# shahbuland/owl-audio-exps

Measured on AMD Instinct MI355X. Metric: latent-tokens/sec/GPU (fwd+bwd) DiT-v4 bf16; 1/2/4/8-GPU scaling, higher is better.
Workload: dtype bf16; 1 GPU; configs/dit_v4.yml training step: global batch 16 x 1536 frames x 8x8 latents (98304 tokens/sample), fwd+bwd + Muon/AdamW step + EMA; model=dit_v4 (16 L, d1536, 24 H, 704.9M params), global_batch=16, seq_len=98304, parallelism=dp1

## Files before the change

include/owlk.h:

```cpp
#ifndef OWLK_H
#define OWLK_H
#ifdef __cplusplus
extern "C" {
#endif

const char* owlk_last_error(void);
int owlk_version(void);
int owlk_device_ok(void);

#define OWLK_DECODE_COUNTER_BYTES 4096
int owlk_gemm(long M, long N, long K, long batch,
              const void* A, long lda, long sA, int a_trans,
              const void* B, long ldb, long sB, int b_trans,
              void* C, long ldc, long sC, int c_f32,
              int epi, float alpha, float beta, const float* bias,
              void* aux, long ldaux, long sAux,
              const void* gate, long ldgate, long sGate, long tpf,
              const void* resid, long ldres, long sRes,
              float* colsum, void* ws, long ws_bytes, void* stream);
#define OWLK_FRAME_ROWS 64
int owlk_gemm_frames(long M, long N, long K, const void* A, long lda, long a_fs, int a_trans,
                     const void* B, long ldb, long b_fs, int b_trans, void* C, long ldc, long c_fs,
                     int c_f32, int epi, float alpha, float beta, const float* bias, void* aux, long ldaux,
                     const void* gate, long ldgate, long tpf, const void* resid, long ldres, void* ws,
                     long ws_bytes, void* stream);
int owlk_gemm_attn_delta(long M, long N, long K, const void* dY, long lddy, const void* W, long ldw, void* dO,
                         long ldc, const void* o, long ldo, long L, int H, int D, float* delta, void* stream);
int owlk_gemm_qk_rope(long M, long N, long K, const void* A, long lda, const void* W, long ldw, const float* bias,
                      void* qkv, long ldq, int H, int D, const float* cosb, const float* sinb, long ld_tab, long n_tab,
                      long tab_off, long tpos_div, void* out, long ldo, float* rstd, void* stream);
long owlk_gemm_splitk_bytes(long M, long N, long K, long batch, int a_trans, int b_trans, int c_f32, int epi,
                            float beta);
long owlk_gemm_ws_bytes(long M, long N, long K, long batch, int a_trans, int b_trans, int c_f32, int epi,
                        float beta, int colsum);
long owlk_gemm_ws_counter_bytes(long M, long N, long K, long batch, int a_trans, int b_trans, int c_f32, int epi,
                                float beta);

int owlk_adaln_fwd(const void* x, long ldx, const void* scale, const void* shift, long ldm, long tpf,
                   long T, int d, void* y, long ldy, float* rstd, void* yact , void* stream);
int owlk_adaln_bwd(const void* dy, long lddy, const void* x, long ldx, const float* rstd,
                   const void* scale, long ldm, long tpf, long T, int d, const void* dres, long ldres,
                   void* dx, long lddx, void* dscale, void* dshift, long ldg,
                   const void* ypre , int mod_bf16, void* stream);

int owlk_gate_bwd(const void* dout, long ldo, const void* y, long ldy, const void* g, long ldg, long tpf,
                  long T, int d, void* dy, long lddy, void* dg, long lddg, int dg_bf16, float* dbias_frames,
                  long ldr, void* stream);
int owlk_adaln_gate_bwd(const void* dy, long lddy, const void* x, long ldx, const float* rstd,
                        const void* scale, long ldm, long tpf, long T, int d, const void* dres, long ldres,
                        void* dx, long lddx, void* dscale, void* dshift, long ldg, int mod_bf16,
                        const void* y, long ldy, const void* g, long ldgg, void* dyg, long lddyg, void* dg,
                        long lddg, int dg_bf16, float* dbias_frames, long ldr, void* stream);

int owlk_qk_rope_fwd(const void* qkv, long ldq, long T, int H, int D, const float* cosb, const float* sinb,
                     long ld_tab, long n_tab, long tab_off, long tpos_div, void* out, long ldo, float* rstd,
                     void* stream);
int owlk_qk_rope_fwd_kv(const void* qkv, long ldq, long T, long L, int H, int D, const float* cosb,
                        const float* sinb, long ld_tab, long n_tab, long tab_off, void* qo, long ldqo, long sqo,
                        void* ko, long ldko, long sko, void* vo, long ldvo, long svo, void* stream);
int owlk_qk_rope_fwd_kv_dev(const void* qkv, long ldq, long T, long L, int H, int D, const float* cosb,
                            const float* sinb, long ld_tab, long n_tab, const long* state, void* qo, long ldqo,
                            long sqo, void* kbuf, long ldk, long skb, void* vbuf, long ldv, long svb, long cap,
                            void* stream);
int owlk_mm_qk_rope_fwd_kv(const void* qkv0, long ld0, const void* qkv1, long ld1, long B, long nf, int n0, int n1,
                           int H, int D, const float* cosb, const float* sinb, long ld_tab, long n_tab,
                           long tab_off, void* qo, long ldqo, long sqo, void* ko, long ldko, long sko, void* vo,
                           long ldvo, long svo, void* stream);
int owlk_qk_rope_bwd(const void* dqk, long ldd, const void* qkv, long ldq, long T, int H, int D,
                     const float* cosb, const float* sinb, long ld_tab, long n_tab, long tab_off, long tpos_div,
                     const float* rstd, void* dqkv, long ldg, void* stream);
long owlk_qk_rope_bwd_ws_bytes(long T, int H, int D);
int owlk_qk_rope_bwd_bias(const void* dqk, long ldd, const void* qkv, long ldq, long T, int H, int D,
                          const float* cosb, const float* sinb, long ld_tab, long n_tab, long tab_off, long tpos_div,
                          const float* rstd, void* dqkv, long ldg, float* dbias, void* ws, long ws_bytes,
                          void* stream);

int owlk_attn_fwd(const void* q, long ldq, long sqb, const void* k, long ldk, long skb, const void* v,
                  long ldv, long svb, void* o, long ldo, long sob, float* lse, long B, int H, long Lq,
                  long Lkv, int head_dim, float scale, float score_bound, long tpf, int window, int causal,
                  long q_offset,
                  const int* kv_lo, const int* q_hi, const int* run_start, const int* doc, long fstride,
                  void* stream);
int owlk_attn_decode_fwd(const void* q, long ldq, long sqb, const void* kbuf, long ldk, long skb,
                         const void* vbuf, long ldv, long svb, void* o, long ldo, long sob, float* lse, long B,
                         int H, long Lq, int head_dim, float scale, float score_bound, const long* state,
                         long Lnew, long window_tokens, long cap, void* stream);
int owlk_attn_decode_joint_fwd(const void* q, long ldq, long sqb, const void* k, long ldk, long skb, const void* v,
                               long ldv, long svb, void* o0, long ldo0, void* o1, long ldo1, float* lse, long B,
                               int H, int n0, int n1, long Lkv, int head_dim, float scale, float score_bound,
                               void* stream);
int owlk_attn_delta(const void* o, const void* dout, long ld, long B, long L, int H, int D, float* delta,
                    void* stream);
int owlk_attn_bwd(const void* q, long ldq, long sqb, const void* k, long ldk, long skb, const void* v,
                  long ldv, long svb, const void* dout, long ldo, long sob, const float* lse,
                  const float* delta, void* dq, long lddq, long sdqb, void* dk, long lddk, long sdkb,
                  void* dv, long lddv, long sdvb, long B, int H, long Lq, long Lkv, int head_dim,
                  float scale, long tpf, int window, int causal, const int* kv_lo, const int* q_hi,
                  const int* run_start, const int* doc, long fstride, void* stream);
int owlk_attn_bwd_dkdv(const void* q, long ldq, long sqb, const void* k, long ldk, long skb, const void* v,
                       long ldv, long svb, const void* dout, long ldo, long sob, const float* lse,
                       const float* delta, void* dq, long lddq, long sdqb, void* dk, long lddk, long sdkb,
                       void* dv, long lddv, long sdvb, long B, int H, long Lq, long Lkv, int head_dim,
                       float scale, long tpf, int window, int causal, const int* kv_lo, const int* q_hi,
                       const int* run_start, const int* doc, long fstride, void* stream);
int owlk_attn_bwd_dq(const void* q, long ldq, long sqb, const void* k, long ldk, long skb, const void* v,
                     long ldv, long svb, const void* dout, long ldo, long sob, const float* lse,
                     const float* delta, void* dq, long lddq, long sdqb, void* dk, long lddk, long sdkb,
                     void* dv, long lddv, long sdvb, long B, int H, long Lq, long Lkv, int head_dim,
                     float scale, long tpf, int window, int causal, const int* kv_lo, const int* q_hi,
                     const int* run_start, const int* doc, long fstride, void* stream);

long owlk_attn_decode_bwd_ws_bytes(long B, int H, long Lq, long Lkv, int head_dim);
int owlk_attn_decode_bwd(const void* q, long ldq, long sqb, const void* k, long ldk, long skb, const void* v,
                         long ldv, long svb, const void* dout, long ldo, long sob, const float* lse,
                         const float* delta, void* dq, long lddq, long sdqb, void* dk_new, long lddk, long sdkb,
                         void* dv_new, long lddv, long sdvb, long B, int H, long Lq, long Lkv, long Lnew,
                         int head_dim, float scale, void* ws, long ws_bytes, void* stream);

long owlk_attn_bwd_fused_ws_bytes(long B, int H, long L, int head_dim);
int owlk_attn_bwd_fused(const void* q, long ldq, long sqb, const void* k, long ldk, long skb, const void* v,
                        long ldv, long svb, const void* dout, long ldo, long sob, const float* lse,
                        const float* delta, void* dq, long lddq, long sdqb, void* dk, long lddk, long sdkb,
                        void* dv, long lddv, long sdvb, long B, int H, long L, int head_dim, float scale,
                        long tpf, int window, int causal, const int* kv_lo, const int* q_hi,
                        const int* run_start, const int* doc, long fstride, void* ws, long ws_bytes,
                        int variant, void* stream);
int owlk_set_cu_reserve(int cus);

int owlk_flow_noise(const void* x, const void* z, const float* ts_raw, int C, int P, long BN, void* xt,
                    void* tgt, float* ts_out, void* stream);
int owlk_unpatchify(const void* tok, int C, int P, long BN, void* out, void* stream);
int owlk_gate_resid(const void* x, long ldx, const void* y, long ldy, const void* g, long ldg, long tpf, long T,
                    int d, void* out, long ldo, void* stream);
int owlk_mse(const void* pred, const void* tgt, long n, float gscale, void* dpred, float* partial,
             int nblocks, float* loss, void* stream);
int owlk_mse_grad(const void* pred, const void* tgt, long n, float gscale, const float* gout, void* dpred,
                  void* stream);
long owlk_dmd_loss_ws_bytes(long B, long N, long F);
int owlk_dmd_loss(const void* video, const void* noisy, int in_f32, const void* v_cond, const void* v_uncond,
                  const void* v_critic, int v_f32, const float* ts, const void* mask, long B, long N, long F,
                  float cfg_scale, float* loss, void* dvideo, void* ws, long ws_bytes, void* stream);
long owlk_critic_loss_ws_bytes(long n);
int owlk_critic_loss(const void* pred, int pred_f32, const void* z, const void* video, int in_f32,
                     const void* mask, long B, long N, long F, float gscale, float* loss, void* dpred, void* ws,
                     long ws_bytes, void* stream);
long owlk_colsum_ws_bytes(long R, long N);
int owlk_colsum(const void* x, int x_f32, long R, long N, long ld, float* out, void* ws, long ws_bytes,
                void* stream);
int owlk_colsum_frames(const void* x, int x_f32, long R, long N, long ld, long fs, float* out, void* ws,
                       long ws_bytes, void* stream);

#define OWLK_NORM_PARTS 256
int owlk_ns_normalize(const void* g, int g_f32, long rows, long cols, long batch, int transpose, void* x,
                      float* work, void* stream);
int owlk_ns_scale(const void* g, int g_f32, long rows, long cols, long batch, int transpose, void* x,
                  const float* sumsq, void* stream);
long owlk_ns_iterate_ws_bytes(long batch, long m, long k);
int owlk_ns_iterate(void* x, long batch, long m, long k, int steps, float a, float b, float c, void* ws,
                    long ws_bytes, void* stream);
long owlk_newton_schulz_ws_bytes(long batch, long rows, long cols);
int owlk_newton_schulz_bf16(const void* g, int g_f32, long batch, long rows, long cols, int steps, float a,
                            float b, float c, void* out, void* ws, long ws_bytes, void* stream);

int owlk_cond_embed(const void* ts, int ts_f32, const float* tfreq, int ht, float tmult, void* ts_in, long ldt,
                    const void* mouse, int mouse_f32, long ldm, const float* mfreq, int hm, float mmult,
                    const float* wang, void* mouse_in, long ldmi, void* ang, const void* btn, int btn_f32, long ldb,
                    int nb, int nbp, void* btn_in, long ldbi, long R, void* stream);
int owlk_cond_silu_fwd(const void* t, const void* m, const void* b, const void* hc, long rows_per, long R, int d,
                       void* cond, void* s, void* stream);
int owlk_cond_silu_bwd(const void* ds, int ds_bf16, const void* cond, const void* hc, long rows_per, long R, int d,
                       void* dcond, void* dctrl, void* stream);
int owlk_small_k_wgrad(const void* dy, long lddy, const void* x, long ldx, long R, long N, int K, float* dw,
                       long ldw, float beta, void* stream);

int owlk_muon_momentum(int count, float* const* g, float* const* buf, long n, float momentum, int nesterov,
                       float* stack, float* sumsq, void* stream);
int owlk_muon_apply(int count, float* const* p, const void* u, long rows, long cols, int transpose, float decay,
                    float alpha, void* stream);
int owlk_adamw(int count, float* const* p, const float* const* g, float* const* m, float* const* v, const long* n,
               float lr, float beta1, float beta2, float weight_decay, float eps, float step_size, float bc2_sqrt,
               void* stream);
int owlk_ema(int count, float* const* shadow, const float* const* p, const long* n, float weight, void* stream);

int owlk_frame_mux(int dir, long frames, int n0, int n1, int cols, void* a, long lda, void* b, long ldb,
                   void* joint, long ldj, void* stream);
int owlk_layernorm_fwd(const void* x, long ldx, long T, int d, void* y, long ldy, float* mean, float* rstd,
                       void* stream);
int owlk_layernorm_bwd(const void* dy, long lddy, const void* x, long ldx, const float* mean, const float* rstd,
                       long T, int d, void* dx, long lddx, void* stream);

#ifdef __cplusplus
}
#endif
#endif
```

owl-audio-exps_amd/csrc/gemm.hip:

```cpp
#include "common.hpp"

#include <algorithm>
#include <cstdlib>

namespace {

enum Epi : int {
  EPI_STORE = 0,
  EPI_SILU = 1,
  EPI_GATE_RESID = 2,
  EPI_DSILU = 3,
  EPI_AXPBY = 4,
  EPI_SCALE2 = 5,
  EPI_DELTA = 6,
  EPI_QKROPE = 7,
};

constexpr int BK = 64;
constexpr int NT = 256;

struct GemmP {
  long M, N, K;
  const bf16* A; long lda, sA;
  const bf16* B; long ldb, sB;
  void* C; long ldc, sC;
  float alpha, beta;
  const float* bias;
  bf16* aux; long ldaux, sAux;
  const bf16* gate; long ldgate, sGate, tpf;
  unsigned tpf_mul; int tpf_shift;
  const bf16* resid; long ldres, sRes;
  int tiles_m, tiles_n;
  long kchunk;
  float* ws;
  float* colsum_req;
  float* colsum;
  float* cs_part;
  int group_m;
  long a_fs, b_fs, c_fs;
  float* delta;
  long dl;
  const float* rcos;
  const float* rsin;
  long ld_tab, tab_off, tpos_div;
  float* rstd;
  long qk_cols;
};
constexpr float QK_RMS_EPS = 1.1920928955078125e-07f;

constexpr int FRAME_ROWS = 64;
#ifndef OWLK_GEMM_EPI2
#define OWLK_GEMM_EPI2 1
#endif

template <bool F>
DEV long row_off(long r, long ld, long fs) {
  return F ? (r >> 6) * fs + (r & 63) * ld : r * ld;
}

template <int ROWS>
DEV int swz_t(int k) {
  if (ROWS >= 128) return (k & 3) | (((k >> 3) & 1) << 2);
  return ((k >> 1) & 1) | (((k >> 3) & 1) << 1);
}

template <int ROWS, bool TRANS>
struct Stager {
  static constexpr int CHUNKS = ROWS * BK / 8;
  static constexpr int PER = CHUNKS / NT;
  bf16x8 r[PER];

  DEV void load(const bf16* base, long ld, long r0, long k0, long R, long K) {
    const int tid = threadIdx.x;
#pragma unroll
    for (int i = 0; i < PER; ++i) {
      const int c = tid + i * NT;
      long row, col;
      bool ok;
      if (!TRANS) {
        row = r0 + (c >> 3);
        col = k0 + (c & 7) * 8;
        ok = row < R && col < K;
        r[i] = ok ? *(const bf16x8*)(base + row * ld + col) : bf16x8{};
      } else {
        constexpr int CPR = ROWS / 8;
        row = k0 + c / CPR;
        col = r0 + (c % CPR) * 8;
        ok = row < K && col < R;
        r[i] = ok ? *(const bf16x8*)(base + row * ld + col) : bf16x8{};
      }
    }
  }

  DEV void store(char* lds) const {
    const int tid = threadIdx.x;
#pragma unroll
    for (int i = 0; i < PER; ++i) {
      const int c = tid + i * NT;
      int off;
      if (!TRANS) {
        const int row = c >> 3, kc = c & 7;
        off = row * 128 + ((kc ^ ((row >> 1) & 7)) << 4);
      } else {
        constexpr int CPR = ROWS / 8;
        const int k = c / CPR, mc = c % CPR;
        off = k * (ROWS * 2) + (((mc >> 1) ^ swz_t<ROWS>(k)) << 5) + ((mc & 1) << 4);
      }
      *(bf16x8*)(lds + off) = r[i];
    }
  }
};

template <int ROWS, bool TRANS>
DEV bf16x8 read_frag(const char* lds, int row0, int kk, int lane) {
  if (!TRANS) {
    const int r = row0 + (lane & 15);
    const int kc = 4 * kk + (lane >> 4);
    return *(const bf16x8*)(lds + r * 128 + ((kc ^ ((r >> 1) & 7)) << 4));
  } else {
    const int g = lane >> 4, q = (lane & 15) >> 2, pp = lane & 3;
    const int blk = row0 >> 4;
    const int k0 = 32 * kk + 8 * g + q;
    const int k1 = k0 + 4;
    s16x4 lo = ds_read_tr16(lds + k0 * (ROWS * 2) + ((blk ^ swz_t<ROWS>(k0)) << 5) + pp * 8);
    s16x4 hi = ds_read_tr16(lds + k1 * (ROWS * 2) + ((blk ^ swz_t<ROWS>(k1)) << 5) + pp * 8);
    return join_tr(lo, hi);
  }
}

template <int ROWS, bool TRANS>
DEV bf16x8 read_frag_async(const char* lds, int row0, int kk, int lane) {
  if (!TRANS) return read_frag<ROWS, false>(lds, row0, kk, lane);
  const int g = lane >> 4, q = (lane & 15) >> 2, pp = lane & 3;
  const int blk = row0 >> 4;
  const int k0 = 32 * kk + 8 * g + q;
  const int k1 = k0 + 4;
  s16x4 lo = ds_read_tr16_async(lds + k0 * (ROWS * 2) + ((blk ^ swz_t<ROWS>(k0)) << 5) + pp * 8);
  s16x4 hi = ds_read_tr16_async(lds + k1 * (ROWS * 2) + ((blk ^ swz_t<ROWS>(k1)) << 5) + pp * 8);
  return join_tr(lo, hi);
}

DEV unsigned frame_of(const GemmP& p, unsigned row) {
  return p.tpf_mul ? __umulhi(row, p.tpf_mul) >> p.tpf_shift : row >> p.tpf_shift;
}

template <int EPI, bool OF32>
DEV void epi_chunk(const GemmP& p, long z, long gm, long gn, float (&v)[8]) {
  float bb[8];
#pragma unroll
  for (int e = 0; e < 8; ++e) bb[e] = 0.f;
  if (p.bias) {
    const f32x4 lo = *(const f32x4*)(p.bias + gn), hi = *(const f32x4*)(p.bias + gn + 4);
#pragma unroll
    for (int e = 0; e < 4; ++e) {
      bb[e] = rb(lo[e]);
      bb[e + 4] = rb(hi[e]);
    }
  }
  if (EPI == EPI_STORE) {
#pragma unroll
    for (int e = 0; e < 8; ++e) v[e] = p.alpha * v[e] + bb[e];
    if (OF32) {
      float* C = (float*)p.C + z * p.sC + gm * p.ldc + gn;
      if (p.beta != 0.f) {
        const f32x4 o0 = *(const f32x4*)C, o1 = *(const f32x4*)(C + 4);
#pragma unroll
        for (int e = 0; e < 4; ++e) {
          v[e] += p.beta * o0[e];
          v[e + 4] += p.beta * o1[e];
        }
      }
      *(f32x4*)C = f32x4{v[0], v[1], v[2], v[3]};
      *(f32x4*)(C + 4) = f32x4{v[4], v[5], v[6], v[7]};
    } else {
      bf16* C = (bf16*)p.C + z * p.sC + gm * p.ldc + gn;
      if (p.beta != 0.f) {
        float o[8];
        unpack8(*(const bf16x8*)C, o);
#pragma unroll
        for (int e = 0; e < 8; ++e) v[e] += p.beta * o[e];
      }
      *(bf16x8*)C = pack8(v);
    }
  } else if (EPI == EPI_SILU) {
    float y[8], s[8];
#pragma unroll
    for (int e = 0; e < 8; ++e) {
      y[e] = rb(v[e] + bb[e]);
      s[e] = silu_f(y[e]);
    }
    *(bf16x8*)(p.aux + z * p.sAux + gm * p.ldaux + gn) = pack8(y);
    *(bf16x8*)((bf16*)p.C + z * p.sC + gm * p.ldc + gn) = pack8(s);
  } else if (EPI == EPI_GATE_RESID) {
    float y[8], g[8], r[8], o[8];
#pragma unroll
    for (int e = 0; e < 8; ++e) y[e] = rb(v[e] + bb[e]);
    unpack8(*(const bf16x8*)(p.gate + z * p.sGate + (long)frame_of(p, (unsigned)gm) * p.ldgate + gn), g);
    unpack8(*(const bf16x8*)(p.resid + z * p.sRes + gm * p.ldres + gn), r);
#pragma unroll
    for (int e = 0; e < 8; ++e) o[e] = r[e] + rb(g[e] * y[e]);
    if (p.aux) *(bf16x8*)(p.aux + z * p.sAux + gm * p.ldaux + gn) = pack8(y);
    *(bf16x8*)((bf16*)p.C + z * p.sC + gm * p.ldc + gn) = pack8(o);
  } else if (EPI == EPI_DSILU) {
    float x[8], o[8];
    unpack8(*(const bf16x8*)(p.aux + z * p.sAux + gm * p.ldaux + gn), x);
#pragma unroll
    for (int e = 0; e < 8; ++e) {
      const float sg = sigmoid_f(x[e]);
      o[e] = rb(v[e]) * sg * (1.f + x[e] * (1.f - sg));
    }
    *(bf16x8*)((bf16*)p.C + z * p.sC + gm * p.ldc + gn) = pack8(o);
    if (p.resid) {
      float a[8];
#pragma unroll
      for (int e = 0; e < 8; ++e) a[e] = silu_f(x[e]);
      *(bf16x8*)((bf16*)p.resid + z * p.sRes + gm * p.ldres + gn) = pack8(a);
    }
  } else if (EPI == EPI_AXPBY) {
    float x[8], o[8];
    unpack8(*(const bf16x8*)(p.aux + z * p.sAux + gm * p.ldaux + gn), x);
#pragma unroll
    for (int e = 0; e < 8; ++e) o[e] = rb(rb(p.alpha * rb(v[e])) + rb(p.beta * x[e]));
    *(bf16x8*)((bf16*)p.C + z * p.sC + gm * p.ldc + gn) = pack8(o);
  } else if (EPI == EPI_SCALE2) {
    float y[8], o[8];
#pragma unroll
    for (int e = 0; e < 8; ++e) {
      y[e] = rb(v[e]);
      o[e] = rb(p.alpha * y[e]);
    }
    *(bf16x8*)((bf16*)p.C + z * p.sC + gm * p.ldc + gn) = pack8(y);
    *(bf16x8*)(p.aux + z * p.sAux + gm * p.ldaux + gn) = pack8(o);
  }
}

DEV void st_nt(bf16x8* dst, bf16x8 v) { __builtin_nontemporal_store(v, dst); }

template <int EPI, bool OF32, bool CF = false>
DEV void epi_apply(const GemmP& p, long z, long gm, long gn, float (&v)[8], const float (&bb)[8], const bf16x8& x,
                   const bf16x8& g, float (&cs)[8]) {
  if (EPI == EPI_STORE) {
#pragma unroll
    for (int e = 0; e < 8; ++e) v[e] = p.alpha * v[e] + bb[e];
    if (OF32) {
      float* C = (float*)p.C + z * p.sC + gm * p.ldc + gn;
      if (p.beta != 0.f) {
        const f32x4 o0 = *(const f32x4*)C, o1 = *(const f32x4*)(C + 4);
#pragma unroll
        for (int e = 0; e < 4; ++e) {
          v[e] += p.beta * o0[e];
          v[e + 4] += p.beta * o1[e];
        }
      }
      *(f32x4*)C = f32x4{v[0], v[1], v[2], v[3]};
      *(f32x4*)(C + 4) = f32x4{v[4], v[5], v[6], v[7]};
    } else {
      bf16* C = (bf16*)p.C + z * p.sC + row_off<CF>(gm, p.ldc, p.c_fs) + gn;
      if (p.beta != 0.f) {
        float o[8];
        unpack8(*(const bf16x8*)C, o);
#pragma unroll
        for (int e = 0; e < 8; ++e) v[e] += p.beta * o[e];
      }
      st_nt((bf16x8*)C, pack8(v));
    }
  } else if (EPI == EPI_SILU) {
    float y[8], s[8];
#pragma unroll
    for (int e = 0; e < 8; ++e) {
      y[e] = rb(v[e] + bb[e]);
      s[e] = silu_f(y[e]);
    }
    st_nt((bf16x8*)(p.aux + z * p.sAux + gm * p.ldaux + gn), pack8(y));
    st_nt((bf16x8*)((bf16*)p.C + z * p.sC + gm * p.ldc + gn), pack8(s));
  } else if (EPI == EPI_GATE_RESID) {
    float y[8], gg[8], r[8], o[8];
#pragma unroll
    for (int e = 0; e < 8; ++e) y[e] = rb(v[e] + bb[e]);
    unpack8(g, gg);
    unpack8(x, r);
#pragma unroll
    for (int e = 0; e < 8; ++e) o[e] = r[e] + rb(gg[e] * y[e]);
    if (p.aux) st_nt((bf16x8*)(p.aux + z * p.sAux + gm * p.ldaux + gn), pack8(y));
    st_nt((bf16x8*)((bf16*)p.C + z * p.sC + gm * p.ldc + gn), pack8(o));
  } else if (EPI == EPI_DSILU) {
    float xx[8], o[8];
    unpack8(x, xx);
#pragma unroll
    for (int e = 0; e < 8; ++e) {
      const float sg = sigmoid_f(xx[e]);
      o[e] = rb(v[e]) * sg * (1.f + xx[e] * (1.f - sg));
    }
    st_nt((bf16x8*)((bf16*)p.C + z * p.sC + gm * p.ldc + gn), pack8(o));
    if (p.resid) {
      float a[8];
#pragma unroll
      for (int e = 0; e < 8; ++e) a[e] = silu_f(xx[e]);
      st_nt((bf16x8*)((bf16*)p.resid + z * p.sRes + gm * p.ldres + gn), pack8(a));
    }
    if (p.colsum) {
#pragma unroll
      for (int e = 0; e < 8; ++e) cs[e] += rb(o[e]);
    }
  } else if (EPI == EPI_AXPBY) {
    float xx[8], o[8];
    unpack8(x, xx);
#pragma unroll
    for (int e = 0; e < 8; ++e) o[e] = rb(rb(p.alpha * rb(v[e])) + rb(p.beta * xx[e]));
    st_nt((bf16x8*)((bf16*)p.C + z * p.sC + gm * p.ldc + gn), pack8(o));
  } else if (EPI == EPI_SCALE2) {
    float y[8], o[8];
#pragma unroll
    for (int e = 0; e < 8; ++e) {
      y[e] = rb(v[e]);
      o[e] = rb(p.alpha * y[e]);
    }
    st_nt((bf16x8*)((bf16*)p.C + z * p.sC + gm * p.ldc + gn), pack8(y));
    st_nt((bf16x8*)(p.aux + z * p.sAux + gm * p.ldaux + gn), pack8(o));
  }
}

template <int EPI, bool OF32>
DEV void epi_apply2(const GemmP& p, long c, long ao, long ro, float (&v)[8], const float (&bb)[8],
                    const bf16x8& x, const bf16x8& g, float (&cs)[8]) {
  const u32x4 xw = __builtin_bit_cast(u32x4, x), gw = __builtin_bit_cast(u32x4, g);
  u32x4 o, y;
  if (EPI == EPI_STORE) {
#pragma unroll
    for (int e = 0; e < 8; ++e) v[e] = p.alpha * v[e] + bb[e];
    if (OF32) {
      float* C = (float*)p.C + c;
      if (p.beta != 0.f) {
        const f32x4 o0 = *(const f32x4*)C, o1 = *(const f32x4*)(C + 4);
#pragma unroll
        for (int e = 0; e < 4; ++e) {
          v[e] += p.beta * o0[e];
          v[e + 4] += p.beta * o1[e];
        }
      }
      *(f32x4*)C = f32x4{v[0], v[1], v[2], v[3]};
      *(f32x4*)(C + 4) = f32x4{v[4], v[5], v[6], v[7]};
    } else {
      bf16* C = (bf16*)p.C + c;
      if (p.beta != 0.f) {
        float ob[8];
        unpack8(*(const bf16x8*)C, ob);
#pragma unroll
        for (int e = 0; e < 8; ++e) v[e] += p.beta * ob[e];
      }
#pragma unroll
      for (int k = 0; k < 4; ++k) o[k] = cvt2(v[2 * k], v[2 * k + 1]);
      st_nt((bf16x8*)C, __builtin_bit_cast(bf16x8, o));
    }
  } else if (EPI == EPI_SILU) {
#pragma unroll
    for (int k = 0; k < 4; ++k) {
      y[k] = cvt2(v[2 * k] + bb[2 * k], v[2 * k + 1] + bb[2 * k + 1]);
      o[k] = cvt2(silu_f(bf_lo(y[k])), silu_f(bf_hi(y[k])));
    }
    st_nt((bf16x8*)(p.aux + ao), __builtin_bit_cast(bf16x8, y));
    st_nt((bf16x8*)((bf16*)p.C + c), __builtin_bit_cast(bf16x8, o));
  } else if (EPI == EPI_GATE_RESID) {
#pragma unroll
    for (int k = 0; k < 4; ++k) {
      y[k] = cvt2(v[2 * k] + bb[2 * k], v[2 * k + 1] + bb[2 * k + 1]);
      const unsigned t = cvt2(bf_lo(gw[k]) * bf_lo(y[k]), bf_hi(gw[k]) * bf_hi(y[k]));
      o[k] = cvt2(bf_lo(xw[k]) + bf_lo(t), bf_hi(xw[k]) + bf_hi(t));
    }
    if (p.aux) st_nt((bf16x8*)(p.aux + ao), __builtin_bit_cast(bf16x8, y));
    st_nt((bf16x8*)((bf16*)p.C + c), __builtin_bit_cast(bf16x8, o));
  } else if (EPI == EPI_DSILU) {
    u32x4 a;
#pragma unroll
    for (int k = 0; k < 4; ++k) {
      const unsigned rv = cvt2(v[2 * k], v[2 * k + 1]);
      float ov[2];
#pragma unroll
      for (int h = 0; h < 2; ++h) {
        const float xx = h ? bf_hi(xw[k]) : bf_lo(xw[k]);
        const float sg = sigmoid_f(xx);
        ov[h] = (h ? bf_hi(rv) : bf_lo(rv)) * sg * (1.f + xx * (1.f - sg));
      }
      o[k] = cvt2(ov[0], ov[1]);
      a[k] = cvt2(silu_f(bf_lo(xw[k])), silu_f(bf_hi(xw[k])));
      cs[2 * k] += bf_lo(o[k]);
      cs[2 * k + 1] += bf_hi(o[k]);
    }
    st_nt((bf16x8*)((bf16*)p.C + c), __builtin_bit_cast(bf16x8, o));
    if (p.resid) st_nt((bf16x8*)((bf16*)p.resid + ro), __builtin_bit_cast(bf16x8, a));
  } else if (EPI == EPI_AXPBY) {
#pragma unroll
    for (int k = 0; k < 4; ++k) {
      const unsigned r = cvt2(v[2 * k], v[2 * k + 1]);
      const unsigned s1 = cvt2(p.alpha * bf_lo(r), p.alpha * bf_hi(r));
      const unsigned s2 = cvt2(p.beta * bf_lo(xw[k]), p.beta * bf_hi(xw[k]));
      o[k] = cvt2(bf_lo(s1) + bf_lo(s2), bf_hi(s1) + bf_hi(s2));
    }
    st_nt((bf16x8*)((bf16*)p.C + c), __builtin_bit_cast(bf16x8, o));
  } else if (EPI == EPI_SCALE2) {
#pragma unroll
    for (int k = 0; k < 4; ++k) {
      y[k] = cvt2(v[2 * k], v[2 * k + 1]);
      o[k] = cvt2(p.alpha * bf_lo(y[k]), p.alpha * bf_hi(y[k]));
    }
    st_nt((bf16x8*)((bf16*)p.C + c), __builtin_bit_cast(bf16x8, y));
    st_nt((bf16x8*)(p.aux + ao), __builtin_bit_cast(bf16x8, o));
  } else if (EPI == EPI_QKROPE) {
#pragma unroll
    for (int e = 0; e < 8; ++e) v[e] = p.alpha * v[e] + bb[e];
#pragma unroll
    for (int k = 0; k < 4; ++k) {
      o[k] = cvt2(v[2 * k], v[2 * k + 1]);
      cs[2 * k] = bf_lo(o[k]);
      cs[2 * k + 1] = bf_hi(o[k]);
    }
    st_nt((bf16x8*)((bf16*)p.C + c), __builtin_bit_cast(bf16x8, o));
  } else if (EPI == EPI_DELTA) {
    float sd = 0.f;
#pragma unroll
    for (int k = 0; k < 4; ++k) {
      o[k] = cvt2(p.alpha * v[2 * k], p.alpha * v[2 * k + 1]);
      sd += bf_lo(xw[k]) * bf_lo(o[k]);
      sd += bf_hi(xw[k]) * bf_hi(o[k]);
    }
    st_nt((bf16x8*)((bf16*)p.C + c), __builtin_bit_cast(bf16x8, o));
    cs[0] = sd;
  }
}

template <int BM, int BN, bool AT, bool BT, int EPI, bool OF32>
__global__ __launch_bounds__(NT) void gemm_kernel(GemmP p) {
  constexpr int WTM = BM / 2, WTN = BN / 2;
  constexpr int TM = WTM / 16, TN = WTN / 16;
  constexpr int A_BYTES = BM * BK * 2, B_BYTES = BN * BK * 2;
  constexpr int STAGE_BYTES = 2 * (A_BYTES + B_BYTES);
  constexpr int EPI_LD = BN + 4;
  constexpr int EPI_BYTES = BM * EPI_LD * 4;
  constexpr int LDS_BYTES = STAGE_BYTES > EPI_BYTES ? STAGE_BYTES : EPI_BYTES;
  __shared__ __attribute__((aligned(16))) char smem[LDS_BYTES];

  const int lane = threadIdx.x & 63, wave = threadIdx.x >> 6;
  const int wm = wave >> 1, wn = wave & 1;

  const int nwg = p.tiles_m * p.tiles_n;
  int bid = blockIdx.x;
  {
    const int q = nwg / 8, r = nwg % 8, x = bid % 8;
    bid = (x < r ? x * (q + 1) : r * (q + 1) + (x - r) * q) + bid / 8;
  }
  const int tm = bid / p.tiles_n, tn = bid % p.tiles_n;
  const long m0 = (long)tm * BM, n0 = (long)tn * BN;
  const long z = blockIdx.z;
  const bf16* A = p.A + z * p.sA;
  const bf16* B = p.B + z * p.sB;

  Stager<BM, AT> sa;
  Stager<BN, BT> sb;
  f32x4 acc[TM][TN];
#pragma unroll
  for (int i = 0; i < TM; ++i)
#pragma unroll
    for (int j = 0; j < TN; ++j) acc[i][j] = f32x4{0.f, 0.f, 0.f, 0.f};

  const long kbeg = (long)blockIdx.y * p.kchunk;
  const long kend = kbeg + p.kchunk < p.K ? kbeg + p.kchunk : p.K;
  const int nk = (int)((kend - kbeg + BK - 1) / BK);
  sa.load(A, p.lda, m0, kbeg, p.M, p.K);
  sb.load(B, p.ldb, n0, kbeg, p.N, p.K);
  sa.store(smem);
  sb.store(smem + A_BYTES);
  __syncthreads();

  for (int kt = 0; kt < nk; ++kt) {
    const int cur = kt & 1;
    const bool more = kt + 1 < nk;
    if (more) {
      sa.load(A, p.lda, m0, kbeg + (long)(kt + 1) * BK, p.M, p.K);
      sb.load(B, p.ldb, n0, kbeg + (long)(kt + 1) * BK, p.N, p.K);
    }
    const char* la = smem + cur * (A_BYTES + B_BYTES);
    const char* lb = la + A_BYTES;
#pragma unroll
    for (int kk = 0; kk < 2; ++kk) {
      bf16x8 af[TM], bfr[TN];
#pragma unroll
      for (int i = 0; i < TM; ++i) af[i] = read_frag<BM, AT>(la, wm * WTM + 16 * i, kk, lane);
#pragma unroll
      for (int j = 0; j < TN; ++j) bfr[j] = read_frag<BN, BT>(lb, wn * WTN + 16 * j, kk, lane);
#pragma unroll
      for (int i = 0; i < TM; ++i)
#pragma unroll
        for (int j = 0; j < TN; ++j)
          acc[i][j] = __builtin_amdgcn_mfma_f32_16x16x32_bf16(af[i], bfr[j], acc[i][j], 0, 0, 0);
    }
    if (more) {
      char* nb = smem + (cur ^ 1) * (A_BYTES + B_BYTES);
      sa.store(nb);
      sb.store(nb + A_BYTES);
    }
    __syncthreads();
  }

  float* ct = (float*)smem;
#pragma unroll
  for (int i = 0; i < TM; ++i)
#pragma unroll
    for (int j = 0; j < TN; ++j) {
      const int col = wn * WTN + 16 * j + (lane & 15);
      const int row = wm * WTM + 16 * i + (lane >> 4) * 4;
#pragma unroll
      for (int r = 0; r < 4; ++r) ct[(row + r) * EPI_LD + col] = acc[i][j][r];
    }
  __syncthreads();

  if (p.ws) {
    float* W = p.ws + (long)blockIdx.y * p.M * p.N;
    for (int c = threadIdx.x; c < BM * BN / 4; c += NT) {
      const int row = c / (BN / 4), col = (c % (BN / 4)) * 4;
      const long gm = m0 + row, gn = n0 + col;
      if (gm < p.M && gn < p.N)
        __builtin_nontemporal_store(*(const f32x4*)(ct + row * EPI_LD + col), (f32x4*)(W + gm * p.N + gn));
    }
    return;
  }
  if (OF32 && EPI == EPI_STORE && gridDim.y > 1) {
    float* C = (float*)p.C + z * p.sC;
    for (int row = wave; row < BM; row += NT / 64) {
      const long gm = m0 + row;
      if (gm >= p.M) break;
#pragma unroll
      for (int cc = 0; cc < BN; cc += 64) {
        const long gn = n0 + cc + lane;
        if (gn < p.N) atomicAdd(C + gm * p.ldc + gn, p.alpha * ct[row * EPI_LD + cc + lane]);
      }
    }
    return;
  }

  constexpr int CH = BM * BN / 8;
  for (int c = threadIdx.x; c < CH; c += NT) {
    const int row = c / (BN / 8), col = (c % (BN / 8)) * 8;
    const long gm = m0 + row, gn = n0 + col;
    if (gm >= p.M || gn >= p.N) continue;
    float v[8];
    {
      const f32x4 lo = *(const f32x4*)(ct + row * EPI_LD + col);
      const f32x4 hi = *(const f32x4*)(ct + row * EPI_LD + col + 4);
#pragma unroll
      for (int e = 0; e < 4; ++e) {
        v[e] = lo[e];
        v[e + 4] = hi[e];
      }
    }
    epi_chunk<EPI, OF32>(p, z, gm, gn, v);
  }
}


constexpr int NT8 = 512;

template <int ROWS, bool TRANS, bool F = false>
DEV void glds_tile(char* lds, const bf16* base, long ld, long r0, long k0, long R, int wave, int lane, long fs = 0) {
  if (!TRANS) {
#pragma unroll
    for (int i = 0; i < ROWS / 64; ++i) {
      const int rbase = (wave * (ROWS / 64) + i) * 8;
      const int row = rbase + (lane >> 3);
      const int ch = (lane & 7) ^ ((row >> 1) & 7);
      long gr = r0 + row;
      gr = gr < R ? gr : R - 1;
      __builtin_amdgcn_global_load_lds((const void __attribute__((address_space(1)))*)(base + row_off<F>(gr, ld, fs) +
                                                                                         k0 + ch * 8),
                                       (void __attribute__((address_space(3)))*)(lds + rbase * 128), 16, 0, 0);
    }
  } else {
    constexpr int KPI = 512 / ROWS;
    constexpr int CPR = ROWS / 8;
#pragma unroll
    for (int i = 0; i < 64 / KPI / 8; ++i) {
      const int kb = (wave * (64 / KPI / 8) + i) * KPI;
      const int k = kb + lane / CPR;
      const int pch = lane % CPR;
      const int lch = ((((pch >> 1) ^ swz_t<ROWS>(k))) << 1) | (pch & 1);
      __builtin_amdgcn_global_load_lds(
          (const void __attribute__((address_space(1)))*)(base + row_off<F>(k0 + k, ld, fs) + r0 + lch * 8),
          (void __attribute__((address_space(3)))*)(lds + kb * ROWS * 2), 16, 0, 0);
    }
  }
}

template <int BN, bool AT, bool BT, int EPI, bool OF32>
__global__ __launch_bounds__(NT8, 1) void gemm256_kernel(GemmP p) {
  constexpr int BM = 256, WARPS_N = BN / 64, WTM = BM / (8 / WARPS_N), WTN = 64, TM = WTM / 16, TN = 4;
  constexpr int NBUF = BN == 256 ? 2 : 3;
  constexpr int A_BYTES = BM * BK * 2, B_BYTES = BN * BK * 2, STAGE = A_BYTES + B_BYTES;
  constexpr int OPS = (BM + BN) * BK * 2 / (NT8 * 16);
  __shared__ __attribute__((aligned(16))) char smem[NBUF * STAGE];
  const int lane = threadIdx.x & 63, wave = __builtin_amdgcn_readfirstlane(threadIdx.x >> 6);
  const int wm = wave / WARPS_N, wn = wave % WARPS_N;

  const int nwg = p.tiles_m * p.tiles_n;
  int bid = blockIdx.x;
  {
    const int q = nwg / 8, r = nwg % 8, x = bid % 8;
    bid = (x < r ? x * (q + 1) : r * (q + 1) + (x - r) * q) + bid / 8;
  }
  const int tm = bid / p.tiles_n, tn = bid % p.tiles_n;
  const long m0 = (long)tm * BM, n0 = (long)tn * BN;
  const long z = blockIdx.z;
  const bf16* A = p.A + z * p.sA;
  const bf16* B = p.B + z * p.sB;
  const long kbeg = (long)blockIdx.y * p.kchunk;
  const long kend = kbeg + p.kchunk < p.K ? kbeg + p.kchunk : p.K;
  const int nk = (int)((kend - kbeg) / BK);

  f32x4 acc[TM][TN];
#pragma unroll
  for (int i = 0; i < TM; ++i)
#pragma unroll
    for (int j = 0; j < TN; ++j) acc[i][j] = f32x4{0.f, 0.f, 0.f, 0.f};

  auto issue = [&](int kt) {
    char* buf = smem + (kt % NBUF) * STAGE;
    glds_tile<BM, AT>(buf, A, p.lda, m0, kbeg + (long)kt * BK, p.M, wave, lane);
    glds_tile<BN, BT>(buf + A_BYTES, B, p.ldb, n0, kbeg + (long)kt * BK, p.N, wave, lane);
  };
  auto wait_next = [&](bool younger_in_flight) {
    if (NBUF > 2 && younger_in_flight)
      asm volatile("s_waitcnt vmcnt(%0)" ::"n"(OPS) : "memory");
    else
      asm volatile("s_waitcnt vmcnt(0)" ::: "memory");
  };
#pragma unroll
  for (int i = 0; i < NBUF - 1; ++i)
    if (i < nk) issue(i);
  wait_next(nk > 1);
  asm volatile("s_waitcnt lgkmcnt(0)\n\ts_barrier" ::: "memory");

  for (int kt = 0; kt < nk; ++kt) {
    if (kt + NBUF - 1 < nk) issue(kt + NBUF - 1);
    const char* la = smem + (kt % NBUF) * STAGE;
    const char* lb = la + A_BYTES;
#pragma unroll
    for (int kk = 0; kk < 2; ++kk) {
      bf16x8 af[TM], bfr[TN];
#pragma unroll
      for (int j = 0; j < TN; ++j) bfr[j] = read_frag<BN, BT>(lb, wn * WTN + 16 * j, kk, lane);
#pragma unroll
      for (int i = 0; i < TM; ++i) af[i] = read_frag<BM, AT>(la, wm * WTM + 16 * i, kk, lane);
      __builtin_amdgcn_s_setprio(1);
#pragma unroll
      for (int i = 0; i < TM; ++i)
#pragma unroll
        for (int j = 0; j < TN; ++j)
          acc[i][j] = __builtin_amdgcn_mfma_f32_16x16x32_bf16(af[i], bfr[j], acc[i][j], 0, 0, 0);
      __builtin_amdgcn_s_setprio(0);
    }
    wait_next(kt + NBUF - 1 < nk);
    asm volatile("s_waitcnt lgkmcnt(0)\n\ts_barrier" ::: "memory");
  }

  float* strip = (float*)smem + wave * (16 * 68);
  const bool atomic = OF32 && EPI == EPI_STORE && gridDim.y > 1;
#pragma unroll
  for (int i = 0; i < TM; ++i) {
#pragma unroll
    for (int j = 0; j < TN; ++j)
#pragma unroll
      for (int r = 0; r < 4; ++r) strip[((lane >> 4) * 4 + r) * 68 + 16 * j + (lane & 15)] = acc[i][j][r];
    asm volatile("s_waitcnt lgkmcnt(0)" ::: "memory");
    const long rbase = m0 + wm * WTM + 16 * i;
    if (atomic) {
      float* C = (float*)p.C + z * p.sC;
#pragma unroll
      for (int rr = 0; rr < 16; ++rr) {
        const long gm = rbase + rr;
        if (gm < p.M) atomicAdd(C + gm * p.ldc + n0 + wn * WTN + lane, p.alpha * strip[rr * 68 + lane]);
      }
    } else {
#pragma unroll
      for (int q = 0; q < 2; ++q) {
        const int c = lane + 64 * q;
        const int rr = c >> 3, col = (c & 7) * 8;
        const long gm = rbase + rr, gn = n0 + wn * WTN + col;
        float v[8];
        const f32x4 lo = *(const f32x4*)(strip + rr * 68 + col);
        const f32x4 hi = *(const f32x4*)(strip + rr * 68 + col + 4);
#pragma unroll
        for (int e = 0; e < 4; ++e) {
          v[e] = lo[e];
          v[e + 4] = hi[e];
        }
        if (gm < p.M) epi_chunk<EPI, OF32>(p, z, gm, gn, v);
      }
    }
    asm volatile("s_waitcnt lgkmcnt(0)" ::: "memory");
  }
}

template <bool AT, bool BT, int EPI, bool OF32, int FS = 0>
__global__ __launch_bounds__(NT8, 1) void gemm_pp_kernel(GemmP p) {
  constexpr bool FA = FS & 1, FB = (FS & 2) != 0, FC = (FS & 4) != 0;
  constexpr int HALF = 128 * BK * 2, STAGE = 4 * HALF;
  __shared__ __attribute__((aligned(16))) char smem[2 * STAGE];
  const int lane = threadIdx.x & 63, wave = __builtin_amdgcn_readfirstlane(threadIdx.x >> 6);
  const int wr = wave >> 2, wc = wave & 3;

  const int nwg = p.tiles_m * p.tiles_n;
  int bid = blockIdx.x;
  {
    const int q = nwg / 8, r = nwg % 8, x = bid % 8;
    bid = (x < r ? x * (q + 1) : r * (q + 1) + (x - r) * q) + bid / 8;
  }
  int tm, tn;
  if (p.group_m > 1) {
    const int span = p.group_m * p.tiles_n, g = bid / span, first = g * p.group_m;
    const int gs = p.tiles_m - first < p.group_m ? p.tiles_m - first : p.group_m;
    tm = first + (bid % span) % gs;
    tn = (bid % span) / gs;
  } else {
    tm = bid / p.tiles_n;
    tn = bid % p.tiles_n;
  }
  const long m0 = (long)tm * 256, n0 = (long)tn * 256;
  const long z = blockIdx.z;
  const bf16* A = p.A + z * p.sA;
  const bf16* B = p.B + z * p.sB;
  const long kbeg = (long)blockIdx.y * p.kchunk;
  const long kend = kbeg + p.kchunk < p.K ? kbeg + p.kchunk : p.K;
  const int nk = (int)((kend - kbeg) / BK);

  f32x4 acc[8][4];
#pragma unroll
  for (int i = 0; i < 8; ++i)
#pragma unroll
    for (int j = 0; j < 4; ++j) acc[i][j] = f32x4{0.f, 0.f, 0.f, 0.f};

  auto issueA = [&](int t) {
    char* st = smem + (t & 1) * STAGE;
    glds_tile<128, AT, FA>(st, A, p.lda, m0, kbeg + (long)t * BK, p.M, wave, lane, p.a_fs);
    glds_tile<128, AT, FA>(st + HALF, A, p.lda, m0 + 128, kbeg + (long)t * BK, p.M, wave, lane, p.a_fs);
  };
  auto issueB = [&](int t) {
    char* st = smem + (t & 1) * STAGE + 2 * HALF;
    glds_tile<128, BT, FB>(st, B, p.ldb, n0, kbeg + (long)t * BK, p.N, wave, lane, p.b_fs);
    glds_tile<128, BT, FB>(st + HALF, B, p.ldb, n0 + 128, kbeg + (long)t * BK, p.N, wave, lane, p.b_fs);
  };
  const int bcol = (wc & 1) * 64;
  auto readA = [&](bf16x8 (&af)[4][2], const char* la, int mh) {
#pragma unroll
    for (int kk = 0; kk < 2; ++kk)
#pragma unroll
      for (int i = 0; i < 4; ++i) af[i][kk] = read_frag_async<128, AT>(la, 64 * mh + 16 * i, kk, lane);
  };
  auto readB = [&](bf16x8 (&bq)[2][2], const char* lb, int nh) {
#pragma unroll
    for (int kk = 0; kk < 2; ++kk)
#pragma unroll
      for (int j = 0; j < 2; ++j) bq[j][kk] = read_frag_async<128, BT>(lb, bcol + 32 * nh + 16 * j, kk, lane);
  };
  auto quad = [&](const bf16x8 (&af)[4][2], const bf16x8 (&bq)[2][2], int mh, int nh) {
    __builtin_amdgcn_s_setprio(1);
#pragma unroll
    for (int kk = 0; kk < 2; ++kk)
#pragma unroll
      for (int i = 0; i < 4; ++i)
#pragma unroll
        for (int j = 0; j < 2; ++j)
          acc[4 * mh + i][2 * nh + j] =
              __builtin_amdgcn_mfma_f32_16x16x32_bf16(af[i][kk], bq[j][kk], acc[4 * mh + i][2 * nh + j], 0, 0, 0);
    __builtin_amdgcn_s_setprio(0);
  };
#define OWLK_PP_BAR() asm volatile("s_barrier" ::: "memory")
#define OWLK_PP_SYNC()                                                  \
  do {                                                                  \
    asm volatile("s_barrier\n\ts_waitcnt lgkmcnt(0)" ::: "memory");   \
    __builtin_amdgcn_sched_barrier(0);                                  \
  } while (0)

  issueA(0);
  issueB(0);
  if (nk > 1) {
    issueB(1);
    asm volatile("s_waitcnt vmcnt(4)" ::: "memory");
  } else {
    asm volatile("s_waitcnt vmcnt(0)" ::: "memory");
  }
  OWLK_PP_BAR();
  if (wr == 1) OWLK_PP_BAR();

  bf16x8 af[4][2], b0[2][2], b1[2][2];
  for (int t = 0; t < nk; ++t) {
    const char* la = smem + (t & 1) * STAGE + wr * HALF;
    const char* lb = smem + (t & 1) * STAGE + (2 + (wc >> 1)) * HALF;
    readB(b0, lb, 0);
    readA(af, la, 0);
    if (t + 1 < nk) issueA(t + 1);
    OWLK_PP_SYNC();
    quad(af, b0, 0, 0);
    OWLK_PP_BAR();
    readB(b1, lb, 1);
    OWLK_PP_SYNC();
    quad(af, b1, 0, 1);
    OWLK_PP_BAR();
    readA(af, la, 1);
    OWLK_PP_SYNC();
    quad(af, b1, 1, 1);
    OWLK_PP_BAR();
    if (t + 2 < nk) {
      issueB(t + 2);
      asm volatile("s_waitcnt vmcnt(4)" ::: "memory");
    } else {
      asm volatile("s_waitcnt vmcnt(0)" ::: "memory");
    }
    OWLK_PP_SYNC();
    quad(af, b0, 1, 0);
    OWLK_PP_BAR();
  }
  if (wr == 0) OWLK_PP_BAR();
#undef OWLK_PP_BAR
#undef OWLK_PP_SYNC
#ifdef OWLK_GEMM_EXP_NOEPI
  {
    float t = 0.f;
#pragma unroll
    for (int i = 0; i < 8; ++i)
#pragma unroll
      for (int j = 0; j < 4; ++j) t += acc[i][j][0];
    if (t == 1234.5f) ((float*)p.C)[threadIdx.x] = t;
    return;
  }
#endif

  const long wrow0 = m0 + 128 * wr, wcol0 = n0 + 64 * wc;
  float* strip = (float*)smem + wave * (16 * 68);
  const bool atomic = OF32 && EPI == EPI_STORE && gridDim.y > 1;
  const int ccol = (lane & 7) * 8;
  const long gn = wcol0 + ccol;
  float bb[8];
#pragma unroll
  for (int e = 0; e < 8; ++e) bb[e] = 0.f;
  if (!atomic && p.bias) {
    const f32x4 lo = *(const f32x4*)(p.bias + gn), hi = *(const f32x4*)(p.bias + gn + 4);
#pragma unroll
    for (int e = 0; e < 4; ++e) {
      bb[e] = rb(lo[e]);
      bb[e + 4] = rb(hi[e]);
    }
  }
  constexpr bool HAS_X = EPI == EPI_GATE_RESID || EPI == EPI_DSILU || EPI == EPI_AXPBY || EPI == EPI_DELTA;
  constexpr bool HAS_G = EPI == EPI_GATE_RESID;
  static_assert((EPI != EPI_DELTA && EPI != EPI_QKROPE) || OWLK_GEMM_EPI2,
                "EPI_DELTA / EPI_QKROPE are built in the paired epilogue only");
  constexpr int PD = (EPI == EPI_DSILU || EPI == EPI_AXPBY || EPI == EPI_DELTA) ? 8 : (EPI == EPI_GATE_RESID ? 4 : 1);
  bf16x8 xin[8][2], gin[8][2];
  const int l8 = lane >> 3;
  const bool full = m0 + 256 <= p.M;
  const long cbase = z * p.sC + row_off<FC>(wrow0 + l8, p.ldc, p.c_fs) + gn;
  const long abase = z * p.sAux + (wrow0 + l8) * p.ldaux + gn;
  const long rbase0 = z * p.sRes + (wrow0 + l8) * p.ldres + gn;
  auto c_step = [&](int d) { return FC ? (long)(d >> 6) * p.c_fs + (long)(d & 63) * p.ldc : (long)d * p.ldc; };
  auto load_in = [&](int i, bf16x8 (&x)[2], bf16x8 (&g)[2]) {
#pragma unroll
    for (int q = 0; q < 2; ++q) {
      long gm = wrow0 + 16 * i + 8 * q + (lane >> 3);
      gm = gm < p.M ? gm : p.M - 1;
      if (HAS_X && OWLK_GEMM_EPI2) {
        const int d = 16 * i + 8 * q;
        const long xo = EPI == EPI_GATE_RESID ? (full ? rbase0 + d * p.ldres : z * p.sRes + gm * p.ldres + gn)
                                              : (full ? abase + d * p.ldaux : z * p.sAux + gm * p.ldaux + gn);
        x[q] = *(const bf16x8*)((EPI == EPI_GATE_RESID ? p.resid : p.aux) + xo);
      } else if (HAS_X) {
        const bf16* src = EPI == EPI_GATE_RESID ? p.resid + z * p.sRes + gm * p.ldres
                                                 : p.aux + z * p.sAux + gm * p.ldaux;
        x[q] = *(const bf16x8*)(src + gn);
      }
      if (HAS_G) g[q] = *(const bf16x8*)(p.gate + z * p.sGate + (long)frame_of(p, (unsigned)gm) * p.ldgate + gn);
    }
  };
  if (!atomic) {
#pragma unroll
    for (int i = 0; i < PD; ++i) load_in(i, xin[i], gin[i]);
  }
  float cs[8];
#pragma unroll
  for (int e = 0; e < 8; ++e) cs[e] = 0.f;
#pragma unroll
  for (int i = 0; i < 8; ++i) {
    if (!atomic && i + PD < 8) load_in(i + PD, xin[i + PD], gin[i + PD]);
    f32x4 rcv[2], rsv[2];
    if constexpr (EPI == EPI_QKROPE) {
      if (wcol0 < p.qk_cols) {
#pragma unroll
        for (int q = 0; q < 2; ++q) {
          long gm = wrow0 + 16 * i + 8 * q + (lane >> 3);
          gm = gm < p.M ? gm : p.M - 1;
          const long pos = p.tab_off + (p.tpos_div > 0 ? gm % p.tpos_div : gm);
          rcv[q] = *(const f32x4*)(p.rcos + pos * p.ld_tab + (lane & 7) * 4);
          rsv[q] = *(const f32x4*)(p.rsin + pos * p.ld_tab + (lane & 7) * 4);
        }
      }
    }
#pragma unroll
    for (int j = 0; j < 4; ++j)
#pragma unroll
      for (int r = 0; r < 4; ++r) strip[((lane >> 4) * 4 + r) * 68 + 16 * j + (lane & 15)] = acc[i][j][r];
    asm volatile("s_waitcnt lgkmcnt(0)" ::: "memory");
    const long rbase = wrow0 + 16 * i;
    if (atomic && p.ws) {
      float* W = p.ws + (long)blockIdx.y * p.M * p.N;
#pragma unroll
      for (int rq = 0; rq < 4; ++rq) {
        const int rr = 4 * rq + (lane >> 4);
        const long gm = rbase + rr;
        if (gm < p.M)
          *(f32x4*)(W + gm * p.N + wcol0 + 4 * (lane & 15)) = *(const f32x4*)(strip + rr * 68 + 4 * (lane & 15));
      }
    } else if (atomic) {
      float* C = (float*)p.C + z * p.sC;
#pragma unroll
      for (int rr = 0; rr < 16; ++rr) {
        const long gm = rbase + rr;
        if (gm < p.M) atomicAdd(C + gm * p.ldc + wcol0 + lane, p.alpha * strip[rr * 68 + lane]);
      }
    } else {
#pragma unroll
      for (int q = 0; q < 2; ++q) {
        const int rr = 8 * q + (lane >> 3);
        const long gm = rbase + rr;
        float v[8];
        const f32x4 lo = *(const f32x4*)(strip + rr * 68 + ccol);
        const f32x4 hi = *(const f32x4*)(strip + rr * 68 + ccol + 4);
#pragma unroll
        for (int e = 0; e < 4; ++e) {
          v[e] = lo[e];
          v[e + 4] = hi[e];
        }
        if (OWLK_GEMM_EPI2) {
          const int d = 16 * i + 8 * q;
          if (gm < p.M)
            epi_apply2<EPI, OF32>(p, cbase + c_step(d), abase + d * p.ldaux, rbase0 + d * p.ldres, v, bb, xin[i][q],
                                  gin[i][q], cs);
          if constexpr (EPI == EPI_QKROPE) {
            if (wcol0 < p.qk_cols) {
              float ss = 0.f;
#pragma unroll
              for (int e = 0; e < 8; ++e) ss += cs[e] * cs[e];
              ss = gm < p.M ? ss : 0.f;
              ss += __shfl_xor(ss, 1, 64);
              ss += __shfl_xor(ss, 2, 64);
              ss += __shfl_xor(ss, 4, 64);
              const float r = rsqrtf(ss / 64 + QK_RMS_EPS);
              if (gm < p.M) {
                const int j = lane & 7;
                const long wh = wcol0 >> 6;
                if (j == 0 && p.rstd) p.rstd[gm * (p.qk_cols >> 6) + wh] = r;
                const f32x4 cv = rcv[q], sv = rsv[q];
                bf16x4 y0, y1;
#pragma unroll
                for (int e = 0; e < 4; ++e) {
                  const float x0 = rb(cs[2 * e] * r), x1 = rb(cs[2 * e + 1] * r);
                  y0[e] = (bf16)(x0 * cv[e] - x1 * sv[e]);
                  y1[e] = (bf16)(x1 * cv[e] + x0 * sv[e]);
                }
                const uint2 w0 = __builtin_bit_cast(uint2, y0), w1 = __builtin_bit_cast(uint2, y1);
                const bool odd = j & 1;
                const uint2 snd = odd ? w0 : w1;
                const uint2 rcv{(unsigned)__shfl_xor((int)snd.x, 1, 64), (unsigned)__shfl_xor((int)snd.y, 1, 64)};
                const u32x4 ow = odd ? u32x4{rcv.x, rcv.y, w1.x, w1.y} : u32x4{w0.x, w0.y, rcv.x, rcv.y};
                *(u32x4*)(p.aux + gm * p.ldaux + wh * 64 + (odd ? 32 : 0) + 8 * (j >> 1)) = ow;
              }
            }
          }
          if constexpr (EPI == EPI_DELTA) {
            float sd = gm < p.M ? cs[0] : 0.f;
            sd += __shfl_xor(sd, 1, 64);
            sd += __shfl_xor(sd, 2, 64);
            sd += __shfl_xor(sd, 4, 64);
            if ((lane & 7) == 0 && gm < p.M) {
              const long b = gm / p.dl;
              p.delta[(b * (p.N >> 6) + (gn >> 6)) * p.dl + (gm - b * p.dl)] = sd;
            }
          }
        } else if (gm < p.M) {
          if constexpr (EPI != EPI_DELTA && EPI != EPI_QKROPE)
            epi_apply<EPI, OF32, FC>(p, z, gm, gn, v, bb, xin[i][q], gin[i][q], cs);
        }
      }
    }
    asm volatile("s_waitcnt lgkmcnt(0)" ::: "memory");
  }
  if (EPI == EPI_DSILU && p.colsum) {
#pragma unroll
    for (int e = 0; e < 8; ++e) {
      cs[e] += __shfl_xor(cs[e], 8, 64);
      cs[e] += __shfl_xor(cs[e], 16, 64);
      cs[e] += __shfl_xor(cs[e], 32, 64);
    }
    if (lane < 8) {
      if (p.cs_part) {
        float* dst = p.cs_part + (long)(2 * tm + wr) * p.N + gn;
        *(f32x4*)dst = f32x4{cs[0], cs[1], cs[2], cs[3]};
        *(f32x4*)(dst + 4) = f32x4{cs[4], cs[5], cs[6], cs[7]};
      } else {
#pragma unroll
        for (int e = 0; e < 8; ++e) atomicAdd(p.colsum + gn + e, cs[e]);
      }
    }
  }
}

template <int BM, int BN, bool AT, bool BT, int EPI, bool OF32>
int launch(GemmP& p, long batch, hipStream_t s) {
  p.tiles_m = (int)((p.M + BM - 1) / BM);
  p.tiles_n = (int)((p.N + BN - 1) / BN);
  const int splits = (int)((p.K + p.kchunk - 1) / p.kchunk);
  dim3 grid(p.tiles_m * p.tiles_n, (unsigned)splits, (unsigned)batch);
  hipLaunchKernelGGL((gemm_kernel<BM, BN, AT, BT, EPI, OF32>), grid, dim3(NT), 0, s, p);
  return owlk::check_launch("gemm");
}

template <int BM, int BN, int EPI, bool OF32>
int dispatch_t(GemmP& p, int at, int bt, long batch, hipStream_t s) {
  if (!at && !bt) return launch<BM, BN, false, false, EPI, OF32>(p, batch, s);
  if (!at && bt) return launch<BM, BN, false, true, EPI, OF32>(p, batch, s);
  if (at && bt) return launch<BM, BN, true, true, EPI, OF32>(p, batch, s);
  return launch<BM, BN, true, false, EPI, OF32>(p, batch, s);
}

template <int BM, int BN>
int dispatch_e(GemmP& p, int at, int bt, int epi, int cf32, long batch, hipStream_t s) {
  switch (epi) {
    case EPI_STORE:
      return cf32 ? dispatch_t<BM, BN, EPI_STORE, true>(p, at, bt, batch, s)
                  : dispatch_t<BM, BN, EPI_STORE, false>(p, at, bt, batch, s);
    case EPI_SILU: return dispatch_t<BM, BN, EPI_SILU, false>(p, at, bt, batch, s);
    case EPI_GATE_RESID: return dispatch_t<BM, BN, EPI_GATE_RESID, false>(p, at, bt, batch, s);
    case EPI_DSILU: return dispatch_t<BM, BN, EPI_DSILU, false>(p, at, bt, batch, s);
    case EPI_AXPBY: return dispatch_t<BM, BN, EPI_AXPBY, false>(p, at, bt, batch, s);
    case EPI_SCALE2:
      if (at || bt) break;
      return launch<BM, BN, false, false, EPI_SCALE2, false>(p, batch, s);
  }
  owlk::set_error("gemm: unknown epilogue %d", epi);
  return 1;
}


template <bool AT, bool BT, int EPI, bool OF32>
int launch256(GemmP& p, long batch, hipStream_t s) {
  p.tiles_m = (int)((p.M + 255) / 256);
  p.tiles_n = (int)((p.N + 255) / 256);
  const int splits = (int)((p.K + p.kchunk - 1) / p.kchunk);
  dim3 grid(p.tiles_m * p.tiles_n, (unsigned)splits, (unsigned)batch);
  static const int pp = getenv("OWLK_GEMM_PP") ? atoi(getenv("OWLK_GEMM_PP")) : 1;
  static const int fuse_cs = getenv("OWLK_GEMM_COLSUM") ? atoi(getenv("OWLK_GEMM_COLSUM")) : 1;
  if (pp && EPI == EPI_DSILU && batch == 1 && fuse_cs) p.colsum = p.colsum_req;
  static const int group_m = getenv("OWLK_GEMM_GROUP") ? atoi(getenv("OWLK_GEMM_GROUP")) : -1;
  p.group_m = group_m >= 0 ? group_m : (splits == 1 && p.kchunk <= 4096 ? 4 : 0);
  const int fs = (p.a_fs ? 1 : 0) | (p.b_fs ? 2 : 0) | (p.c_fs ? 4 : 0);
  if (fs) {
    bool ok = false;
    if constexpr (!AT && !BT && EPI == EPI_STORE && !OF32) {
      if (fs == 4) {
        hipLaunchKernelGGL((gemm_pp_kernel<AT, BT, EPI, OF32, 4>), grid, dim3(NT8), 0, s, p);
        ok = true;
      }
    }
    if constexpr (!AT && !BT && EPI == EPI_GATE_RESID) {
      if (fs == 1) {
        hipLaunchKernelGGL((gemm_pp_kernel<AT, BT, EPI, OF32, 1>), grid, dim3(NT8), 0, s, p);
        ok = true;
      }
    }
    if constexpr (!AT && BT && EPI == EPI_STORE && !OF32) {
      if (fs == 4) {
        hipLaunchKernelGGL((gemm_pp_kernel<AT, BT, EPI, OF32, 4>), grid, dim3(NT8), 0, s, p);
        ok = true;
      }
      if (fs == 1) {
        hipLaunchKernelGGL((gemm_pp_kernel<AT, BT, EPI, OF32, 1>), grid, dim3(NT8), 0, s, p);
        ok = true;
      }
    }
    if constexpr (AT && BT && EPI == EPI_STORE && OF32) {
      if (fs == 1) {
        hipLaunchKernelGGL((gemm_pp_kernel<AT, BT, EPI, OF32, 1>), grid, dim3(NT8), 0, s, p);
        ok = true;
      }
      if (fs == 2) {
        hipLaunchKernelGGL((gemm_pp_kernel<AT, BT, EPI, OF32, 2>), grid, dim3(NT8), 0, s, p);
        ok = true;
      }
    }
    OWLK_REQUIRE(ok && pp, "gemm: frame-strided rows (mask %d) not built for this operand layout / epilogue", fs);
    return owlk::check_launch("gemm256");
  }
  if constexpr (EPI == EPI_DELTA || EPI == EPI_QKROPE) {
    OWLK_REQUIRE(pp && splits == 1 && batch == 1, "gemm: the delta / rope epilogues run in the unsplit ping-pong kernel");
    hipLaunchKernelGGL((gemm_pp_kernel<AT, BT, EPI, OF32>), grid, dim3(NT8), 0, s, p);
  } else if (pp) {
    hipLaunchKernelGGL((gemm_pp_kernel<AT, BT, EPI, OF32>), grid, dim3(NT8), 0, s, p);
  } else {
    hipLaunchKernelGGL((gemm256_kernel<256, AT, BT, EPI, OF32>), grid, dim3(NT8), 0, s, p);
  }
  return owlk::check_launch("gemm256");
}

template <int EPI, bool OF32>
int dispatch256_t(GemmP& p, int at, int bt, long batch, hipStream_t s) {
  if (!at && !bt) return launch256<false, false, EPI, OF32>(p, batch, s);
  if (!at && bt) return launch256<false, true, EPI, OF32>(p, batch, s);
  if (at && bt) return launch256<true, true, EPI, OF32>(p, batch, s);
  return launch256<true, false, EPI, OF32>(p, batch, s);
}

int dispatch256(GemmP& p, int at, int bt, int epi, int cf32, long batch, hipStream_t s) {
  switch (epi) {
    case EPI_STORE:
      return cf32 ? dispatch256_t<EPI_STORE, true>(p, at, bt, batch, s)
                  : dispatch256_t<EPI_STORE, false>(p, at, bt, batch, s);
    case EPI_SILU: return dispatch256_t<EPI_SILU, false>(p, at, bt, batch, s);
    case EPI_GATE_RESID: return dispatch256_t<EPI_GATE_RESID, false>(p, at, bt, batch, s);
    case EPI_DSILU: return dispatch256_t<EPI_DSILU, false>(p, at, bt, batch, s);
    case EPI_AXPBY: return dispatch256_t<EPI_AXPBY, false>(p, at, bt, batch, s);
    case EPI_SCALE2:
      if (at || bt) break;
      return launch256<false, false, EPI_SCALE2, false>(p, batch, s);
    case EPI_DELTA:
      if (at || !bt) break;
      return launch256<false, true, EPI_DELTA, false>(p, batch, s);
    case EPI_QKROPE:
      if (at || bt) break;
      return launch256<false, false, EPI_QKROPE, false>(p, batch, s);
  }
  owlk::set_error("gemm: unknown epilogue %d", epi);
  return 1;
}
__global__ __launch_bounds__(256) void splitk_reduce_k(const float* __restrict__ W, int splits, long M, long N,
                                                       float* C, long ldc, float alpha, float beta) {
  const long nq = N / 4, total = M * nq, MN = M * N;
  for (long i = (long)blockIdx.x * 256 + threadIdx.x; i < total; i += (long)gridDim.x * 256) {
    const long m = i / nq, n = (i - m * nq) * 4;
    const float* w = W + m * N + n;
    f32x4 a = __builtin_nontemporal_load((const f32x4*)w);
    for (int sp = 1; sp < splits; ++sp) {
      const f32x4 b = __builtin_nontemporal_load((const f32x4*)(w + sp * MN));
#pragma unroll
      for (int e = 0; e < 4; ++e) a[e] += b[e];
    }
    f32x4* c = (f32x4*)(C + m * ldc + n);
    f32x4 o;
    if (beta != 0.f) {
      const f32x4 old = *c;
#pragma unroll
      for (int e = 0; e < 4; ++e) o[e] = alpha * a[e] + beta * old[e];
    } else {
#pragma unroll
      for (int e = 0; e < 4; ++e) o[e] = alpha * a[e];
    }
    *c = o;
  }
}

template <int EPI>
__global__ __launch_bounds__(256) void splitk_epi_k(GemmP p, int splits) {
  const long n8 = p.N / 8, total = p.M * n8, MN = p.M * p.N;
  for (long i = (long)blockIdx.x * 256 + threadIdx.x; i < total; i += (long)gridDim.x * 256) {
    const long m = i / n8, n = (i - m * n8) * 8;
    const float* w = p.ws + m * p.N + n;
    float v[8];
    {
      const f32x4 lo = __builtin_nontemporal_load((const f32x4*)w), hi = __builtin_nontemporal_load((const f32x4*)(w + 4));
#pragma unroll
      for (int e = 0; e < 4; ++e) {
        v[e] = lo[e];
        v[e + 4] = hi[e];
      }
    }
#pragma unroll 8
    for (int sp = 1; sp < splits; ++sp) {
      const f32x4 lo = __builtin_nontemporal_load((const f32x4*)(w + sp * MN));
      const f32x4 hi = __builtin_nontemporal_load((const f32x4*)(w + sp * MN + 4));
#pragma unroll
      for (int e = 0; e < 4; ++e) {
        v[e] += lo[e];
        v[e + 4] += hi[e];
      }
    }
    epi_chunk<EPI, false>(p, 0, m, n, v);
  }
}

constexpr int DEC_T = 64;
constexpr int DEC_KC = 256;
constexpr int DEC_ROWB = DEC_KC * 2;
constexpr int DEC_LD = DEC_T + 4;
constexpr long kDecodeCounterBytes = 4096;

template <int EPI>
__global__ __launch_bounds__(256, 1) void gemm_decode_k(GemmP p, int* counters, int nsub) {
  constexpr int STAGE = 2 * DEC_T * DEC_ROWB;
  __shared__ __attribute__((aligned(16))) char smem[2 * STAGE];
  float* tilef = (float*)smem;
  int* flag = (int*)(smem + DEC_T * DEC_LD * 4);
  const int lane = threadIdx.x & 63, wave = threadIdx.x >> 6;
  const int tile = blockIdx.x, split = blockIdx.y, S = gridDim.y, mt = blockIdx.z;
  const int tiles = gridDim.x;
  const long n0 = (long)tile * DEC_T, m0 = (long)mt * DEC_T;
  const int r16 = lane & 15, g = lane >> 4;
  const long kfirst = (long)split * nsub * DEC_KC;
  const int nst = (int)((p.K - kfirst + DEC_KC - 1) / DEC_KC < nsub ? (p.K - kfirst + DEC_KC - 1) / DEC_KC : nsub);
  const bool isw = wave < 2;
  const bf16* rowp[16];
#pragma unroll
  for (int j = 0; j < 16; ++j) {
    const int r = (wave & 1) * 32 + 2 * j + (lane >> 5);
    if (isw) {
      rowp[j] = p.B + (n0 + r) * p.ldb;
    } else {
      const long m = m0 + r < p.M ? m0 + r : p.M - 1;
      rowp[j] = p.A + m * p.lda;
    }
  }
  const int ldsrow0 = (isw ? 0 : DEC_T) + (wave & 1) * 32;
  auto issue = [&](int i) {
    const long kbeg = kfirst + (long)i * DEC_KC;
    const int nch = (int)((p.K - kbeg < DEC_KC ? p.K - kbeg : DEC_KC) / 8);
    char* buf = smem + (i & 1) * STAGE + ldsrow0 * DEC_ROWB;
#pragma unroll
    for (int j = 0; j < 16; ++j) {
      const int r = 2 * j + (lane >> 5);
      int ch = (lane & 31) ^ r;
      ch = ch < nch ? ch : nch - 1;
      __builtin_amdgcn_global_load_lds((const void __attribute__((address_space(1)))*)(rowp[j] + kbeg + ch * 8),
                                       (void __attribute__((address_space(3)))*)(buf + 2 * j * DEC_ROWB), 16, 0, 0);
    }
  };
  f32x4 acc[4];
#pragma unroll
  for (int j = 0; j < 4; ++j) acc[j] = f32x4{0.f, 0.f, 0.f, 0.f};
  const int xr = DEC_T + 16 * wave + r16;
  issue(0);
  if (nst > 1) issue(1);
  for (int sc = 0; sc < nst; ++sc) {
    if (sc + 1 < nst)
      asm volatile("s_waitcnt vmcnt(16)" ::: "memory");
    else
      asm volatile("s_waitcnt vmcnt(0)" ::: "memory");
    asm volatile("s_barrier" ::: "memory");
    const long kbeg = kfirst + (long)sc * DEC_KC;
    const int kc = (int)(p.K - kbeg < DEC_KC ? p.K - kbeg : DEC_KC);
    const char* buf = smem + (sc & 1) * STAGE;
    for (int st = 0; st < kc / 32; ++st) {
      const int c = 4 * st + g;
      const bf16x8 a = *(const bf16x8*)(buf + xr * DEC_ROWB + ((c ^ (xr & 31)) << 4));
#pragma unroll
      for (int j = 0; j < 4; ++j) {
        const int wr = 16 * j + r16;
        const bf16x8 b = *(const bf16x8*)(buf + wr * DEC_ROWB + ((c ^ (wr & 31)) << 4));
        acc[j] = __builtin_amdgcn_mfma_f32_16x16x32_bf16(a, b, acc[j], 0, 0, 0);
      }
    }
    if (sc + 2 < nst) {
      asm volatile("s_waitcnt lgkmcnt(0)\n\ts_barrier" ::: "memory");
      issue(sc + 2);
    }
  }
  __syncthreads();
#pragma unroll
  for (int j = 0; j < 4; ++j)
#pragma unroll
    for (int r = 0; r < 4; ++r) tilef[(16 * wave + 4 * g + r) * DEC_LD + 16 * j + r16] = acc[j][r];
  __syncthreads();
  const long rows = p.M - m0 < DEC_T ? p.M - m0 : DEC_T;
  const long pstride = (long)tiles * DEC_T * DEC_T * 4;
  const long mbase = (long)mt * S * pstride + (long)tile * DEC_T * DEC_T * 4;
  const __amdgpu_buffer_rsrc_t prs =
      __builtin_amdgcn_make_buffer_rsrc(p.ws, (short)0, S > 1 ? (int)(S * pstride * gridDim.z) : 0, 0x00020000);
  for (int it = threadIdx.x; it < DEC_T * (DEC_T / 8); it += 256) {
    const int row = it >> 3, c = (it & 7) * 8;
    if (row >= rows) continue;
    const f32x4 lo = *(const f32x4*)(tilef + row * DEC_LD + c), hi = *(const f32x4*)(tilef + row * DEC_LD + c + 4);
    if (S == 1) {
      float v[8] = {lo[0], lo[1], lo[2], lo[3], hi[0], hi[1], hi[2], hi[3]};
      epi_chunk<EPI, false>(p, 0, m0 + row, n0 + c, v);
    } else {
      const int off = (int)(mbase + split * pstride + (row * DEC_T + c) * 4);
      __builtin_amdgcn_raw_buffer_store_b128(__builtin_bit_cast(u32x4, lo), prs, off, 0, 16);
      __builtin_amdgcn_raw_buffer_store_b128(__builtin_bit_cast(u32x4, hi), prs, off + 16, 0, 16);
    }
  }
  if (S == 1) return;
  asm volatile("s_waitcnt vmcnt(0)" ::: "memory");
  __syncthreads();
  int* cnt = counters + mt * tiles + tile;
  if (threadIdx.x == 0) *flag = __hip_atomic_fetch_add(cnt, 1, __ATOMIC_RELAXED, __HIP_MEMORY_SCOPE_AGENT);
  __syncthreads();
  if (*flag != S - 1) return;
  __builtin_amdgcn_fence(__ATOMIC_ACQUIRE, "wavefront");
  for (int it = threadIdx.x; it < DEC_T * (DEC_T / 8); it += 256) {
    const int row = it >> 3, c = (it & 7) * 8;
    if (row >= rows) continue;
    const int off = (int)(mbase + (row * DEC_T + c) * 4);
    float v[8];
#pragma unroll
    for (int e = 0; e < 8; ++e) v[e] = 0.f;
#pragma unroll 4
    for (int sp = 0; sp < S; ++sp) {
      const f32x4 lo = __builtin_bit_cast(f32x4, __builtin_amdgcn_raw_buffer_load_b128(prs, off + sp * (int)pstride, 0, 16));
      const f32x4 hi =
          __builtin_bit_cast(f32x4, __builtin_amdgcn_raw_buffer_load_b128(prs, off + sp * (int)pstride + 16, 0, 16));
#pragma unroll
      for (int e = 0; e < 4; ++e) {
        v[e] += lo[e];
        v[e + 4] += hi[e];
      }
    }
    epi_chunk<EPI, false>(p, 0, m0 + row, n0 + c, v);
  }
  if (threadIdx.x == 0) __hip_atomic_store(cnt, 0, __ATOMIC_RELAXED, __HIP_MEMORY_SCOPE_AGENT);
}

void decode_split(long M, long N, long K, long& S, long& nsub) {
  const long mtiles = (M + DEC_T - 1) / DEC_T, tiles = N / DEC_T, subs = (K + DEC_KC - 1) / DEC_KC;
  static const int force = getenv("OWLK_DECODE_NSUB") ? atoi(getenv("OWLK_DECODE_NSUB")) : 0;
  long sp = 256 / (tiles * mtiles);
  if (sp < 1) sp = 1;
  nsub = force > 0 ? force : (subs + sp - 1) / sp;
  if (nsub > subs) nsub = subs;
  S = (subs + nsub - 1) / nsub;
}

int launch_decode(GemmP& p, int epi, void* ws, hipStream_t s) {
  long S, nsub;
  decode_split(p.M, p.N, p.K, S, nsub);
  const long tiles = p.N / DEC_T, mtiles = (p.M + DEC_T - 1) / DEC_T;
  int* counters = (int*)ws;
  p.ws = S > 1 ? (float*)((char*)ws + kDecodeCounterBytes) : nullptr;
  const dim3 grid((unsigned)tiles, (unsigned)S, (unsigned)mtiles);
  switch (epi) {
    case EPI_STORE: hipLaunchKernelGGL(gemm_decode_k<EPI_STORE>, grid, dim3(256), 0, s, p, counters, (int)nsub); break;
    case EPI_SILU: hipLaunchKernelGGL(gemm_decode_k<EPI_SILU>, grid, dim3(256), 0, s, p, counters, (int)nsub); break;
    default: hipLaunchKernelGGL(gemm_decode_k<EPI_GATE_RESID>, grid, dim3(256), 0, s, p, counters, (int)nsub); break;
  }
  return owlk::check_launch("gemm_decode");
}

long pick_splits(long tiles, long K) {
  constexpr long CUS = 256;
  long best = 1;
  double best_score = -1.0;
  for (long sp = 2; sp <= 64 && K / sp >= 2048; ++sp) {
    const long wg = tiles * sp;
    if (wg < 2 * CUS) continue;
    const long rounds = (wg + CUS - 1) / CUS;
    const double score = (double)wg / (double)(rounds * CUS) - 0.004 * (double)sp;
    if (score > best_score) {
      best_score = score;
      best = sp;
    }
  }
  return best;
}
}

static bool fits256(long M, long N, long K, int a_trans, int b_trans, int c_f32, float beta) {
  static const int use256 = getenv("OWLK_GEMM_NO256") ? 0 : 1;
  return use256 && K % 64 == 0 && N % 256 == 0 && (!a_trans || M % 256 == 0) && (!b_trans || N % 256 == 0) &&
         !(c_f32 && beta != 0.f && beta != 1.f);
}
static long min_tiles256() {
  static const long v = getenv("OWLK_GEMM_MIN256") ? atol(getenv("OWLK_GEMM_MIN256")) : 192;
  return v;
}
static long skinny_splits(long M, long N, long K, long batch, int c_f32, int epi, float beta) {
  if (batch != 1 || c_f32 || M > 256 || K < 512 || K % BK) return 1;
  if (!(epi == EPI_SILU || epi == EPI_GATE_RESID || (epi == EPI_STORE && beta == 0.f))) return 1;
  const long tiles = ((M + 63) / 64) * ((N + 63) / 64);
  if (tiles >= 256) return 1;
  long sp = (768 + tiles - 1) / tiles;
  const long maxsp = K / (2 * BK);
  if (sp > maxsp) sp = maxsp;
  if (sp < 2) return 1;
  const long kchunk = ((K + sp - 1) / sp + BK - 1) / BK * BK;
  return (K + kchunk - 1) / kchunk;
}

enum SplitKind { SPLIT_NONE = 0, SPLIT_SKINNY, SPLIT_256, SPLIT_128, SPLIT_DECODE };
struct SplitPlan {
  int kind;
  long splits, kchunk;
  bool opt = false;
};

static SplitPlan split_plan(long M, long N, long K, long batch, int a_trans, int b_trans, int c_f32, int epi,
                            float beta, bool frames = false, bool allow_opt = true) {
  SplitPlan pl{SPLIT_NONE, 1, K, false};
  static const int use_decode = getenv("OWLK_GEMM_DECODE") ? atoi(getenv("OWLK_GEMM_DECODE")) : 1;
  if (use_decode && !frames && M <= 128 && batch == 1 && !a_trans && !b_trans && !c_f32 && N % DEC_T == 0 && K % 32 == 0 &&
      ((M + DEC_T - 1) / DEC_T) * (N / DEC_T) <= kDecodeCounterBytes / 4 &&
      (epi == EPI_SILU || epi == EPI_GATE_RESID || epi == EPI_STORE)) {
    decode_split(M, N, K, pl.splits, pl.kchunk);
    pl.kind = SPLIT_DECODE;
    return pl;
  }
  auto chunk = [&](long sp) { return ((K + sp - 1) / sp + BK - 1) / BK * BK; };
  const long sk = frames ? 1 : skinny_splits(M, N, K, batch, c_f32, epi, beta);
  if (sk > 1) {
    pl.kchunk = chunk(sk);
    pl.splits = (K + pl.kchunk - 1) / pl.kchunk;
    pl.kind = SPLIT_SKINNY;
    return pl;
  }
  const long tiles128 = ((M + 127) / 128) * ((N + 127) / 128) * batch;
  const long tiles256 = ((M + 255) / 256) * ((N + 255) / 256) * batch;
  if (fits256(M, N, K, a_trans, b_trans, c_f32, beta)) {
    if (c_f32 && epi == EPI_STORE && batch == 1 && (beta == 0.f || beta == 1.f) && K >= 8192 && tiles256 < 1024) {
      const long sp = pick_splits(tiles256, K);
      if (sp > 1) {
        pl.kchunk = chunk(sp);
        pl.splits = (K + pl.kchunk - 1) / pl.kchunk;
        pl.kind = SPLIT_256;
        return pl;
      }
    }
    if (allow_opt && c_f32 && epi == EPI_STORE && batch == 1 && (beta == 0.f || beta == 1.f) && K >= 8192 &&
        K < 16384 && tiles256 < 128) {
      long sp = 256 / tiles256;
      if (sp > K / 1024) sp = K / 1024;
      if (sp > 1) {
        pl.kchunk = chunk(sp);
        pl.splits = (K + pl.kchunk - 1) / pl.kchunk;
        pl.kind = SPLIT_256;
        pl.opt = true;
        return pl;
      }
    }
    if (tiles256 >= min_tiles256()) return pl;
  }
  if (c_f32 && epi == EPI_STORE && (beta == 1.f || (beta == 0.f && batch == 1)) && K >= 8192 && tiles128 < 1024) {
    long sp = (1024 + tiles128 - 1) / tiles128;
    if (sp > K / 4096) sp = K / 4096;
    if (sp > 1) {
      pl.kchunk = chunk(sp);
      pl.splits = (K + pl.kchunk - 1) / pl.kchunk;
      pl.kind = SPLIT_128;
    }
  }
  return pl;
}

static long split_ws_bytes(const SplitPlan& pl, long M, long N, long batch) {
  if (pl.kind == SPLIT_NONE || (pl.kind == SPLIT_128 && batch != 1)) return 0;
  if (pl.kind == SPLIT_DECODE)
    return pl.splits > 1 ? kDecodeCounterBytes + pl.splits * ((M + DEC_T - 1) / DEC_T) * DEC_T * N * (long)sizeof(float)
                         : 0;
  return pl.splits * M * N * (long)sizeof(float);
}

static int gemm_dispatch(GemmP& p, long M, long N, long K, long batch,
                         const void* A, long lda, long sA, int a_trans,
                         const void* B, long ldb, long sB, int b_trans,
                         void* C, long ldc, long sC, int c_f32,
                         int epi, float alpha, float beta, const float* bias,
                         void* aux, long ldaux, long sAux,
                         const void* gate, long ldgate, long sGate, long tpf,
                         const void* resid, long ldres, long sRes,
                         void* ws, long ws_bytes, void* stream) {
  OWLK_REQUIRE(M > 0 && N > 0 && K > 0 && batch > 0, "gemm: bad sizes M=%ld N=%ld K=%ld b=%ld", M, N, K, batch);
  OWLK_REQUIRE(N % 8 == 0, "gemm: N=%ld must be a multiple of 8", N);
  OWLK_REQUIRE(a_trans ? (M % 8 == 0) : (K % 8 == 0), "gemm: A contiguous dim must be a multiple of 8");
  OWLK_REQUIRE(b_trans ? (N % 8 == 0) : (K % 8 == 0), "gemm: B contiguous dim must be a multiple of 8");
  OWLK_REQUIRE(lda % 8 == 0 && ldb % 8 == 0 && ldc % 8 == 0, "gemm: leading dims must be multiples of 8");
  OWLK_REQUIRE(((uintptr_t)A | (uintptr_t)B | (uintptr_t)C) % 16 == 0, "gemm: operands must be 16-byte aligned");
  OWLK_REQUIRE(!c_f32 || epi == EPI_STORE, "gemm: fp32 output only with EPI_STORE");
  OWLK_REQUIRE(epi != EPI_GATE_RESID || (gate && resid && tpf > 0), "gemm: gate epilogue needs gate/resid/tpf");
  OWLK_REQUIRE(epi != EPI_GATE_RESID || M < (1L << 31), "gemm: gate epilogue rows must stay below 2^31");
  OWLK_REQUIRE(!(epi == EPI_SILU || epi == EPI_DSILU || epi == EPI_AXPBY || epi == EPI_SCALE2) || aux,
               "gemm: epilogue needs aux");
  OWLK_REQUIRE(epi != EPI_SCALE2 || (!a_trans && !b_trans), "gemm: SCALE2 epilogue needs k-contiguous operands");
  p.M = M; p.N = N; p.K = K;
  p.A = (const bf16*)A; p.lda = lda; p.sA = sA;
  p.B = (const bf16*)B; p.ldb = ldb; p.sB = sB;
  p.C = C; p.ldc = ldc; p.sC = sC;
  p.alpha = alpha; p.beta = beta; p.bias = bias;
  p.aux = (bf16*)aux; p.ldaux = ldaux; p.sAux = sAux;
  p.gate = (const bf16*)gate; p.ldgate = ldgate; p.sGate = sGate; p.tpf = tpf > 0 ? tpf : 1;
  {
    int sh = 0;
    while ((2L << sh) <= p.tpf) ++sh;
    p.tpf_shift = sh;
    p.tpf_mul = (p.tpf & (p.tpf - 1)) ? (unsigned)(((1ULL << (32 + sh)) + p.tpf - 1) / p.tpf) : 0u;
  }
  p.resid = (const bf16*)resid; p.ldres = ldres; p.sRes = sRes;
  hipStream_t s = (hipStream_t)stream;
  const long tiles128 = ((M + 127) / 128) * ((N + 127) / 128) * batch;
  const long tiles256 = ((M + 255) / 256) * ((N + 255) / 256) * batch;
  p.kchunk = K;
  const bool frames = p.a_fs || p.b_fs || p.c_fs;
  SplitPlan pl = split_plan(M, N, K, batch, a_trans, b_trans, c_f32, epi, beta, frames);
  const long pws = split_ws_bytes(pl, M, N, batch);
  bool have_ws = ws && (uintptr_t)ws % 16 == 0 && pws > 0 && ws_bytes >= pws;
  static const int atomic_splitk = getenv("OWLK_GEMM_ATOMIC") ? atoi(getenv("OWLK_GEMM_ATOMIC")) : 0;
  if (pl.opt && (!have_ws || atomic_splitk)) {
    const SplitPlan p128 = split_plan(M, N, K, batch, a_trans, b_trans, c_f32, epi, beta, frames, false);
    const long w128 = split_ws_bytes(p128, M, N, batch);
    const bool ws128 = ws && (uintptr_t)ws % 16 == 0 && w128 > 0 && ws_bytes >= w128;
    pl = (atomic_splitk || ws128) ? p128 : SplitPlan{SPLIT_NONE, 1, K, false};
    have_ws = ws128;
  }
  if (pl.kind == SPLIT_DECODE && (pl.splits == 1 || have_ws)) return launch_decode(p, epi, ws, s);
  {
    const long sk = pl.splits;
    if (pl.kind == SPLIT_SKINNY && have_ws) {
      p.kchunk = pl.kchunk;
      p.ws = (float*)ws;
      if (int e = dispatch_e<64, 64>(p, a_trans, b_trans, epi, c_f32, batch, s)) return e;
      const long work = M * (N / 8);
      const unsigned grid = (unsigned)std::min<long>((work + 255) / 256, 2048);
      switch (epi) {
        case EPI_STORE: hipLaunchKernelGGL(splitk_epi_k<EPI_STORE>, dim3(grid), dim3(256), 0, s, p, (int)sk); break;
        case EPI_SILU: hipLaunchKernelGGL(splitk_epi_k<EPI_SILU>, dim3(grid), dim3(256), 0, s, p, (int)sk); break;
        default: hipLaunchKernelGGL(splitk_epi_k<EPI_GATE_RESID>, dim3(grid), dim3(256), 0, s, p, (int)sk); break;
      }
      return owlk::check_launch("splitk_epi");
    }
  }
  OWLK_REQUIRE(!frames || (fits256(M, N, K, a_trans, b_trans, c_f32, beta) && batch == 1 &&
                           (pl.kind == SPLIT_256 || pl.kind == SPLIT_NONE) &&
                           (pl.kind != SPLIT_256 || (have_ws && !atomic_splitk)) && pl.kchunk % FRAME_ROWS == 0),
               "gemm: frame-strided rows need the 256^2 kernel (M=%ld N=%ld K=%ld)", M, N, K);
  if (frames && pl.kind == SPLIT_NONE) return dispatch256(p, a_trans, b_trans, epi, c_f32, batch, s);
  if (fits256(M, N, K, a_trans, b_trans, c_f32, beta)) {
    const long nsp = pl.kind == SPLIT_256 ? pl.splits : 1;
    if (nsp > 1) {
      p.kchunk = pl.kchunk;
      if (atomic_splitk || !have_ws) {
        if (beta == 0.f)
          OWLK_REQUIRE(hipMemset2DAsync(C, ldc * sizeof(float), 0, N * sizeof(float), M, s) == hipSuccess,
                       "gemm: clearing the split-K output failed");
        return dispatch256(p, a_trans, b_trans, epi, c_f32, batch, s);
      }
      {
        p.ws = (float*)ws;
        if (int e = dispatch256(p, a_trans, b_trans, epi, c_f32, batch, s)) return e;
        const long work = M * (N / 4);
        const unsigned grid = (unsigned)std::min<long>((work + 255) / 256, 2048);
        hipLaunchKernelGGL(splitk_reduce_k, dim3(grid), dim3(256), 0, s, p.ws, (int)nsp, M, N, (float*)C, ldc,
                           alpha, beta);
        return owlk::check_launch("splitk_reduce");
      }
    }
    if (tiles256 >= min_tiles256()) return dispatch256(p, a_trans, b_trans, epi, c_f32, batch, s);
  }
  if (pl.kind == SPLIT_128) {
    p.kchunk = pl.kchunk;
    if (have_ws && !atomic_splitk) {
      p.ws = (float*)ws;
      if (int e = dispatch_e<128, 128>(p, a_trans, b_trans, epi, c_f32, batch, s)) return e;
      const long work = M * (N / 4);
      const unsigned grid = (unsigned)std::min<long>((work + 255) / 256, 2048);
      hipLaunchKernelGGL(splitk_reduce_k, dim3(grid), dim3(256), 0, s, p.ws, (int)pl.splits, M, N, (float*)C, ldc,
                         alpha, beta);
      return owlk::check_launch("splitk_reduce");
    }
    if (beta == 0.f) {
      OWLK_REQUIRE(hipMemset2DAsync(C, ldc * sizeof(float), 0, N * sizeof(float), M, s) == hipSuccess,
                   "gemm: clearing the split-K output failed");
      p.beta = 1.f;
    }
    return dispatch_e<128, 128>(p, a_trans, b_trans, epi, c_f32, batch, s);
  }
  if (tiles128 < 512) return dispatch_e<64, 64>(p, a_trans, b_trans, epi, c_f32, batch, s);
  return dispatch_e<128, 128>(p, a_trans, b_trans, epi, c_f32, batch, s);
}

extern "C" int owlk_colsum(const void* x, int x_f32, long R, long N, long ld, float* out, void* ws, long ws_bytes,
                           void* stream);
extern "C" long owlk_colsum_ws_bytes(long R, long N);

static long fused_colsum_bytes(long M, long N) { return ((M + 255) / 256) * 2 * N * (long)sizeof(float); }

extern "C" int owlk_gemm(long M, long N, long K, long batch,
                         const void* A, long lda, long sA, int a_trans,
                         const void* B, long ldb, long sB, int b_trans,
                         void* C, long ldc, long sC, int c_f32,
                         int epi, float alpha, float beta, const float* bias,
                         void* aux, long ldaux, long sAux,
                         const void* gate, long ldgate, long sGate, long tpf,
                         const void* resid, long ldres, long sRes,
                         float* colsum, void* ws, long ws_bytes, void* stream) {
  OWLK_REQUIRE(!colsum || (batch == 1 && !c_f32), "gemm: colsum needs batch 1 and a bf16 output");
  GemmP p{};
  p.colsum_req = colsum;
  if (colsum && ws && (uintptr_t)ws % 16 == 0 && ws_bytes >= fused_colsum_bytes(M, N)) p.cs_part = (float*)ws;
  if (int e = gemm_dispatch(p, M, N, K, batch, A, lda, sA, a_trans, B, ldb, sB, b_trans, C, ldc, sC, c_f32, epi,
                            alpha, beta, bias, aux, ldaux, sAux, gate, ldgate, sGate, tpf, resid, ldres, sRes, ws,
                            ws_bytes, stream))
    return e;
  if (colsum && p.colsum && p.cs_part)
    return owlk::colsum_reduce(p.cs_part, (int)(((M + 255) / 256) * 2), N, colsum, (hipStream_t)stream);
  if (colsum && !p.colsum)
    return owlk_colsum(C, 0, M, N, ldc, colsum, ws, ws_bytes, stream);
  return 0;
}

extern "C" int owlk_attn_delta(const void* o, const void* dout, long ld, long B, long L, int H, int D, float* delta,
                               void* stream);

extern "C" int owlk_gemm_attn_delta(long M, long N, long K, const void* dY, long lddy, const void* W, long ldw,
                                    void* dO, long ldc, const void* o, long ldo, long L, int H, int D,
                                    float* delta, void* stream) {
  OWLK_REQUIRE(L > 0 && M % L == 0 && H > 0 && D > 0 && N == (long)H * D && o && delta,
               "gemm_attn_delta: bad shape M=%ld N=%ld L=%ld H=%d D=%d", M, N, L, H, D);
  static const int pp = getenv("OWLK_GEMM_PP") ? atoi(getenv("OWLK_GEMM_PP")) : 1;
  static const int fuse_env = getenv("OWLK_GEMM_DELTA") ? atoi(getenv("OWLK_GEMM_DELTA")) : 1;
  const long tiles256 = ((M + 255) / 256) * ((N + 255) / 256);
  const SplitPlan pl = split_plan(M, N, K, 1, 0, 1, 0, EPI_DELTA, 0.f);
  if (fuse_env && pp && D == 64 && fits256(M, N, K, 0, 1, 0, 0.f) && tiles256 >= min_tiles256() &&
      pl.kind == SPLIT_NONE && ldo % 8 == 0 && (uintptr_t)o % 16 == 0) {
    GemmP p{};
    p.delta = delta;
    p.dl = L;
    return gemm_dispatch(p, M, N, K, 1, dY, lddy, 0, 0, W, ldw, 0, 1, dO, ldc, 0, 0, EPI_DELTA, 1.f, 0.f, nullptr,
                         const_cast<void*>(o), ldo, 0, nullptr, 0, 0, 0, nullptr, 0, 0, nullptr, 0, stream);
  }
  OWLK_REQUIRE(ldo == ldc, "gemm_attn_delta: the unfused form needs O and dO with one row stride");
  if (int e = owlk_gemm(M, N, K, 1, dY, lddy, 0, 0, W, ldw, 0, 1, dO, ldc, 0, 0, EPI_STORE, 1.f, 0.f, nullptr,
                        nullptr, 0, 0, nullptr, 0, 0, 0, nullptr, 0, 0, nullptr, nullptr, 0, stream))
    return e;
  return owlk_attn_delta(o, dO, ldc, M / L, L, H, D, delta, stream);
}

extern "C" int owlk_qk_rope_fwd(const void* qkv, long ldq, long T, int H, int D, const float* cosb,
                                const float* sinb, long ld_tab, long n_tab, long tab_off, long tpos_div, void* out,
                                long ldo, float* rstd, void* stream);

extern "C" int owlk_gemm_qk_rope(long M, long N, long K, const void* A, long lda, const void* W, long ldw,
                                 const float* bias, void* qkv, long ldq, int H, int D, const float* cosb,
                                 const float* sinb, long ld_tab, long n_tab, long tab_off, long tpos_div, void* out,
                                 long ldo, float* rstd, void* stream) {
  OWLK_REQUIRE(H > 0 && (D == 64 || D == 128) && N == 3L * H * D && out && cosb && sinb,
               "gemm_qk_rope: bad shape N=%ld H=%d D=%d", N, H, D);
  {
    const long span = tpos_div > 0 ? (M < tpos_div ? M : tpos_div) : M;
    OWLK_REQUIRE(n_tab > 0 && tab_off >= 0 && tab_off + span <= n_tab,
                 "gemm_qk_rope: positions %ld.. past the %ld-row rope table", tab_off, n_tab);
  }
  static const int pp = getenv("OWLK_GEMM_PP") ? atoi(getenv("OWLK_GEMM_PP")) : 1;
  static const int fuse_env = getenv("OWLK_GEMM_ROPE") ? atoi(getenv("OWLK_GEMM_ROPE")) : 1;
  const long tiles256 = ((M + 255) / 256) * ((N + 255) / 256);
  const SplitPlan pl = split_plan(M, N, K, 1, 0, 0, 0, EPI_QKROPE, 0.f);
  if (fuse_env && pp && D == 64 && fits256(M, N, K, 0, 0, 0, 0.f) && tiles256 >= min_tiles256() &&
      pl.kind == SPLIT_NONE && ldo % 8 == 0 && ld_tab % 4 == 0 && (uintptr_t)out % 16 == 0 &&
      (uintptr_t)cosb % 16 == 0 && (uintptr_t)sinb % 16 == 0) {
    GemmP p{};
    p.rcos = cosb;
    p.rsin = sinb;
    p.ld_tab = ld_tab;
    p.tab_off = tab_off;
    p.tpos_div = tpos_div;
    p.rstd = rstd;
    p.qk_cols = 2L * H * D;
    return gemm_dispatch(p, M, N, K, 1, A, lda, 0, 0, W, ldw, 0, 0, qkv, ldq, 0, 0, EPI_QKROPE, 1.f, 0.f, bias, out,
                         ldo, 0, nullptr, 0, 0, 0, nullptr, 0, 0, nullptr, 0, stream);
  }
  if (int e = owlk_gemm(M, N, K, 1, A, lda, 0, 0, W, ldw, 0, 0, qkv, ldq, 0, 0, EPI_STORE, 1.f, 0.f, bias, nullptr,
                        0, 0, nullptr, 0, 0, 0, nullptr, 0, 0, nullptr, nullptr, 0, stream))
    return e;
  return owlk_qk_rope_fwd(qkv, ldq, M, H, D, cosb, sinb, ld_tab, n_tab, tab_off, tpos_div, out, ldo, rstd, stream);
}

extern "C" int owlk_gemm_frames(long M, long N, long K, const void* A, long lda, long a_fs, int a_trans,
                                const void* B, long ldb, long b_fs, int b_trans, void* C, long ldc, long c_fs,
                                int c_f32, int epi, float alpha, float beta, const float* bias, void* aux, long ldaux,
                                const void* gate, long ldgate, long tpf, const void* resid, long ldres, void* ws,
                                long ws_bytes, void* stream) {
  OWLK_REQUIRE(a_fs >= 0 && b_fs >= 0 && c_fs >= 0 && a_fs % 8 == 0 && b_fs % 8 == 0 && c_fs % 8 == 0,
               "gemm_frames: frame strides must be non-negative multiples of 8");
  OWLK_REQUIRE(!c_fs || (!c_f32 && epi == EPI_STORE), "gemm_frames: frame-strided C only for a bf16 STORE");
  OWLK_REQUIRE((!a_fs || (a_trans ? K : M) % FRAME_ROWS == 0) && (!b_fs || (b_trans ? K : N) % FRAME_ROWS == 0) &&
                   (!c_fs || M % FRAME_ROWS == 0),
               "gemm_frames: frame-strided dims must be whole frames of %d rows", FRAME_ROWS);
  GemmP p{};
  p.a_fs = a_fs;
  p.b_fs = b_fs;
  p.c_fs = c_fs;
  return gemm_dispatch(p, M, N, K, 1, A, lda, 0, a_trans, B, ldb, 0, b_trans, C, ldc, 0, c_f32, epi, alpha, beta, bias,
                       aux, ldaux, 0, gate, ldgate, 0, tpf, resid, ldres, 0, ws, ws_bytes, stream);
}

extern "C" long owlk_gemm_splitk_bytes(long M, long N, long K, long batch, int a_trans, int b_trans, int c_f32,
                                       int epi, float beta) {
  if (M <= 0 || N <= 0 || K <= 0 || batch <= 0) return 0;
  return split_ws_bytes(split_plan(M, N, K, batch, a_trans, b_trans, c_f32, epi, beta), M, N, batch);
}

extern "C" long owlk_gemm_ws_counter_bytes(long M, long N, long K, long batch, int a_trans, int b_trans, int c_f32,
                                           int epi, float beta) {
  if (M <= 0 || N <= 0 || K <= 0 || batch <= 0) return 0;
  const SplitPlan pl = split_plan(M, N, K, batch, a_trans, b_trans, c_f32, epi, beta);
  return pl.kind == SPLIT_DECODE && pl.splits > 1 ? kDecodeCounterBytes : 0;
}

extern "C" long owlk_gemm_ws_bytes(long M, long N, long K, long batch, int a_trans, int b_trans, int c_f32, int epi,
                                   float beta, int colsum) {
  long b = owlk_gemm_splitk_bytes(M, N, K, batch, a_trans, b_trans, c_f32, epi, beta);
  if (colsum && M > 0 && N > 0) {
    const long c = std::max(fused_colsum_bytes(M, N), owlk_colsum_ws_bytes(M, N));
    b = std::max(b, c);
  }
  return b;
}
```

owl-audio-exps_amd/owl_wms/_lib/__init__.py:

```python
import ctypes
import os

import torch

_HERE = os.path.dirname(os.path.abspath(__file__))
LIB_PATH = os.path.join(_HERE, "libowlk.so")

L, I, F, P = ctypes.c_long, ctypes.c_int, ctypes.c_float, ctypes.c_void_p

_SIGS = {
    "owlk_gemm": [L, L, L, L, P, L, L, I, P, L, L, I, P, L, L, I, I, F, F, P, P, L, L, P, L, L, L, P, L, L, P, P, L,
                  P],
    "owlk_gemm_frames": [L, L, L, P, L, L, I, P, L, L, I, P, L, L, I, I, F, F, P, P, L, P, L, L, P, L, P, L, P],
    "owlk_gemm_splitk_bytes": [L, L, L, L, I, I, I, I, F],
    "owlk_gemm_ws_bytes": [L, L, L, L, I, I, I, I, F, I],
    "owlk_gemm_ws_counter_bytes": [L, L, L, L, I, I, I, I, F],
    "owlk_adaln_fwd": [P, L, P, P, L, L, L, I, P, L, P, P, P],
    "owlk_adaln_bwd": [P, L, P, L, P, P, L, L, L, I, P, L, P, L, P, P, L, P, I, P],
    "owlk_gate_bwd": [P, L, P, L, P, L, L, L, I, P, L, P, L, I, P, L, P],
    "owlk_adaln_gate_bwd": [P, L, P, L, P, P, L, L, L, I, P, L, P, L, P, P, L, I, P, L, P, L, P, L, P, L, I, P, L,
                            P],
    "owlk_cond_embed": [P, I, P, I, F, P, L, P, I, L, P, I, F, P, P, L, P, P, I, L, I, I, P, L, L, P],
    "owlk_cond_silu_fwd": [P, P, P, P, L, L, I, P, P, P],
    "owlk_cond_silu_bwd": [P, I, P, P, L, L, I, P, P, P],
    "owlk_small_k_wgrad": [P, L, P, L, L, L, I, P, L, F, P],
    "owlk_qk_rope_fwd": [P, L, L, I, I, P, P, L, L, L, L, P, L, P, P],
    "owlk_qk_rope_fwd_kv": [P, L, L, L, I, I, P, P, L, L, L, P, L, L, P, L, L, P, L, L, P],
    "owlk_qk_rope_fwd_kv_dev": [P, L, L, L, I, I, P, P, L, L, P, P, L, L, P, L, L, P, L, L, L, P],
    "owlk_attn_decode_fwd": [P, L, L, P, L, L, P, L, L, P, L, L, P, L, I, L, I, F, F, P, L, L, L, P],
    "owlk_mm_qk_rope_fwd_kv": [P, L, P, L, L, L, I, I, I, I, P, P, L, L, L, P, L, L, P, L, L, P, L, L, P],
    "owlk_attn_decode_joint_fwd": [P, L, L, P, L, L, P, L, L, P, L, P, L, P, L, I, I, I, L, I, F, F, P],
    "owlk_qk_rope_bwd": [P, L, P, L, L, I, I, P, P, L, L, L, L, P, P, L, P],
    "owlk_qk_rope_bwd_ws_bytes": [L, I, I],
    "owlk_qk_rope_bwd_bias": [P, L, P, L, L, I, I, P, P, L, L, L, L, P, P, L, P, P, L, P],
    "owlk_attn_fwd": [P, L, L, P, L, L, P, L, L, P, L, L, P, L, I, L, L, I, F, F, L, I, I, L, P, P, P, P, L, P],
    "owlk_attn_delta": [P, P, L, L, L, I, I, P, P],
    "owlk_frame_mux": [I, L, I, I, I, P, L, P, L, P, L, P],
    "owlk_layernorm_fwd": [P, L, L, I, P, L, P, P, P],
    "owlk_layernorm_bwd": [P, L, P, L, P, P, L, I, P, L, P],
    "owlk_attn_bwd": [P, L, L, P, L, L, P, L, L, P, L, L, P, P, P, L, L, P, L, L, P, L, L, L, I, L, L, I, F, L, I, I,
                      P, P, P, P, L, P],
    "owlk_attn_bwd_dkdv": [P, L, L, P, L, L, P, L, L, P, L, L, P, P, P, L, L, P, L, L, P, L, L, L, I, L, L, I, F, L, I,
                           I, P, P, P, P, L, P],
    "owlk_attn_bwd_dq": [P, L, L, P, L, L, P, L, L, P, L, L, P, P, P, L, L, P, L, L, P, L, L, L, I, L, L, I, F, L, I, I,
                         P, P, P, P, L, P],
    "owlk_attn_decode_bwd_ws_bytes": [L, I, L, L, I],
    "owlk_attn_decode_bwd": [P, L, L, P, L, L, P, L, L, P, L, L, P, P, P, L, L, P, L, L, P, L, L, L, I, L, L, L, I, F,
                             P, L, P],
    "owlk_attn_bwd_fused_ws_bytes": [L, I, L, I],
    "owlk_attn_bwd_fused": [P, L, L, P, L, L, P, L, L, P, L, L, P, P, P, L, L, P, L, L, P, L, L, L, I, L, I, F, L, I, I,
                            P, P, P, P, L, P, L, I, P],
    "owlk_set_cu_reserve": [I],
    "owlk_gemm_attn_delta": [L, L, L, P, L, P, L, P, L, P, L, L, I, I, P, P],
    "owlk_gemm_qk_rope": [L, L, L, P, L, P, L, P, P, L, I, I, P, P, L, L, L, L, P, L, P, P],
    "owlk_flow_noise": [P, P, P, I, I, L, P, P, P, P],
    "owlk_unpatchify": [P, I, I, L, P, P],
    "owlk_mse": [P, P, L, F, P, P, I, P, P],
    "owlk_mse_grad": [P, P, L, F, P, P, P],
    "owlk_dmd_loss_ws_bytes": [L, L, L],
    "owlk_dmd_loss": [P, P, I, P, P, P, I, P, P, L, L, L, F, P, P, P, L, P],
    "owlk_critic_loss_ws_bytes": [L],
    "owlk_critic_loss": [P, I, P, P, I, P, L, L, L, F, P, P, P, L, P],
    "owlk_gate_resid": [P, L, P, L, P, L, L, L, I, P, L, P],
    "owlk_colsum_ws_bytes": [L, L],
    "owlk_colsum": [P, I, L, L, L, P, P, L, P],
    "owlk_colsum_frames": [P, I, L, L, L, L, P, P, L, P],
    "owlk_ns_normalize": [P, I, L, L, L, I, P, P, P],
    "owlk_ns_scale": [P, I, L, L, L, I, P, P, P],
    "owlk_ns_iterate_ws_bytes": [L, L, L],
    "owlk_ns_iterate": [P, L, L, L, I, F, F, F, P, L, P],
    "owlk_newton_schulz_ws_bytes": [L, L, L],
    "owlk_newton_schulz_bf16": [P, I, L, L, L, I, F, F, F, P, P, L, P],
    "owlk_muon_momentum": [I, P, P, L, F, I, P, P, P],
    "owlk_muon_apply": [I, P, P, L, L, I, F, F, P],
    "owlk_adamw": [I, P, P, P, P, P, F, F, F, F, F, F, F, P],
    "owlk_ema": [I, P, P, P, F, P],
}

_RESTYPES = {n: ctypes.c_long for n in ("owlk_gemm_splitk_bytes", "owlk_gemm_ws_bytes", "owlk_gemm_ws_counter_bytes",
                                         "owlk_qk_rope_bwd_ws_bytes", "owlk_attn_bwd_fused_ws_bytes",
                                        "owlk_attn_decode_bwd_ws_bytes",
                                        "owlk_dmd_loss_ws_bytes", "owlk_critic_loss_ws_bytes",
                                        "owlk_colsum_ws_bytes", "owlk_ns_iterate_ws_bytes",
                                        "owlk_newton_schulz_ws_bytes")}

_lib = None


def lib():
    global _lib
    if _lib is None:
        path = os.environ.get("OWLK_LIB", LIB_PATH)
        if not os.path.exists(path):
            raise RuntimeError(f"libowlk.so not built at {path}: run `make -C owl-audio-exps_amd/csrc` "
                               "(or __graft_entry__.build()); there is no non-HIP fallback")
        h = ctypes.CDLL(path, mode=ctypes.RTLD_GLOBAL)
        for name, args in _SIGS.items():
            if path != LIB_PATH and not hasattr(h, name):
                continue
            fn = getattr(h, name)
            fn.argtypes = args
            fn.restype = _RESTYPES.get(name, ctypes.c_int)
        h.owlk_last_error.restype = ctypes.c_char_p
        h.owlk_last_error.argtypes = []
        h.owlk_version.restype = ctypes.c_int
        h.owlk_device_ok.restype = ctypes.c_int
        _lib = h
    return _lib


def exported_symbols():
    return ["owlk_last_error", "owlk_version", "owlk_device_ok"] + list(_SIGS)


_profile = None


def profiling():
    return _profile is not None


def profile_begin():
    global _profile
    _profile = []


def profile_end():
    global _profile
    torch.cuda.synchronize()
    out = {}
    for key, flops, e0, e1 in _profile or []:
        n, ms, fl = out.get(key, (0, 0.0, 0.0))
        out[key] = (n + 1, ms + e0.elapsed_time(e1), fl + (flops or 0.0))
    _profile = None
    return out


def call(name, *args, key=None, flops=None):
    prof = _profile
    if prof is not None:
        e0 = torch.cuda.Event(enable_timing=True)
        e0.record()
    rc = getattr(lib(), name)(*args)
    if rc != 0:
        raise RuntimeError(f"{name} failed ({rc}): {lib().owlk_last_error().decode()}")
    if prof is not None:
        e1 = torch.cuda.Event(enable_timing=True)
        e1.record()
        prof.append((key or name, flops() if callable(flops) else flops, e0, e1))


def ptr(t):
    return None if t is None else ctypes.c_void_p(t.data_ptr())


def stream():
    return ctypes.c_void_p(torch.cuda.current_stream().cuda_stream)
```

Baseline: 147,800 latent-tokens/s.

## Add hand-scheduled inline-asm K-loop for ping-pong GEMM and enable by default

Adds a generated inline-assembly K-loop for the 256x256 ping-pong GEMM kernel. It uses a deeper multi-stage LDS ring (160 KB) of global_load_lds DMA buffers, pinned registers, explicit s_setprio and barrier interleaving of MFMA with ds_read, and a rotating unrolled stage schedule. The default OWLK_GEMM_PP becomes 2, so all unsplit ping-pong GEMMs, including the delta and rope epilogues, take the new path, and a runtime setter can override the body and the tile threshold. The aim is to hide memory latency and cut compiler scheduling overhead in the main GEMM loop, at the cost of fragile hard-coded register and LDS assignments.

```diff
diff --git a/include/owlk.h b/include/owlk.h
--- a/include/owlk.h
+++ b/include/owlk.h
@@ -35,6 +35,7 @@
                         float beta, int colsum);
 long owlk_gemm_ws_counter_bytes(long M, long N, long K, long batch, int a_trans, int b_trans, int c_f32, int epi,
                                 float beta);
+int owlk_set_gemm_pp(int body, long min_tiles);
 
 int owlk_adaln_fwd(const void* x, long ldx, const void* scale, const void* shift, long ldm, long tpf,
                    long T, int d, void* y, long ldy, float* rstd, void* yact , void* stream);
diff --git a/owl-audio-exps_amd/csrc/gemm.hip b/owl-audio-exps_amd/csrc/gemm.hip
--- a/owl-audio-exps_amd/csrc/gemm.hip
+++ b/owl-audio-exps_amd/csrc/gemm.hip
@@ -698,11 +698,39 @@
   }
 }
 
-template <bool AT, bool BT, int EPI, bool OF32, int FS = 0>
+#include "gemm_pp_step.inc"
+
+template <bool TRANS>
+DEV unsigned ppa_dma_off(long ld, long rel0, long lim, int wave, int lane, int i) {
+  if (!TRANS) {
+    const int row = (wave * 2 + i) * 8 + (lane >> 3);
+    const int ch = (lane & 7) ^ ((row >> 1) & 7);
+    long rel = rel0 + row;
+    rel = rel < lim ? rel : lim;
+    return (unsigned)(rel * ld * 2 + ch * 16);
+  }
+  const int k = (wave * 2 + i) * 4 + lane / 16;
+  const int pch = lane % 16;
+  const int lch = (((pch >> 1) ^ swz_t<128>(k)) << 1) | (pch & 1);
+  return (unsigned)(((long)k * ld + rel0 + lch * 8) * 2);
+}
+template <bool TRANS>
+DEV unsigned ppa_read_addr(unsigned base, int x, int row0, int lane) {
+  if (!TRANS) {
+    const int r = lane & 15, kc = 4 * x + (lane >> 4);
+    return base + (row0 + r) * 128 + ((kc ^ ((r >> 1) & 7)) << 4);
+  }
+  const int g = lane >> 4, q = (lane & 15) >> 2, pp = lane & 3;
+  const int k0 = 8 * g + q;
+  return base + k0 * 256 + ((x ^ swz_t<128>(k0)) << 5) + pp * 8;
+}
+
+template <bool AT, bool BT, int EPI, bool OF32, int FS = 0, bool ASM = false>
 __global__ __launch_bounds__(NT8, 1) void gemm_pp_kernel(GemmP p) {
   constexpr bool FA = FS & 1, FB = (FS & 2) != 0, FC = (FS & 4) != 0;
   constexpr int HALF = 128 * BK * 2, STAGE = 4 * HALF;
-  __shared__ __attribute__((aligned(16))) char smem[2 * STAGE];
+  static_assert(!ASM || FS == 0, "the generated K-loop reads plain rows");
+  __shared__ __attribute__((aligned(16))) char smem[ASM ? PPA_LDS_BYTES : 2 * STAGE];
   const int lane = threadIdx.x & 63, wave = __builtin_amdgcn_readfirstlane(threadIdx.x >> 6);
   const int wr = wave >> 2, wc = wave & 3;
 
@@ -736,6 +764,46 @@
 #pragma unroll
     for (int j = 0; j < 4; ++j) acc[i][j] = f32x4{0.f, 0.f, 0.f, 0.f};
 
+  if constexpr (ASM) {
+    f32x16 cv[8];
+#pragma unroll
+    for (int i = 0; i < 8; ++i)
+#pragma unroll
+      for (int e = 0; e < 16; ++e) cv[i][e] = 0.f;
+    const unsigned L0 = (unsigned)(uintptr_t)(__attribute__((address_space(3))) char*)smem;
+    PPLane f;
+#pragma unroll
+    for (int h = 0; h < 2; ++h)
+#pragma unroll
+      for (int i = 0; i < 2; ++i) {
+        f.dma[2 * h + i] = ppa_dma_off<BT>(p.ldb, 128 * h, p.N - 1 - n0, wave, lane, i);
+        f.dma[4 + 2 * h + i] = ppa_dma_off<AT>(p.lda, 128 * h, p.M - 1 - m0, wave, lane, i);
+      }
+    const unsigned abase = L0 + PPA_A_PAIR0 + wr * HALF, bbase = L0 + (wc >> 1) * HALF;
+#pragma unroll
+    for (int x = 0; x < 8; ++x) f.ra[x] = ppa_read_addr<AT>(abase, x, 0, lane);
+#pragma unroll
+    for (int x = 0; x < 4; ++x) f.rb[x] = ppa_read_addr<BT>(bbase, BT ? 4 * (wc & 1) + x : x, (wc & 1) * 64, lane);
+    const bf16* ab = AT ? A + kbeg * p.lda + m0 : A + m0 * p.lda + kbeg;
+    const bf16* bb = BT ? B + kbeg * p.ldb + n0 : B + n0 * p.ldb + kbeg;
+    auto sgpr = [](unsigned x) { return (unsigned)__builtin_amdgcn_readfirstlane((int)x); };
+    auto sptr = [&](const bf16* q) {
+      const unsigned long long u = (unsigned long long)q;
+      return (const void*)((unsigned long long)sgpr((unsigned)u) | ((unsigned long long)sgpr((unsigned)(u >> 32)) << 32));
+    };
+    u32x4 sc;
+    sc[0] = sgpr(AT ? (unsigned)(BK * p.lda * 2) : BK * 2);
+    sc[1] = sgpr(BT ? (unsigned)(BK * p.ldb * 2) : BK * 2);
+    sc[2] = sgpr(L0 + (unsigned)(wave * 2048));
+    sc[3] = sgpr((unsigned)wr);
+    gemm_pp_loop<AT, BT>(cv, f, sptr(ab), sptr(bb), sgpr((unsigned)nk), sc);
+#pragma unroll
+    for (int i = 0; i < 8; ++i)
+#pragma unroll
+      for (int j = 0; j < 4; ++j)
+#pragma unroll
+        for (int r = 0; r < 4; ++r) acc[i][j][r] = cv[i][4 * j + r];
+  } else {
   auto issueA = [&](int t) {
     char* st = smem + (t & 1) * STAGE;
     glds_tile<128, AT, FA>(st, A, p.lda, m0, kbeg + (long)t * BK, p.M, wave, lane, p.a_fs);
@@ -820,6 +888,7 @@
   if (wr == 0) OWLK_PP_BAR();
 #undef OWLK_PP_BAR
 #undef OWLK_PP_SYNC
+  }
 #ifdef OWLK_GEMM_EXP_NOEPI
   {
     float t = 0.f;
@@ -1047,13 +1116,20 @@
 }
 
 
+int g_pp_body = -1;
+long g_min_tiles256 = -1;
+int pp_body() {
+  static const int env = getenv("OWLK_GEMM_PP") ? atoi(getenv("OWLK_GEMM_PP")) : 2;
+  return g_pp_body >= 0 ? g_pp_body : env;
+}
+
 template <bool AT, bool BT, int EPI, bool OF32>
 int launch256(GemmP& p, long batch, hipStream_t s) {
   p.tiles_m = (int)((p.M + 255) / 256);
   p.tiles_n = (int)((p.N + 255) / 256);
   const int splits = (int)((p.K + p.kchunk - 1) / p.kchunk);
   dim3 grid(p.tiles_m * p.tiles_n, (unsigned)splits, (unsigned)batch);
-  static const int pp = getenv("OWLK_GEMM_PP") ? atoi(getenv("OWLK_GEMM_PP")) : 1;
+  const int pp = pp_body();
   static const int fuse_cs = getenv("OWLK_GEMM_COLSUM") ? atoi(getenv("OWLK_GEMM_COLSUM")) : 1;
   if (pp && EPI == EPI_DSILU && batch == 1 && fuse_cs) p.colsum = p.colsum_req;
   static const int group_m = getenv("OWLK_GEMM_GROUP") ? atoi(getenv("OWLK_GEMM_GROUP")) : -1;
@@ -1098,7 +1174,12 @@
   }
   if constexpr (EPI == EPI_DELTA || EPI == EPI_QKROPE) {
     OWLK_REQUIRE(pp && splits == 1 && batch == 1, "gemm: the delta / rope epilogues run in the unsplit ping-pong kernel");
-    hipLaunchKernelGGL((gemm_pp_kernel<AT, BT, EPI, OF32>), grid, dim3(NT8), 0, s, p);
+    if (pp >= 2)
+      hipLaunchKernelGGL((gemm_pp_kernel<AT, BT, EPI, OF32, 0, true>), grid, dim3(NT8), 0, s, p);
+    else
+      hipLaunchKernelGGL((gemm_pp_kernel<AT, BT, EPI, OF32>), grid, dim3(NT8), 0, s, p);
+  } else if (pp >= 2) {
+    hipLaunchKernelGGL((gemm_pp_kernel<AT, BT, EPI, OF32, 0, true>), grid, dim3(NT8), 0, s, p);
   } else if (pp) {
     hipLaunchKernelGGL((gemm_pp_kernel<AT, BT, EPI, OF32>), grid, dim3(NT8), 0, s, p);
   } else {
@@ -1372,7 +1453,13 @@
 }
 static long min_tiles256() {
   static const long v = getenv("OWLK_GEMM_MIN256") ? atol(getenv("OWLK_GEMM_MIN256")) : 192;
-  return v;
+  return g_min_tiles256 >= 0 ? g_min_tiles256 : v;
+}
+extern "C" int owlk_set_gemm_pp(int body, long min_tiles) {
+  OWLK_REQUIRE(body >= -1 && body <= 2, "owlk_set_gemm_pp: body %d (0 gemm256, 1 ping-pong, 2 generated loop, -1 default)", body);
+  g_pp_body = body;
+  g_min_tiles256 = min_tiles < 0 ? -1 : min_tiles;
+  return 0;
 }
 static long skinny_splits(long M, long N, long K, long batch, int c_f32, int epi, float beta) {
   if (batch != 1 || c_f32 || M > 256 || K < 512 || K % BK) return 1;
@@ -1614,7 +1701,7 @@
                                     float* delta, void* stream) {
   OWLK_REQUIRE(L > 0 && M % L == 0 && H > 0 && D > 0 && N == (long)H * D && o && delta,
                "gemm_attn_delta: bad shape M=%ld N=%ld L=%ld H=%d D=%d", M, N, L, H, D);
-  static const int pp = getenv("OWLK_GEMM_PP") ? atoi(getenv("OWLK_GEMM_PP")) : 1;
+  const int pp = pp_body();
   static const int fuse_env = getenv("OWLK_GEMM_DELTA") ? atoi(getenv("OWLK_GEMM_DELTA")) : 1;
   const long tiles256 = ((M + 255) / 256) * ((N + 255) / 256);
   const SplitPlan pl = split_plan(M, N, K, 1, 0, 1, 0, EPI_DELTA, 0.f);
@@ -1648,7 +1735,7 @@
     OWLK_REQUIRE(n_tab > 0 && tab_off >= 0 && tab_off + span <= n_tab,
                  "gemm_qk_rope: positions %ld.. past the %ld-row rope table", tab_off, n_tab);
   }
-  static const int pp = getenv("OWLK_GEMM_PP") ? atoi(getenv("OWLK_GEMM_PP")) : 1;
+  const int pp = pp_body();
   static const int fuse_env = getenv("OWLK_GEMM_ROPE") ? atoi(getenv("OWLK_GEMM_ROPE")) : 1;
   const long tiles256 = ((M + 255) / 256) * ((N + 255) / 256);
   const SplitPlan pl = split_plan(M, N, K, 1, 0, 0, 0, EPI_QKROPE, 0.f);
diff --git a/owl-audio-exps_amd/csrc/gemm_pp_step.inc b/owl-audio-exps_amd/csrc/gemm_pp_step.inc
--- /dev/null
+++ b/owl-audio-exps_amd/csrc/gemm_pp_step.inc
@@ -0,0 +1,611 @@
+#pragma once
+
+typedef unsigned int u32x8 __attribute__((ext_vector_type(8)));
+constexpr int PPA_LDS_BYTES = 163840;
+constexpr int PPA_A_PAIR0 = 32768;
+
+struct PPLane {
+  u32x8 dma, ra;
+  u32x4 rb;
+};
+
+template <bool AT, bool BT>
+__attribute__((always_inline)) DEV void gemm_pp_loop(f32x16 (&c)[8], PPLane& f, const void* ab, const void* bb,
+                                                     unsigned nk, u32x4 sc);
+
+#define PPA_DB0_S0 \
+  "s_add_u32 m0, s74, 0\n" "s_nop 0\n" "global_load_lds_dwordx4 v192, s[66:67]\n" "s_add_u32 m0, s74, 1024\n" \
+  "s_nop 0\n" "global_load_lds_dwordx4 v193, s[66:67]\n"
+#define PPA_DB1_S1 \
+  "s_add_u32 m0, s74, 16384\n" "s_nop 0\n" "global_load_lds_dwordx4 v194, s[66:67]\n" "s_add_u32 m0, s74, 17408\n" \
+  "s_nop 0\n" "global_load_lds_dwordx4 v195, s[66:67]\n"
+#define PPA_DA0_S2 \
+  "s_add_u32 m0, s74, 32768\n" "s_nop 0\n" "global_load_lds_dwordx4 v196, s[64:65]\n" "s_add_u32 m0, s74, 33792\n" \
+  "s_nop 0\n" "global_load_lds_dwordx4 v197, s[64:65]\n"
+#define PPA_DA1_S3 \
+  "s_add_u32 m0, s74, 49152\n" "s_nop 0\n" "global_load_lds_dwordx4 v198, s[64:65]\n" "s_add_u32 m0, s74, 50176\n" \
+  "s_nop 0\n" "global_load_lds_dwordx4 v199, s[64:65]\n"
+#define PPA_DB0_S4 \
+  "s_add_u32 m0, s74, 65536\n" "s_nop 0\n" "global_load_lds_dwordx4 v192, s[66:67]\n" "s_add_u32 m0, s74, 66560\n" \
+  "s_nop 0\n" "global_load_lds_dwordx4 v193, s[66:67]\n"
+#define PPA_DB1_S5 \
+  "s_add_u32 m0, s74, 81920\n" "s_nop 0\n" "global_load_lds_dwordx4 v194, s[66:67]\n" "s_add_u32 m0, s74, 82944\n" \
+  "s_nop 0\n" "global_load_lds_dwordx4 v195, s[66:67]\n"
+#define PPA_DA0_S6 \
+  "s_add_u32 m0, s74, 98304\n" "s_nop 0\n" "global_load_lds_dwordx4 v196, s[64:65]\n" "s_add_u32 m0, s74, 99328\n" \
+  "s_nop 0\n" "global_load_lds_dwordx4 v197, s[64:65]\n"
+#define PPA_R0 \
+  "ds_read_b128 v[160:163], v208 offset:0\n" "ds_read_b128 v[168:171], v208 offset:2048\n" \
+  "ds_read_b128 v[128:131], v200 offset:0\n" "ds_read_b128 v[136:139], v200 offset:2048\n" \
+  "ds_read_b128 v[144:147], v200 offset:4096\n" "ds_read_b128 v[152:155], v200 offset:6144\n" \
+  "ds_read_b128 v[164:167], v209 offset:0\n" "ds_read_b128 v[172:175], v209 offset:2048\n" \
+  "ds_read_b128 v[132:135], v201 offset:0\n" "ds_read_b128 v[140:143], v201 offset:2048\n" \
+  "ds_read_b128 v[148:151], v201 offset:4096\n" "ds_read_b128 v[156:159], v201 offset:6144\n"
+#define PPA_DA1_S7 \
+  "s_add_u32 m0, s74, 114688\n" "s_nop 0\n" "global_load_lds_dwordx4 v198, s[64:65]\n" "s_add_u32 m0, s74, 115712\n" \
+  "s_nop 0\n" "global_load_lds_dwordx4 v199, s[64:65]\n"
+#define PPA_M0A \
+  "s_barrier\n" "s_waitcnt lgkmcnt(6)\n" "s_setprio 1\n" \
+  "v_mfma_f32_16x16x32_bf16 v[0:3], v[128:131], v[160:163], v[0:3]\n" \
+  "v_mfma_f32_16x16x32_bf16 v[4:7], v[128:131], v[168:171], v[4:7]\n"
+#define PPA_M0B \
+  "v_mfma_f32_16x16x32_bf16 v[16:19], v[136:139], v[160:163], v[16:19]\n" \
+  "v_mfma_f32_16x16x32_bf16 v[20:23], v[136:139], v[168:171], v[20:23]\n" \
+  "v_mfma_f32_16x16x32_bf16 v[32:35], v[144:147], v[160:163], v[32:35]\n" \
+  "v_mfma_f32_16x16x32_bf16 v[36:39], v[144:147], v[168:171], v[36:39]\n" \
+  "v_mfma_f32_16x16x32_bf16 v[48:51], v[152:155], v[160:163], v[48:51]\n" \
+  "v_mfma_f32_16x16x32_bf16 v[52:55], v[152:155], v[168:171], v[52:55]\n" "s_waitcnt lgkmcnt(0)\n" \
+  "v_mfma_f32_16x16x32_bf16 v[0:3], v[132:135], v[164:167], v[0:3]\n" \
+  "v_mfma_f32_16x16x32_bf16 v[4:7], v[132:135], v[172:175], v[4:7]\n" \
+  "v_mfma_f32_16x16x32_bf16 v[16:19], v[140:143], v[164:167], v[16:19]\n" \
+  "v_mfma_f32_16x16x32_bf16 v[20:23], v[140:143], v[172:175], v[20:23]\n" \
+  "v_mfma_f32_16x16x32_bf16 v[32:35], v[148:151], v[164:167], v[32:35]\n" \
+  "v_mfma_f32_16x16x32_bf16 v[36:39], v[148:151], v[172:175], v[36:39]\n" \
+  "v_mfma_f32_16x16x32_bf16 v[48:51], v[156:159], v[164:167], v[48:51]\n" \
+  "v_mfma_f32_16x16x32_bf16 v[52:55], v[156:159], v[172:175], v[52:55]\n" "s_setprio 0\n" "s_barrier\n"
+#define PPA_R1 \
+  "ds_read_b128 v[176:179], v208 offset:4096\n" "ds_read_b128 v[184:187], v208 offset:6144\n" \
+  "ds_read_b128 v[180:183], v209 offset:4096\n" "ds_read_b128 v[188:191], v209 offset:6144\n"
+#define PPA_DB0_S8 \
+  "s_add_u32 m0, s74, 131072\n" "s_nop 0\n" "global_load_lds_dwordx4 v192, s[66:67]\n" "s_add_u32 m0, s74, 132096\n" \
+  "s_nop 0\n" "global_load_lds_dwordx4 v193, s[66:67]\n"
+#define PPA_M1A \
+  "s_barrier\n" "s_waitcnt lgkmcnt(2)\n" "s_setprio 1\n" \
+  "v_mfma_f32_16x16x32_bf16 v[8:11], v[128:131], v[176:179], v[8:11]\n" \
+  "v_mfma_f32_16x16x32_bf16 v[12:15], v[128:131], v[184:187], v[12:15]\n"
+#define PPA_M1B \
+  "v_mfma_f32_16x16x32_bf16 v[24:27], v[136:139], v[176:179], v[24:27]\n" \
+  "v_mfma_f32_16x16x32_bf16 v[28:31], v[136:139], v[184:187], v[28:31]\n" \
+  "v_mfma_f32_16x16x32_bf16 v[40:43], v[144:147], v[176:179], v[40:43]\n" \
+  "v_mfma_f32_16x16x32_bf16 v[44:47], v[144:147], v[184:187], v[44:47]\n" \
+  "v_mfma_f32_16x16x32_bf16 v[56:59], v[152:155], v[176:179], v[56:59]\n" \
+  "v_mfma_f32_16x16x32_bf16 v[60:63], v[152:155], v[184:187], v[60:63]\n" "s_waitcnt lgkmcnt(0)\n" \
+  "v_mfma_f32_16x16x32_bf16 v[8:11], v[132:135], v[180:183], v[8:11]\n" \
+  "v_mfma_f32_16x16x32_bf16 v[12:15], v[132:135], v[188:191], v[12:15]\n" \
+  "v_mfma_f32_16x16x32_bf16 v[24:27], v[140:143], v[180:183], v[24:27]\n" \
+  "v_mfma_f32_16x16x32_bf16 v[28:31], v[140:143], v[188:191], v[28:31]\n" \
+  "v_mfma_f32_16x16x32_bf16 v[40:43], v[148:151], v[180:183], v[40:43]\n" \
+  "v_mfma_f32_16x16x32_bf16 v[44:47], v[148:151], v[188:191], v[44:47]\n" \
+  "v_mfma_f32_16x16x32_bf16 v[56:59], v[156:159], v[180:183], v[56:59]\n" \
+  "v_mfma_f32_16x16x32_bf16 v[60:63], v[156:159], v[188:191], v[60:63]\n" "s_setprio 0\n" "s_barrier\n"
+#define PPA_R2 \
+  "ds_read_b128 v[128:131], v200 offset:8192\n" "ds_read_b128 v[136:139], v200 offset:10240\n" \
+  "ds_read_b128 v[144:147], v200 offset:12288\n" "ds_read_b128 v[152:155], v200 offset:14336\n" \
+  "ds_read_b128 v[132:135], v201 offset:8192\n" "ds_read_b128 v[140:143], v201 offset:10240\n" "s_nop 0\n" \
+  "ds_read_b128 v[148:151], v201 offset:12288\n" "s_nop 0\n" "ds_read_b128 v[156:159], v201 offset:14336\n"
+#define PPA_DB1_S9 \
+  "s_add_u32 m0, s74, 147456\n" "s_nop 0\n" "global_load_lds_dwordx4 v194, s[66:67]\n" "s_add_u32 m0, s74, 148480\n" \
+  "s_nop 0\n" "global_load_lds_dwordx4 v195, s[66:67]\n"
+#define PPA_M2A \
+  "s_barrier\n" "s_waitcnt lgkmcnt(4)\n" "s_setprio 1\n" \
+  "v_mfma_f32_16x16x32_bf16 v[72:75], v[128:131], v[176:179], v[72:75]\n" \
+  "v_mfma_f32_16x16x32_bf16 v[76:79], v[128:131], v[184:187], v[76:79]\n"
+#define PPA_VB_P4 \
+  "v_add_u32 v208, 0x10000, v208\n" "v_add_u32 v209, 0x10000, v209\n"
+#define PPA_M2B \
+  "v_mfma_f32_16x16x32_bf16 v[88:91], v[136:139], v[176:179], v[88:91]\n" \
+  "v_mfma_f32_16x16x32_bf16 v[92:95], v[136:139], v[184:187], v[92:95]\n" \
+  "v_mfma_f32_16x16x32_bf16 v[104:107], v[144:147], v[176:179], v[104:107]\n" \
+  "v_mfma_f32_16x16x32_bf16 v[108:111], v[144:147], v[184:187], v[108:111]\n" \
+  "v_mfma_f32_16x16x32_bf16 v[120:123], v[152:155], v[176:179], v[120:123]\n" \
+  "v_mfma_f32_16x16x32_bf16 v[124:127], v[152:155], v[184:187], v[124:127]\n" "s_waitcnt lgkmcnt(0)\n" \
+  "v_mfma_f32_16x16x32_bf16 v[72:75], v[132:135], v[180:183], v[72:75]\n" \
+  "v_mfma_f32_16x16x32_bf16 v[76:79], v[132:135], v[188:191], v[76:79]\n" \
+  "v_mfma_f32_16x16x32_bf16 v[88:91], v[140:143], v[180:183], v[88:91]\n" \
+  "v_mfma_f32_16x16x32_bf16 v[92:95], v[140:143], v[188:191], v[92:95]\n" \
+  "v_mfma_f32_16x16x32_bf16 v[104:107], v[148:151], v[180:183], v[104:107]\n" \
+  "v_mfma_f32_16x16x32_bf16 v[108:111], v[148:151], v[188:191], v[108:111]\n" \
+  "v_mfma_f32_16x16x32_bf16 v[120:123], v[156:159], v[180:183], v[120:123]\n" \
+  "v_mfma_f32_16x16x32_bf16 v[124:127], v[156:159], v[188:191], v[124:127]\n" "s_setprio 0\n" "s_barrier\n"
+#define PPA_DA0_S0 \
+  "s_add_u32 m0, s74, 0\n" "s_nop 0\n" "global_load_lds_dwordx4 v196, s[64:65]\n" "s_add_u32 m0, s74, 1024\n" \
+  "s_nop 0\n" "global_load_lds_dwordx4 v197, s[64:65]\n"
+#define PPA_M3A \
+  "s_barrier\n" "s_setprio 1\n" "v_mfma_f32_16x16x32_bf16 v[64:67], v[128:131], v[160:163], v[64:67]\n" \
+  "v_mfma_f32_16x16x32_bf16 v[68:71], v[128:131], v[168:171], v[68:71]\n"
+#define PPA_VA_P4 \
+  "v_add_u32 v200, 0x10000, v200\n" "v_add_u32 v201, 0x10000, v201\n"
+#define PPA_M3B \
+  "v_mfma_f32_16x16x32_bf16 v[80:83], v[136:139], v[160:163], v[80:83]\n" \
+  "v_mfma_f32_16x16x32_bf16 v[84:87], v[136:139], v[168:171], v[84:87]\n" \
+  "v_mfma_f32_16x16x32_bf16 v[96:99], v[144:147], v[160:163], v[96:99]\n" \
+  "v_mfma_f32_16x16x32_bf16 v[100:103], v[144:147], v[168:171], v[100:103]\n" \
+  "v_mfma_f32_16x16x32_bf16 v[112:115], v[152:155], v[160:163], v[112:115]\n" \
+  "v_mfma_f32_16x16x32_bf16 v[116:119], v[152:155], v[168:171], v[116:119]\n" \
+  "v_mfma_f32_16x16x32_bf16 v[64:67], v[132:135], v[164:167], v[64:67]\n" \
+  "v_mfma_f32_16x16x32_bf16 v[68:71], v[132:135], v[172:175], v[68:71]\n" \
+  "v_mfma_f32_16x16x32_bf16 v[80:83], v[140:143], v[164:167], v[80:83]\n" \
+  "v_mfma_f32_16x16x32_bf16 v[84:87], v[140:143], v[172:175], v[84:87]\n" \
+  "v_mfma_f32_16x16x32_bf16 v[96:99], v[148:151], v[164:167], v[96:99]\n" \
+  "v_mfma_f32_16x16x32_bf16 v[100:103], v[148:151], v[172:175], v[100:103]\n" \
+  "v_mfma_f32_16x16x32_bf16 v[112:115], v[156:159], v[164:167], v[112:115]\n" \
+  "v_mfma_f32_16x16x32_bf16 v[116:119], v[156:159], v[172:175], v[116:119]\n" "s_setprio 0\n" "s_barrier\n"
+#define PPA_DA1_S1 \
+  "s_add_u32 m0, s74, 16384\n" "s_nop 0\n" "global_load_lds_dwordx4 v198, s[64:65]\n" "s_add_u32 m0, s74, 17408\n" \
+  "s_nop 0\n" "global_load_lds_dwordx4 v199, s[64:65]\n"
+#define PPA_DB0_S2 \
+  "s_add_u32 m0, s74, 32768\n" "s_nop 0\n" "global_load_lds_dwordx4 v192, s[66:67]\n" "s_add_u32 m0, s74, 33792\n" \
+  "s_nop 0\n" "global_load_lds_dwordx4 v193, s[66:67]\n"
+#define PPA_DB1_S3 \
+  "s_add_u32 m0, s74, 49152\n" "s_nop 0\n" "global_load_lds_dwordx4 v194, s[66:67]\n" "s_add_u32 m0, s74, 50176\n" \
+  "s_nop 0\n" "global_load_lds_dwordx4 v195, s[66:67]\n"
+#define PPA_DA0_S4 \
+  "s_add_u32 m0, s74, 65536\n" "s_nop 0\n" "global_load_lds_dwordx4 v196, s[64:65]\n" "s_add_u32 m0, s74, 66560\n" \
+  "s_nop 0\n" "global_load_lds_dwordx4 v197, s[64:65]\n"
+#define PPA_VA_M6 \
+  "v_add_u32 v200, 0xfffe8000, v200\n" "v_add_u32 v201, 0xfffe8000, v201\n"
+#define PPA_DA1_S5 \
+  "s_add_u32 m0, s74, 81920\n" "s_nop 0\n" "global_load_lds_dwordx4 v198, s[64:65]\n" "s_add_u32 m0, s74, 82944\n" \
+  "s_nop 0\n" "global_load_lds_dwordx4 v199, s[64:65]\n"
+#define PPA_DB0_S6 \
+  "s_add_u32 m0, s74, 98304\n" "s_nop 0\n" "global_load_lds_dwordx4 v192, s[66:67]\n" "s_add_u32 m0, s74, 99328\n" \
+  "s_nop 0\n" "global_load_lds_dwordx4 v193, s[66:67]\n"
+#define PPA_DB1_S7 \
+  "s_add_u32 m0, s74, 114688\n" "s_nop 0\n" "global_load_lds_dwordx4 v194, s[66:67]\n" "s_add_u32 m0, s74, 115712\n" \
+  "s_nop 0\n" "global_load_lds_dwordx4 v195, s[66:67]\n"
+#define PPA_VB_M6 \
+  "v_add_u32 v208, 0xfffe8000, v208\n" "v_add_u32 v209, 0xfffe8000, v209\n"
+#define PPA_DA0_S8 \
+  "s_add_u32 m0, s74, 131072\n" "s_nop 0\n" "global_load_lds_dwordx4 v196, s[64:65]\n" "s_add_u32 m0, s74, 132096\n" \
+  "s_nop 0\n" "global_load_lds_dwordx4 v197, s[64:65]\n"
+#define PPA_DA1_S9 \
+  "s_add_u32 m0, s74, 147456\n" "s_nop 0\n" "global_load_lds_dwordx4 v198, s[64:65]\n" "s_add_u32 m0, s74, 148480\n" \
+  "s_nop 0\n" "global_load_lds_dwordx4 v199, s[64:65]\n"
+#define PPA_R0_2 \
+  "ds_read_b128 v[160:163], v208 offset:0\n" "ds_read_b128 v[168:171], v208 offset:2048\n" \
+  "ds_read_b128 v[128:131], v200 offset:0\n" "ds_read_b128 v[136:139], v200 offset:2048\n" \
+  "ds_read_b128 v[144:147], v200 offset:4096\n" "ds_read_b128 v[152:155], v200 offset:6144\n" "s_nop 0\n" \
+  "ds_read_b128 v[164:167], v209 offset:0\n" "ds_read_b128 v[172:175], v209 offset:2048\n" \
+  "ds_read_b128 v[132:135], v201 offset:0\n" "ds_read_b128 v[140:143], v201 offset:2048\n" \
+  "ds_read_b128 v[148:151], v201 offset:4096\n" "ds_read_b128 v[156:159], v201 offset:6144\n"
+#define PPA_R0_3 \
+  "ds_read_b64_tr_b16 v[160:161], v208 offset:0\n" "ds_read_b64_tr_b16 v[162:163], v208 offset:1024\n" \
+  "ds_read_b64_tr_b16 v[168:169], v209 offset:0\n" "ds_read_b64_tr_b16 v[170:171], v209 offset:1024\n" \
+  "ds_read_b128 v[128:131], v200 offset:0\n" "ds_read_b128 v[136:139], v200 offset:2048\n" \
+  "ds_read_b128 v[144:147], v200 offset:4096\n" "ds_read_b128 v[152:155], v200 offset:6144\n" \
+  "ds_read_b64_tr_b16 v[164:165], v208 offset:8192\n" "ds_read_b64_tr_b16 v[166:167], v208 offset:9216\n" \
+  "ds_read_b64_tr_b16 v[172:173], v209 offset:8192\n" "ds_read_b64_tr_b16 v[174:175], v209 offset:9216\n" \
+  "ds_read_b128 v[132:135], v201 offset:0\n" "ds_read_b128 v[140:143], v201 offset:2048\n" \
+  "ds_read_b128 v[148:151], v201 offset:4096\n" "ds_read_b128 v[156:159], v201 offset:6144\n"
+#define PPA_M0A_2 \
+  "s_barrier\n" "s_waitcnt lgkmcnt(8)\n" "s_setprio 1\n" \
+  "v_mfma_f32_16x16x32_bf16 v[0:3], v[128:131], v[160:163], v[0:3]\n" \
+  "v_mfma_f32_16x16x32_bf16 v[4:7], v[128:131], v[168:171], v[4:7]\n"
+#define PPA_R1_2 \
+  "ds_read_b64_tr_b16 v[176:177], v210 offset:0\n" "ds_read_b64_tr_b16 v[178:179], v210 offset:1024\n" \
+  "ds_read_b64_tr_b16 v[184:185], v211 offset:0\n" "ds_read_b64_tr_b16 v[186:187], v211 offset:1024\n" \
+  "ds_read_b64_tr_b16 v[180:181], v210 offset:8192\n" "ds_read_b64_tr_b16 v[182:183], v210 offset:9216\n" \
+  "ds_read_b64_tr_b16 v[188:189], v211 offset:8192\n" "ds_read_b64_tr_b16 v[190:191], v211 offset:9216\n"
+#define PPA_M1A_2 \
+  "s_barrier\n" "s_waitcnt lgkmcnt(4)\n" "s_setprio 1\n" \
+  "v_mfma_f32_16x16x32_bf16 v[8:11], v[128:131], v[176:179], v[8:11]\n" \
+  "v_mfma_f32_16x16x32_bf16 v[12:15], v[128:131], v[184:187], v[12:15]\n"
+#define PPA_VB_P4_2 \
+  "v_add_u32 v208, 0x10000, v208\n" "v_add_u32 v209, 0x10000, v209\n" "v_add_u32 v210, 0x10000, v210\n" \
+  "v_add_u32 v211, 0x10000, v211\n"
+#define PPA_VB_M6_2 \
+  "v_add_u32 v208, 0xfffe8000, v208\n" "v_add_u32 v209, 0xfffe8000, v209\n" "v_add_u32 v210, 0xfffe8000, v210\n" \
+  "v_add_u32 v211, 0xfffe8000, v211\n"
+#define PPA_R0_4 \
+  "ds_read_b128 v[160:163], v208 offset:0\n" "ds_read_b128 v[168:171], v208 offset:2048\n" \
+  "ds_read_b64_tr_b16 v[128:129], v200 offset:0\n" "ds_read_b64_tr_b16 v[130:131], v200 offset:1024\n" \
+  "ds_read_b64_tr_b16 v[136:137], v201 offset:0\n" "ds_read_b64_tr_b16 v[138:139], v201 offset:1024\n" \
+  "ds_read_b64_tr_b16 v[144:145], v202 offset:0\n" "ds_read_b64_tr_b16 v[146:147], v202 offset:1024\n" \
+  "ds_read_b64_tr_b16 v[152:153], v203 offset:0\n" "ds_read_b64_tr_b16 v[154:155], v203 offset:1024\n" \
+  "ds_read_b128 v[164:167], v209 offset:0\n" "ds_read_b128 v[172:175], v209 offset:2048\n" \
+  "ds_read_b64_tr_b16 v[132:133], v200 offset:8192\n" "ds_read_b64_tr_b16 v[134:135], v200 offset:9216\n" \
+  "ds_read_b64_tr_b16 v[140:141], v201 offset:8192\n" "ds_read_b64_tr_b16 v[142:143], v201 offset:9216\n" \
+  "ds_read_b64_tr_b16 v[148:149], v202 offset:8192\n" "ds_read_b64_tr_b16 v[150:151], v202 offset:9216\n" \
+  "ds_read_b64_tr_b16 v[156:157], v203 offset:8192\n" "ds_read_b64_tr_b16 v[158:159], v203 offset:9216\n"
+#define PPA_M0A_3 \
+  "s_barrier\n" "s_waitcnt lgkmcnt(10)\n" "s_setprio 1\n" \
+  "v_mfma_f32_16x16x32_bf16 v[0:3], v[128:131], v[160:163], v[0:3]\n" \
+  "v_mfma_f32_16x16x32_bf16 v[4:7], v[128:131], v[168:171], v[4:7]\n"
+#define PPA_R2_2 \
+  "ds_read_b64_tr_b16 v[128:129], v204 offset:0\n" "ds_read_b64_tr_b16 v[130:131], v204 offset:1024\n" \
+  "ds_read_b64_tr_b16 v[136:137], v205 offset:0\n" "ds_read_b64_tr_b16 v[138:139], v205 offset:1024\n" \
+  "ds_read_b64_tr_b16 v[144:145], v206 offset:0\n" "ds_read_b64_tr_b16 v[146:147], v206 offset:1024\n" \
+  "ds_read_b64_tr_b16 v[152:153], v207 offset:0\n" "ds_read_b64_tr_b16 v[154:155], v207 offset:1024\n" \
+  "ds_read_b64_tr_b16 v[132:133], v204 offset:8192\n" "ds_read_b64_tr_b16 v[134:135], v204 offset:9216\n" \
+  "ds_read_b64_tr_b16 v[140:141], v205 offset:8192\n" "ds_read_b64_tr_b16 v[142:143], v205 offset:9216\n" \
+  "ds_read_b64_tr_b16 v[148:149], v206 offset:8192\n" "ds_read_b64_tr_b16 v[150:151], v206 offset:9216\n" \
+  "ds_read_b64_tr_b16 v[156:157], v207 offset:8192\n" "ds_read_b64_tr_b16 v[158:159], v207 offset:9216\n"
+#define PPA_M2A_2 \
+  "s_barrier\n" "s_waitcnt lgkmcnt(8)\n" "s_setprio 1\n" \
+  "v_mfma_f32_16x16x32_bf16 v[72:75], v[128:131], v[176:179], v[72:75]\n" \
+  "v_mfma_f32_16x16x32_bf16 v[76:79], v[128:131], v[184:187], v[76:79]\n"
+#define PPA_VA_P4_2 \
+  "v_add_u32 v200, 0x10000, v200\n" "v_add_u32 v201, 0x10000, v201\n" "v_add_u32 v202, 0x10000, v202\n" \
+  "v_add_u32 v203, 0x10000, v203\n" "v_add_u32 v204, 0x10000, v204\n" "v_add_u32 v205, 0x10000, v205\n" \
+  "v_add_u32 v206, 0x10000, v206\n" "v_add_u32 v207, 0x10000, v207\n"
+#define PPA_VA_M6_2 \
+  "v_add_u32 v200, 0xfffe8000, v200\n" "v_add_u32 v201, 0xfffe8000, v201\n" "v_add_u32 v202, 0xfffe8000, v202\n" \
+  "v_add_u32 v203, 0xfffe8000, v203\n" "v_add_u32 v204, 0xfffe8000, v204\n" "v_add_u32 v205, 0xfffe8000, v205\n" \
+  "v_add_u32 v206, 0xfffe8000, v206\n" "v_add_u32 v207, 0xfffe8000, v207\n"
+#define PPA_R0_5 \
+  "ds_read_b64_tr_b16 v[160:161], v208 offset:0\n" "ds_read_b64_tr_b16 v[162:163], v208 offset:1024\n" \
+  "ds_read_b64_tr_b16 v[168:169], v209 offset:0\n" "ds_read_b64_tr_b16 v[170:171], v209 offset:1024\n" \
+  "ds_read_b64_tr_b16 v[128:129], v200 offset:0\n" "ds_read_b64_tr_b16 v[130:131], v200 offset:1024\n" \
+  "ds_read_b64_tr_b16 v[136:137], v201 offset:0\n" "ds_read_b64_tr_b16 v[138:139], v201 offset:1024\n" \
+  "ds_read_b64_tr_b16 v[144:145], v202 offset:0\n" "ds_read_b64_tr_b16 v[146:147], v202 offset:1024\n" \
+  "ds_read_b64_tr_b16 v[152:153], v203 offset:0\n" "ds_read_b64_tr_b16 v[154:155], v203 offset:1024\n" \
+  "ds_read_b64_tr_b16 v[164:165], v208 offset:8192\n" "ds_read_b64_tr_b16 v[166:167], v208 offset:9216\n" \
+  "ds_read_b64_tr_b16 v[172:173], v209 offset:8192\n" "ds_read_b64_tr_b16 v[174:175], v209 offset:9216\n" \
+  "ds_read_b64_tr_b16 v[132:133], v200 offset:8192\n" "ds_read_b64_tr_b16 v[134:135], v200 offset:9216\n" \
+  "ds_read_b64_tr_b16 v[140:141], v201 offset:8192\n" "ds_read_b64_tr_b16 v[142:143], v201 offset:9216\n" \
+  "ds_read_b64_tr_b16 v[148:149], v202 offset:8192\n" "ds_read_b64_tr_b16 v[150:151], v202 offset:9216\n" \
+  "ds_read_b64_tr_b16 v[156:157], v203 offset:8192\n" "ds_read_b64_tr_b16 v[158:159], v203 offset:9216\n"
+#define PPA_M0A_4 \
+  "s_barrier\n" "s_waitcnt lgkmcnt(12)\n" "s_setprio 1\n" \
+  "v_mfma_f32_16x16x32_bf16 v[0:3], v[128:131], v[160:163], v[0:3]\n" \
+  "v_mfma_f32_16x16x32_bf16 v[4:7], v[128:131], v[168:171], v[4:7]\n"
+
+template <>
+__attribute__((always_inline)) DEV void gemm_pp_loop<false, false>(f32x16 (&c)[8], PPLane& f, const void* ab, const void* bb,
+                                                                  unsigned nk, u32x4 sc) {
+  asm volatile(
+      PPA_DB0_S0 PPA_DB1_S1 "s_add_u32 s66, s66, s73\n" "s_addc_u32 s67, s67, 0\n" PPA_DA0_S2 PPA_DA1_S3
+      "s_add_u32 s64, s64, s72\n" "s_addc_u32 s65, s65, 0\n" "s_cmp_lt_u32 s68, 2\n"
+      "s_cbranch_scc1 .Lpp_p1%=\n"
+      PPA_DB0_S4 PPA_DB1_S5 "s_add_u32 s66, s66, s73\n" "s_addc_u32 s67, s67, 0\n" PPA_DA0_S6 "s_waitcnt vmcnt(6)\n"
+      "s_branch .Lpp_p2%=\n"
+      ".Lpp_p1%=:\n" "s_waitcnt vmcnt(0)\n"
+      ".Lpp_p2%=:\n" "s_barrier\n" "s_cmp_eq_u32 s75, 1\n"
+      "s_cbranch_scc0 .Lpp_g0%=\n"
+      "s_barrier\n"
+      ".Lpp_g0%=:\n"
+      ".Lpp_r0%=:\n" "s_cmp_lt_u32 s68, 3\n"
+      "s_cbranch_scc1 .Lpp_t0%=\n"
+      PPA_R0 PPA_DA1_S7 PPA_M0A PPA_M0B PPA_R1 PPA_DB0_S8 PPA_M1A PPA_M1B PPA_R2 PPA_DB1_S9
+      "s_add_u32 s66, s66, s73\n" "s_addc_u32 s67, s67, 0\n" PPA_M2A PPA_VB_P4 PPA_M2B "s_add_u32 s64, s64, s72\n"
+      "s_addc_u32 s65, s65, 0\n" PPA_DA0_S0 "s_waitcnt vmcnt(6)\n" PPA_M3A PPA_VA_P4 PPA_M3B "s_sub_u32 s68, s68, 1\n"
+      ".Lpp_r1%=:\n" "s_cmp_lt_u32 s68, 3\n"
+      "s_cbranch_scc1 .Lpp_t1%=\n"
+      PPA_R0 PPA_DA1_S1 PPA_M0A PPA_M0B PPA_R1 PPA_DB0_S2 PPA_M1A PPA_M1B PPA_R2 PPA_DB1_S3
+      "s_add_u32 s66, s66, s73\n" "s_addc_u32 s67, s67, 0\n" PPA_M2A PPA_VB_P4 PPA_M2B "s_add_u32 s64, s64, s72\n"
+      "s_addc_u32 s65, s65, 0\n" PPA_DA0_S4 "s_waitcnt vmcnt(6)\n" PPA_M3A PPA_VA_M6 PPA_M3B "s_sub_u32 s68, s68, 1\n"
+      ".Lpp_r2%=:\n" "s_cmp_lt_u32 s68, 3\n"
+      "s_cbranch_scc1 .Lpp_t2%=\n"
+      PPA_R0 PPA_DA1_S5 PPA_M0A PPA_M0B PPA_R1 PPA_DB0_S6 PPA_M1A PPA_M1B PPA_R2 PPA_DB1_S7
+      "s_add_u32 s66, s66, s73\n" "s_addc_u32 s67, s67, 0\n" PPA_M2A PPA_VB_M6 PPA_M2B "s_add_u32 s64, s64, s72\n"
+      "s_addc_u32 s65, s65, 0\n" PPA_DA0_S8 "s_waitcnt vmcnt(6)\n" PPA_M3A PPA_VA_P4 PPA_M3B "s_sub_u32 s68, s68, 1\n"
+      ".Lpp_r3%=:\n" "s_cmp_lt_u32 s68, 3\n"
+      "s_cbranch_scc1 .Lpp_t3%=\n"
+      PPA_R0 PPA_DA1_S9 PPA_M0A PPA_M0B PPA_R1 PPA_DB0_S0 PPA_M1A PPA_M1B PPA_R2 PPA_DB1_S1
+      "s_add_u32 s66, s66, s73\n" "s_addc_u32 s67, s67, 0\n" PPA_M2A PPA_VB_P4 PPA_M2B "s_add_u32 s64, s64, s72\n"
+      "s_addc_u32 s65, s65, 0\n" PPA_DA0_S2 "s_waitcnt vmcnt(6)\n" PPA_M3A PPA_VA_P4 PPA_M3B "s_sub_u32 s68, s68, 1\n"
+      ".Lpp_r4%=:\n" "s_cmp_lt_u32 s68, 3\n"
+      "s_cbranch_scc1 .Lpp_t4%=\n"
+      PPA_R0 PPA_DA1_S3 PPA_M0A PPA_M0B PPA_R1 PPA_DB0_S4 PPA_M1A PPA_M1B PPA_R2 PPA_DB1_S5
+      "s_add_u32 s66, s66, s73\n" "s_addc_u32 s67, s67, 0\n" PPA_M2A PPA_VB_M6 PPA_M2B "s_add_u32 s64, s64, s72\n"
+      "s_addc_u32 s65, s65, 0\n" PPA_DA0_S6 "s_waitcnt vmcnt(6)\n" PPA_M3A PPA_VA_M6 PPA_M3B "s_sub_u32 s68, s68, 1\n"
+      "s_branch .Lpp_r0%=\n"
+      ".Lpp_t0%=:\n" "s_cmp_lt_u32 s68, 2\n"
+      "s_cbranch_scc1 .Lpp_l0%=\n"
+      PPA_R0 PPA_DA1_S7 PPA_M0A PPA_M0B PPA_R1 PPA_M1A PPA_M1B PPA_R2 PPA_M2A PPA_VB_P4 PPA_M2B "s_waitcnt vmcnt(0)\n"
+      PPA_M3A PPA_VA_P4 PPA_M3B
+      "s_branch .Lpp_l1%=\n"
+      ".Lpp_t1%=:\n" "s_cmp_lt_u32 s68, 2\n"
+      "s_cbranch_scc1 .Lpp_l1%=\n"
+      PPA_R0 PPA_DA1_S1 PPA_M0A PPA_M0B PPA_R1 PPA_M1A PPA_M1B PPA_R2 PPA_M2A PPA_VB_P4 PPA_M2B "s_waitcnt vmcnt(0)\n"
+      PPA_M3A PPA_VA_M6 PPA_M3B
+      "s_branch .Lpp_l2%=\n"
+      ".Lpp_t2%=:\n" "s_cmp_lt_u32 s68, 2\n"
+      "s_cbranch_scc1 .Lpp_l2%=\n"
+      PPA_R0 PPA_DA1_S5 PPA_M0A PPA_M0B PPA_R1 PPA_M1A PPA_M1B PPA_R2 PPA_M2A PPA_VB_M6 PPA_M2B "s_waitcnt vmcnt(0)\n"
+      PPA_M3A PPA_VA_P4 PPA_M3B
+      "s_branch .Lpp_l3%=\n"
+      ".Lpp_t3%=:\n" "s_cmp_lt_u32 s68, 2\n"
+      "s_cbranch_scc1 .Lpp_l3%=\n"
+      PPA_R0 PPA_DA1_S9 PPA_M0A PPA_M0B PPA_R1 PPA_M1A PPA_M1B PPA_R2 PPA_M2A PPA_VB_P4 PPA_M2B "s_waitcnt vmcnt(0)\n"
+      PPA_M3A PPA_VA_P4 PPA_M3B
+      "s_branch .Lpp_l4%=\n"
+      ".Lpp_t4%=:\n" "s_cmp_lt_u32 s68, 2\n"
+      "s_cbranch_scc1 .Lpp_l4%=\n"
+      PPA_R0 PPA_DA1_S3 PPA_M0A PPA_M0B PPA_R1 PPA_M1A PPA_M1B PPA_R2 PPA_M2A PPA_VB_M6 PPA_M2B "s_waitcnt vmcnt(0)\n"
+      PPA_M3A PPA_VA_M6 PPA_M3B
+      "s_branch .Lpp_l0%=\n"
+      ".Lpp_l0%=:\n" PPA_R0_2 PPA_M0A PPA_M0B PPA_R1 PPA_M1A PPA_M1B PPA_R2 PPA_M2A PPA_M2B PPA_M3A PPA_M3B
+      "s_branch .Lpp_end%=\n"
+      ".Lpp_l1%=:\n" PPA_R0_2 PPA_M0A PPA_M0B PPA_R1 PPA_M1A PPA_M1B PPA_R2 PPA_M2A PPA_M2B PPA_M3A PPA_M3B
+      "s_branch .Lpp_end%=\n"
+      ".Lpp_l2%=:\n" PPA_R0_2 PPA_M0A PPA_M0B PPA_R1 PPA_M1A PPA_M1B PPA_R2 PPA_M2A PPA_M2B PPA_M3A PPA_M3B
+      "s_branch .Lpp_end%=\n"
+      ".Lpp_l3%=:\n" PPA_R0_2 PPA_M0A PPA_M0B PPA_R1 PPA_M1A PPA_M1B PPA_R2 PPA_M2A PPA_M2B PPA_M3A PPA_M3B
+      "s_branch .Lpp_end%=\n"
+      ".Lpp_l4%=:\n" PPA_R0_2 PPA_M0A PPA_M0B PPA_R1 PPA_M1A PPA_M1B PPA_R2 PPA_M2A PPA_M2B PPA_M3A PPA_M3B
+      "s_branch .Lpp_end%=\n"
+      ".Lpp_end%=:\n" "s_cmp_eq_u32 s75, 0\n"
+      "s_cbranch_scc0 .Lpp_g1%=\n"
+      "s_barrier\n"
+      ".Lpp_g1%=:\n" "s_nop 7\n" "s_nop 7\n"
+      : "+{v[0:15]}"(c[0]), "+{v[16:31]}"(c[1]), "+{v[32:47]}"(c[2]), "+{v[48:63]}"(c[3]), "+{v[64:79]}"(c[4]), "+{v[80:95]}"(c[5]), "+{v[96:111]}"(c[6]), "+{v[112:127]}"(c[7]),
+        "+{v[200:207]}"(f.ra), "+{v[208:211]}"(f.rb), "+{s[64:65]}"(ab), "+{s[66:67]}"(bb), "+{s68}"(nk)
+      : "{v[192:199]}"(f.dma), "{s[72:75]}"(sc)
+      : "memory", "m0", "scc", "v128", "v129", "v130", "v131", "v132", "v133", "v134", "v135", "v136", "v137", "v138", "v139", "v140", "v141", "v142", "v143", "v144", "v145", "v146", "v147", "v148", "v149", "v150", "v151", "v152", "v153", "v154", "v155", "v156", "v157", "v158", "v159", "v160", "v161", "v162", "v163", "v164", "v165", "v166", "v167", "v168", "v169", "v170", "v171", "v172", "v173", "v174", "v175", "v176", "v177", "v178", "v179", "v180", "v181", "v182", "v183", "v184", "v185", "v186", "v187", "v188", "v189", "v190", "v191");
+}
+
+template <>
+__attribute__((always_inline)) DEV void gemm_pp_loop<false, true>(f32x16 (&c)[8], PPLane& f, const void* ab, const void* bb,
+                                                                  unsigned nk, u32x4 sc) {
+  asm volatile(
+      PPA_DB0_S0 PPA_DB1_S1 "s_add_u32 s66, s66, s73\n" "s_addc_u32 s67, s67, 0\n" PPA_DA0_S2 PPA_DA1_S3
+      "s_add_u32 s64, s64, s72\n" "s_addc_u32 s65, s65, 0\n" "s_cmp_lt_u32 s68, 2\n"
+      "s_cbranch_scc1 .Lpp_p1%=\n"
+      PPA_DB0_S4 PPA_DB1_S5 "s_add_u32 s66, s66, s73\n" "s_addc_u32 s67, s67, 0\n" PPA_DA0_S6 "s_waitcnt vmcnt(6)\n"
+      "s_branch .Lpp_p2%=\n"
+      ".Lpp_p1%=:\n" "s_waitcnt vmcnt(0)\n"
+      ".Lpp_p2%=:\n" "s_barrier\n" "s_cmp_eq_u32 s75, 1\n"
+      "s_cbranch_scc0 .Lpp_g0%=\n"
+      "s_barrier\n"
+      ".Lpp_g0%=:\n"
+      ".Lpp_r0%=:\n" "s_cmp_lt_u32 s68, 3\n"
+      "s_cbranch_scc1 .Lpp_t0%=\n"
+      PPA_R0_3 PPA_DA1_S7 PPA_M0A_2 PPA_M0B PPA_R1_2 PPA_DB0_S8 PPA_M1A_2 PPA_M1B PPA_R2 PPA_DB1_S9
+      "s_add_u32 s66, s66, s73\n" "s_addc_u32 s67, s67, 0\n" PPA_M2A PPA_VB_P4_2 PPA_M2B "s_add_u32 s64, s64, s72\n"
+      "s_addc_u32 s65, s65, 0\n" PPA_DA0_S0 "s_waitcnt vmcnt(6)\n" PPA_M3A PPA_VA_P4 PPA_M3B "s_sub_u32 s68, s68, 1\n"
+      ".Lpp_r1%=:\n" "s_cmp_lt_u32 s68, 3\n"
+      "s_cbranch_scc1 .Lpp_t1%=\n"
+      PPA_R0_3 PPA_DA1_S1 PPA_M0A_2 PPA_M0B PPA_R1_2 PPA_DB0_S2 PPA_M1A_2 PPA_M1B PPA_R2 PPA_DB1_S3
+      "s_add_u32 s66, s66, s73\n" "s_addc_u32 s67, s67, 0\n" PPA_M2A PPA_VB_P4_2 PPA_M2B "s_add_u32 s64, s64, s72\n"
+      "s_addc_u32 s65, s65, 0\n" PPA_DA0_S4 "s_waitcnt vmcnt(6)\n" PPA_M3A PPA_VA_M6 PPA_M3B "s_sub_u32 s68, s68, 1\n"
+      ".Lpp_r2%=:\n" "s_cmp_lt_u32 s68, 3\n"
+      "s_cbranch_scc1 .Lpp_t2%=\n"
+      PPA_R0_3 PPA_DA1_S5 PPA_M0A_2 PPA_M0B PPA_R1_2 PPA_DB0_S6 PPA_M1A_2 PPA_M1B PPA_R2 PPA_DB1_S7
+      "s_add_u32 s66, s66, s73\n" "s_addc_u32 s67, s67, 0\n" PPA_M2A PPA_VB_M6_2 PPA_M2B "s_add_u32 s64, s64, s72\n"
+      "s_addc_u32 s65, s65, 0\n" PPA_DA0_S8 "s_waitcnt vmcnt(6)\n" PPA_M3A PPA_VA_P4 PPA_M3B "s_sub_u32 s68, s68, 1\n"
+      ".Lpp_r3%=:\n" "s_cmp_lt_u32 s68, 3\n"
+      "s_cbranch_scc1 .Lpp_t3%=\n"
+      PPA_R0_3 PPA_DA1_S9 PPA_M0A_2 PPA_M0B PPA_R1_2 PPA_DB0_S0 PPA_M1A_2 PPA_M1B PPA_R2 PPA_DB1_S1
+      "s_add_u32 s66, s66, s73\n" "s_addc_u32 s67, s67, 0\n" PPA_M2A PPA_VB_P4_2 PPA_M2B "s_add_u32 s64, s64, s72\n"
+      "s_addc_u32 s65, s65, 0\n" PPA_DA0_S2 "s_waitcnt vmcnt(6)\n" PPA_M3A PPA_VA_P4 PPA_M3B "s_sub_u32 s68, s68, 1\n"
+      ".Lpp_r4%=:\n" "s_cmp_lt_u32 s68, 3\n"
+      "s_cbranch_scc1 .Lpp_t4%=\n"
+      PPA_R0_3 PPA_DA1_S3 PPA_M0A_2 PPA_M0B PPA_R1_2 PPA_DB0_S4 PPA_M1A_2 PPA_M1B PPA_R2 PPA_DB1_S5
+      "s_add_u32 s66, s66, s73\n" "s_addc_u32 s67, s67, 0\n" PPA_M2A PPA_VB_M6_2 PPA_M2B "s_add_u32 s64, s64, s72\n"
+      "s_addc_u32 s65, s65, 0\n" PPA_DA0_S6 "s_waitcnt vmcnt(6)\n" PPA_M3A PPA_VA_M6 PPA_M3B "s_sub_u32 s68, s68, 1\n"
+      "s_branch .Lpp_r0%=\n"
+      ".Lpp_t0%=:\n" "s_cmp_lt_u32 s68, 2\n"
+      "s_cbranch_scc1 .Lpp_l0%=\n"
+      PPA_R0_3 PPA_DA1_S7 PPA_M0A_2 PPA_M0B PPA_R1_2 PPA_M1A_2 PPA_M1B PPA_R2 PPA_M2A PPA_VB_P4_2 PPA_M2B
+      "s_waitcnt vmcnt(0)\n" PPA_M3A PPA_VA_P4 PPA_M3B
+      "s_branch .Lpp_l1%=\n"
+      ".Lpp_t1%=:\n" "s_cmp_lt_u32 s68, 2\n"
+      "s_cbranch_scc1 .Lpp_l1%=\n"
+      PPA_R0_3 PPA_DA1_S1 PPA_M0A_2 PPA_M0B PPA_R1_2 PPA_M1A_2 PPA_M1B PPA_R2 PPA_M2A PPA_VB_P4_2 PPA_M2B
+      "s_waitcnt vmcnt(0)\n" PPA_M3A PPA_VA_M6 PPA_M3B
+      "s_branch .Lpp_l2%=\n"
+      ".Lpp_t2%=:\n" "s_cmp_lt_u32 s68, 2\n"
+      "s_cbranch_scc1 .Lpp_l2%=\n"
+      PPA_R0_3 PPA_DA1_S5 PPA_M0A_2 PPA_M0B PPA_R1_2 PPA_M1A_2 PPA_M1B PPA_R2 PPA_M2A PPA_VB_M6_2 PPA_M2B
+      "s_waitcnt vmcnt(0)\n" PPA_M3A PPA_VA_P4 PPA_M3B
+      "s_branch .Lpp_l3%=\n"
+      ".Lpp_t3%=:\n" "s_cmp_lt_u32 s68, 2\n"
+      "s_cbranch_scc1 .Lpp_l3%=\n"
+      PPA_R0_3 PPA_DA1_S9 PPA_M0A_2 PPA_M0B PPA_R1_2 PPA_M1A_2 PPA_M1B PPA_R2 PPA_M2A PPA_VB_P4_2 PPA_M2B
+      "s_waitcnt vmcnt(0)\n" PPA_M3A PPA_VA_P4 PPA_M3B
+      "s_branch .Lpp_l4%=\n"
+      ".Lpp_t4%=:\n" "s_cmp_lt_u32 s68, 2\n"
+      "s_cbranch_scc1 .Lpp_l4%=\n"
+      PPA_R0_3 PPA_DA1_S3 PPA_M0A_2 PPA_M0B PPA_R1_2 PPA_M1A_2 PPA_M1B PPA_R2 PPA_M2A PPA_VB_M6_2 PPA_M2B
+      "s_waitcnt vmcnt(0)\n" PPA_M3A PPA_VA_M6 PPA_M3B
+      "s_branch .Lpp_l0%=\n"
+      ".Lpp_l0%=:\n" PPA_R0_3 PPA_M0A_2 PPA_M0B PPA_R1_2 PPA_M1A_2 PPA_M1B PPA_R2 PPA_M2A PPA_M2B PPA_M3A PPA_M3B
+      "s_branch .Lpp_end%=\n"
+      ".Lpp_l1%=:\n" PPA_R0_3 PPA_M0A_2 PPA_M0B PPA_R1_2 PPA_M1A_2 PPA_M1B PPA_R2 PPA_M2A PPA_M2B PPA_M3A PPA_M3B
+      "s_branch .Lpp_end%=\n"
+      ".Lpp_l2%=:\n" PPA_R0_3 PPA_M0A_2 PPA_M0B PPA_R1_2 PPA_M1A_2 PPA_M1B PPA_R2 PPA_M2A PPA_M2B PPA_M3A PPA_M3B
+      "s_branch .Lpp_end%=\n"
+      ".Lpp_l3%=:\n" PPA_R0_3 PPA_M0A_2 PPA_M0B PPA_R1_2 PPA_M1A_2 PPA_M1B PPA_R2 PPA_M2A PPA_M2B PPA_M3A PPA_M3B
+      "s_branch .Lpp_end%=\n"
+      ".Lpp_l4%=:\n" PPA_R0_3 PPA_M0A_2 PPA_M0B PPA_R1_2 PPA_M1A_2 PPA_M1B PPA_R2 PPA_M2A PPA_M2B PPA_M3A PPA_M3B
+      "s_branch .Lpp_end%=\n"
+      ".Lpp_end%=:\n" "s_cmp_eq_u32 s75, 0\n"
+      "s_cbranch_scc0 .Lpp_g1%=\n"
+      "s_barrier\n"
+      ".Lpp_g1%=:\n" "s_nop 7\n" "s_nop 7\n"
+      : "+{v[0:15]}"(c[0]), "+{v[16:31]}"(c[1]), "+{v[32:47]}"(c[2]), "+{v[48:63]}"(c[3]), "+{v[64:79]}"(c[4]), "+{v[80:95]}"(c[5]), "+{v[96:111]}"(c[6]), "+{v[112:127]}"(c[7]),
+        "+{v[200:207]}"(f.ra), "+{v[208:211]}"(f.rb), "+{s[64:65]}"(ab), "+{s[66:67]}"(bb), "+{s68}"(nk)
+      : "{v[192:199]}"(f.dma), "{s[72:75]}"(sc)
+      : "memory", "m0", "scc", "v128", "v129", "v130", "v131", "v132", "v133", "v134", "v135", "v136", "v137", "v138", "v139", "v140", "v141", "v142", "v143", "v144", "v145", "v146", "v147", "v148", "v149", "v150", "v151", "v152", "v153", "v154", "v155", "v156", "v157", "v158", "v159", "v160", "v161", "v162", "v163", "v164", "v165", "v166", "v167", "v168", "v169", "v170", "v171", "v172", "v173", "v174", "v175", "v176", "v177", "v178", "v179", "v180", "v181", "v182", "v183", "v184", "v185", "v186", "v187", "v188", "v189", "v190", "v191");
+}
+
+template <>
+__attribute__((always_inline)) DEV void gemm_pp_loop<true, false>(f32x16 (&c)[8], PPLane& f, const void* ab, const void* bb,
+                                                                  unsigned nk, u32x4 sc) {
+  asm volatile(
+      PPA_DB0_S0 PPA_DB1_S1 "s_add_u32 s66, s66, s73\n" "s_addc_u32 s67, s67, 0\n" PPA_DA0_S2 PPA_DA1_S3
+      "s_add_u32 s64, s64, s72\n" "s_addc_u32 s65, s65, 0\n" "s_cmp_lt_u32 s68, 2\n"
+      "s_cbranch_scc1 .Lpp_p1%=\n"
+      PPA_DB0_S4 PPA_DB1_S5 "s_add_u32 s66, s66, s73\n" "s_addc_u32 s67, s67, 0\n" PPA_DA0_S6 "s_waitcnt vmcnt(6)\n"
+      "s_branch .Lpp_p2%=\n"
+      ".Lpp_p1%=:\n" "s_waitcnt vmcnt(0)\n"
+      ".Lpp_p2%=:\n" "s_barrier\n" "s_cmp_eq_u32 s75, 1\n"
+      "s_cbranch_scc0 .Lpp_g0%=\n"
+      "s_barrier\n"
+      ".Lpp_g0%=:\n"
+      ".Lpp_r0%=:\n" "s_cmp_lt_u32 s68, 3\n"
+      "s_cbranch_scc1 .Lpp_t0%=\n"
+      PPA_R0_4 PPA_DA1_S7 PPA_M0A_3 PPA_M0B PPA_R1 PPA_DB0_S8 PPA_M1A PPA_M1B PPA_R2_2 PPA_DB1_S9
+      "s_add_u32 s66, s66, s73\n" "s_addc_u32 s67, s67, 0\n" PPA_M2A_2 PPA_VB_P4 PPA_M2B "s_add_u32 s64, s64, s72\n"
+      "s_addc_u32 s65, s65, 0\n" PPA_DA0_S0 "s_waitcnt vmcnt(6)\n" PPA_M3A PPA_VA_P4_2 PPA_M3B
+      "s_sub_u32 s68, s68, 1\n"
+      ".Lpp_r1%=:\n" "s_cmp_lt_u32 s68, 3\n"
+      "s_cbranch_scc1 .Lpp_t1%=\n"
+      PPA_R0_4 PPA_DA1_S1 PPA_M0A_3 PPA_M0B PPA_R1 PPA_DB0_S2 PPA_M1A PPA_M1B PPA_R2_2 PPA_DB1_S3
+      "s_add_u32 s66, s66, s73\n" "s_addc_u32 s67, s67, 0\n" PPA_M2A_2 PPA_VB_P4 PPA_M2B "s_add_u32 s64, s64, s72\n"
+      "s_addc_u32 s65, s65, 0\n" PPA_DA0_S4 "s_waitcnt vmcnt(6)\n" PPA_M3A PPA_VA_M6_2 PPA_M3B
+      "s_sub_u32 s68, s68, 1\n"
+      ".Lpp_r2%=:\n" "s_cmp_lt_u32 s68, 3\n"
+      "s_cbranch_scc1 .Lpp_t2%=\n"
+      PPA_R0_4 PPA_DA1_S5 PPA_M0A_3 PPA_M0B PPA_R1 PPA_DB0_S6 PPA_M1A PPA_M1B PPA_R2_2 PPA_DB1_S7
+      "s_add_u32 s66, s66, s73\n" "s_addc_u32 s67, s67, 0\n" PPA_M2A_2 PPA_VB_M6 PPA_M2B "s_add_u32 s64, s64, s72\n"
+      "s_addc_u32 s65, s65, 0\n" PPA_DA0_S8 "s_waitcnt vmcnt(6)\n" PPA_M3A PPA_VA_P4_2 PPA_M3B
+      "s_sub_u32 s68, s68, 1\n"
+      ".Lpp_r3%=:\n" "s_cmp_lt_u32 s68, 3\n"
+      "s_cbranch_scc1 .Lpp_t3%=\n"
+      PPA_R0_4 PPA_DA1_S9 PPA_M0A_3 PPA_M0B PPA_R1 PPA_DB0_S0 PPA_M1A PPA_M1B PPA_R2_2 PPA_DB1_S1
+      "s_add_u32 s66, s66, s73\n" "s_addc_u32 s67, s67, 0\n" PPA_M2A_2 PPA_VB_P4 PPA_M2B "s_add_u32 s64, s64, s72\n"
+      "s_addc_u32 s65, s65, 0\n" PPA_DA0_S2 "s_waitcnt vmcnt(6)\n" PPA_M3A PPA_VA_P4_2 PPA_M3B
+      "s_sub_u32 s68, s68, 1\n"
+      ".Lpp_r4%=:\n" "s_cmp_lt_u32 s68, 3\n"
+      "s_cbranch_scc1 .Lpp_t4%=\n"
+      PPA_R0_4 PPA_DA1_S3 PPA_M0A_3 PPA_M0B PPA_R1 PPA_DB0_S4 PPA_M1A PPA_M1B PPA_R2_2 PPA_DB1_S5
+      "s_add_u32 s66, s66, s73\n" "s_addc_u32 s67, s67, 0\n" PPA_M2A_2 PPA_VB_M6 PPA_M2B "s_add_u32 s64, s64, s72\n"
+      "s_addc_u32 s65, s65, 0\n" PPA_DA0_S6 "s_waitcnt vmcnt(6)\n" PPA_M3A PPA_VA_M6_2 PPA_M3B
+      "s_sub_u32 s68, s68, 1\n"
+      "s_branch .Lpp_r0%=\n"
+      ".Lpp_t0%=:\n" "s_cmp_lt_u32 s68, 2\n"
+      "s_cbranch_scc1 .Lpp_l0%=\n"
+      PPA_R0_4 PPA_DA1_S7 PPA_M0A_3 PPA_M0B PPA_R1 PPA_M1A PPA_M1B PPA_R2_2 PPA_M2A_2 PPA_VB_P4 PPA_M2B
+      "s_waitcnt vmcnt(0)\n" PPA_M3A PPA_VA_P4_2 PPA_M3B
+      "s_branch .Lpp_l1%=\n"
+      ".Lpp_t1%=:\n" "s_cmp_lt_u32 s68, 2\n"
+      "s_cbranch_scc1 .Lpp_l1%=\n"
+      PPA_R0_4 PPA_DA1_S1 PPA_M0A_3 PPA_M0B PPA_R1 PPA_M1A PPA_M1B PPA_R2_2 PPA_M2A_2 PPA_VB_P4 PPA_M2B
+      "s_waitcnt vmcnt(0)\n" PPA_M3A PPA_VA_M6_2 PPA_M3B
+      "s_branch .Lpp_l2%=\n"
+      ".Lpp_t2%=:\n" "s_cmp_lt_u32 s68, 2\n"
+      "s_cbranch_scc1 .Lpp_l2%=\n"
+      PPA_R0_4 PPA_DA1_S5 PPA_M0A_3 PPA_M0B PPA_R1 PPA_M1A PPA_M1B PPA_R2_2 PPA_M2A_2 PPA_VB_M6 PPA_M2B
+      "s_waitcnt vmcnt(0)\n" PPA_M3A PPA_VA_P4_2 PPA_M3B
+      "s_branch .Lpp_l3%=\n"
+      ".Lpp_t3%=:\n" "s_cmp_lt_u32 s68, 2\n"
+      "s_cbranch_scc1 .Lpp_l3%=\n"
+      PPA_R0_4 PPA_DA1_S9 PPA_M0A_3 PPA_M0B PPA_R1 PPA_M1A PPA_M1B PPA_R2_2 PPA_M2A_2 PPA_VB_P4 PPA_M2B
+      "s_waitcnt vmcnt(0)\n" PPA_M3A PPA_VA_P4_2 PPA_M3B
+      "s_branch .Lpp_l4%=\n"
+      ".Lpp_t4%=:\n" "s_cmp_lt_u32 s68, 2\n"
+      "s_cbranch_scc1 .Lpp_l4%=\n"
+      PPA_R0_4 PPA_DA1_S3 PPA_M0A_3 PPA_M0B PPA_R1 PPA_M1A PPA_M1B PPA_R2_2 PPA_M2A_2 PPA_VB_M6 PPA_M2B
+      "s_waitcnt vmcnt(0)\n" PPA_M3A PPA_VA_M6_2 PPA_M3B
+      "s_branch .Lpp_l0%=\n"
+      ".Lpp_l0%=:\n" PPA_R0_4 PPA_M0A_3 PPA_M0B PPA_R1 PPA_M1A PPA_M1B PPA_R2_2 PPA_M2A_2 PPA_M2B PPA_M3A PPA_M3B
+      "s_branch .Lpp_end%=\n"
+      ".Lpp_l1%=:\n" PPA_R0_4 PPA_M0A_3 PPA_M0B PPA_R1 PPA_M1A PPA_M1B PPA_R2_2 PPA_M2A_2 PPA_M2B PPA_M3A PPA_M3B
+      "s_branch .Lpp_end%=\n"
+      ".Lpp_l2%=:\n" PPA_R0_4 PPA_M0A_3 PPA_M0B PPA_R1 PPA_M1A PPA_M1B PPA_R2_2 PPA_M2A_2 PPA_M2B PPA_M3A PPA_M3B
+      "s_branch .Lpp_end%=\n"
+      ".Lpp_l3%=:\n" PPA_R0_4 PPA_M0A_3 PPA_M0B PPA_R1 PPA_M1A PPA_M1B PPA_R2_2 PPA_M2A_2 PPA_M2B PPA_M3A PPA_M3B
+      "s_branch .Lpp_end%=\n"
+      ".Lpp_l4%=:\n" PPA_R0_4 PPA_M0A_3 PPA_M0B PPA_R1 PPA_M1A PPA_M1B PPA_R2_2 PPA_M2A_2 PPA_M2B PPA_M3A PPA_M3B
+      "s_branch .Lpp_end%=\n"
+      ".Lpp_end%=:\n" "s_cmp_eq_u32 s75, 0\n"
+      "s_cbranch_scc0 .Lpp_g1%=\n"
+      "s_barrier\n"
+      ".Lpp_g1%=:\n" "s_nop 7\n" "s_nop 7\n"
+      : "+{v[0:15]}"(c[0]), "+{v[16:31]}"(c[1]), "+{v[32:47]}"(c[2]), "+{v[48:63]}"(c[3]), "+{v[64:79]}"(c[4]), "+{v[80:95]}"(c[5]), "+{v[96:111]}"(c[6]), "+{v[112:127]}"(c[7]),
+        "+{v[200:207]}"(f.ra), "+{v[208:211]}"(f.rb), "+{s[64:65]}"(ab), "+{s[66:67]}"(bb), "+{s68}"(nk)
+      : "{v[192:199]}"(f.dma), "{s[72:75]}"(sc)
+      : "memory", "m0", "scc", "v128", "v129", "v130", "v131", "v132", "v133", "v134", "v135", "v136", "v137", "v138", "v139", "v140", "v141", "v142", "v143", "v144", "v145", "v146", "v147", "v148", "v149", "v150", "v151", "v152", "v153", "v154", "v155", "v156", "v157", "v158", "v159", "v160", "v161", "v162", "v163", "v164", "v165", "v166", "v167", "v168", "v169", "v170", "v171", "v172", "v173", "v174", "v175", "v176", "v177", "v178", "v179", "v180", "v181", "v182", "v183", "v184", "v185", "v186", "v187", "v188", "v189", "v190", "v191");
+}
+
+template <>
+__attribute__((always_inline)) DEV void gemm_pp_loop<true, true>(f32x16 (&c)[8], PPLane& f, const void* ab, const void* bb,
+                                                                  unsigned nk, u32x4 sc) {
+  asm volatile(
+      PPA_DB0_S0 PPA_DB1_S1 "s_add_u32 s66, s66, s73\n" "s_addc_u32 s67, s67, 0\n" PPA_DA0_S2 PPA_DA1_S3
+      "s_add_u32 s64, s64, s72\n" "s_addc_u32 s65, s65, 0\n" "s_cmp_lt_u32 s68, 2\n"
+      "s_cbranch_scc1 .Lpp_p1%=\n"
+      PPA_DB0_S4 PPA_DB1_S5 "s_add_u32 s66, s66, s73\n" "s_addc_u32 s67, s67, 0\n" PPA_DA0_S6 "s_waitcnt vmcnt(6)\n"
+      "s_branch .Lpp_p2%=\n"
+      ".Lpp_p1%=:\n" "s_waitcnt vmcnt(0)\n"
+      ".Lpp_p2%=:\n" "s_barrier\n" "s_cmp_eq_u32 s75, 1\n"
+      "s_cbranch_scc0 .Lpp_g0%=\n"
+      "s_barrier\n"
+      ".Lpp_g0%=:\n"
+      ".Lpp_r0%=:\n" "s_cmp_lt_u32 s68, 3\n"
+      "s_cbranch_scc1 .Lpp_t0%=\n"
+      PPA_R0_5 PPA_DA1_S7 PPA_M0A_4 PPA_M0B PPA_R1_2 PPA_DB0_S8 PPA_M1A_2 PPA_M1B PPA_R2_2 PPA_DB1_S9
+      "s_add_u32 s66, s66, s73\n" "s_addc_u32 s67, s67, 0\n" PPA_M2A_2 PPA_VB_P4_2 PPA_M2B "s_add_u32 s64, s64, s72\n"
+      "s_addc_u32 s65, s65, 0\n" PPA_DA0_S0 "s_waitcnt vmcnt(6)\n" PPA_M3A PPA_VA_P4_2 PPA_M3B
+      "s_sub_u32 s68, s68, 1\n"
+      ".Lpp_r1%=:\n" "s_cmp_lt_u32 s68, 3\n"
+      "s_cbranch_scc1 .Lpp_t1%=\n"
+      PPA_R0_5 PPA_DA1_S1 PPA_M0A_4 PPA_M0B PPA_R1_2 PPA_DB0_S2 PPA_M1A_2 PPA_M1B PPA_R2_2 PPA_DB1_S3
+      "s_add_u32 s66, s66, s73\n" "s_addc_u32 s67, s67, 0\n" PPA_M2A_2 PPA_VB_P4_2 PPA_M2B "s_add_u32 s64, s64, s72\n"
+      "s_addc_u32 s65, s65, 0\n" PPA_DA0_S4 "s_waitcnt vmcnt(6)\n" PPA_M3A PPA_VA_M6_2 PPA_M3B
+      "s_sub_u32 s68, s68, 1\n"
+      ".Lpp_r2%=:\n" "s_cmp_lt_u32 s68, 3\n"
+      "s_cbranch_scc1 .Lpp_t2%=\n"
+      PPA_R0_5 PPA_DA1_S5 PPA_M0A_4 PPA_M0B PPA_R1_2 PPA_DB0_S6 PPA_M1A_2 PPA_M1B PPA_R2_2 PPA_DB1_S7
+      "s_add_u32 s66, s66, s73\n" "s_addc_u32 s67, s67, 0\n" PPA_M2A_2 PPA_VB_M6_2 PPA_M2B "s_add_u32 s64, s64, s72\n"
+      "s_addc_u32 s65, s65, 0\n" PPA_DA0_S8 "s_waitcnt vmcnt(6)\n" PPA_M3A PPA_VA_P4_2 PPA_M3B
+      "s_sub_u32 s68, s68, 1\n"
+      ".Lpp_r3%=:\n" "s_cmp_lt_u32 s68, 3\n"
+      "s_cbranch_scc1 .Lpp_t3%=\n"
+      PPA_R0_5 PPA_DA1_S9 PPA_M0A_4 PPA_M0B PPA_R1_2 PPA_DB0_S0 PPA_M1A_2 PPA_M1B PPA_R2_2 PPA_DB1_S1
+      "s_add_u32 s66, s66, s73\n" "s_addc_u32 s67, s67, 0\n" PPA_M2A_2 PPA_VB_P4_2 PPA_M2B "s_add_u32 s64, s64, s72\n"
+      "s_addc_u32 s65, s65, 0\n" PPA_DA0_S2 "s_waitcnt vmcnt(6)\n" PPA_M3A PPA_VA_P4_2 PPA_M3B
+      "s_sub_u32 s68, s68, 1\n"
+      ".Lpp_r4%=:\n" "s_cmp_lt_u32 s68, 3\n"
+      "s_cbranch_scc1 .Lpp_t4%=\n"
+      PPA_R0_5 PPA_DA1_S3 PPA_M0A_4 PPA_M0B PPA_R1_2 PPA_DB0_S4 PPA_M1A_2 PPA_M1B PPA_R2_2 PPA_DB1_S5
+      "s_add_u32 s66, s66, s73\n" "s_addc_u32 s67, s67, 0\n" PPA_M2A_2 PPA_VB_M6_2 PPA_M2B "s_add_u32 s64, s64, s72\n"
+      "s_addc_u32 s65, s65, 0\n" PPA_DA0_S6 "s_waitcnt vmcnt(6)\n" PPA_M3A PPA_VA_M6_2 PPA_M3B
+      "s_sub_u32 s68, s68, 1\n"
+      "s_branch .Lpp_r0%=\n"
+      ".Lpp_t0%=:\n" "s_cmp_lt_u32 s68, 2\n"
+      "s_cbranch_scc1 .Lpp_l0%=\n"
+      PPA_R0_5 PPA_DA1_S7 PPA_M0A_4 PPA_M0B PPA_R1_2 PPA_M1A_2 PPA_M1B PPA_R2_2 PPA_M2A_2 PPA_VB_P4_2 PPA_M2B
+      "s_waitcnt vmcnt(0)\n" PPA_M3A PPA_VA_P4_2 PPA_M3B
+      "s_branch .Lpp_l1%=\n"
+      ".Lpp_t1%=:\n" "s_cmp_lt_u32 s68, 2\n"
+      "s_cbranch_scc1 .Lpp_l1%=\n"
+      PPA_R0_5 PPA_DA1_S1 PPA_M0A_4 PPA_M0B PPA_R1_2 PPA_M1A_2 PPA_M1B PPA_R2_2 PPA_M2A_2 PPA_VB_P4_2 PPA_M2B
+      "s_waitcnt vmcnt(0)\n" PPA_M3A PPA_VA_M6_2 PPA_M3B
+      "s_branch .Lpp_l2%=\n"
+      ".Lpp_t2%=:\n" "s_cmp_lt_u32 s68, 2\n"
+      "s_cbranch_scc1 .Lpp_l2%=\n"
+      PPA_R0_5 PPA_DA1_S5 PPA_M0A_4 PPA_M0B PPA_R1_2 PPA_M1A_2 PPA_M1B PPA_R2_2 PPA_M2A_2 PPA_VB_M6_2 PPA_M2B
+      "s_waitcnt vmcnt(0)\n" PPA_M3A PPA_VA_P4_2 PPA_M3B
+      "s_branch .Lpp_l3%=\n"
+      ".Lpp_t3%=:\n" "s_cmp_lt_u32 s68, 2\n"
+      "s_cbranch_scc1 .Lpp_l3%=\n"
+      PPA_R0_5 PPA_DA1_S9 PPA_M0A_4 PPA_M0B PPA_R1_2 PPA_M1A_2 PPA_M1B PPA_R2_2 PPA_M2A_2 PPA_VB_P4_2 PPA_M2B
+      "s_waitcnt vmcnt(0)\n" PPA_M3A PPA_VA_P4_2 PPA_M3B
+      "s_branch .Lpp_l4%=\n"
+      ".Lpp_t4%=:\n" "s_cmp_lt_u32 s68, 2\n"
+      "s_cbranch_scc1 .Lpp_l4%=\n"
+      PPA_R0_5 PPA_DA1_S3 PPA_M0A_4 PPA_M0B PPA_R1_2 PPA_M1A_2 PPA_M1B PPA_R2_2 PPA_M2A_2 PPA_VB_M6_2 PPA_M2B
+      "s_waitcnt vmcnt(0)\n" PPA_M3A PPA_VA_M6_2 PPA_M3B
+      "s_branch .Lpp_l0%=\n"
+      ".Lpp_l0%=:\n" PPA_R0_5 PPA_M0A_4 PPA_M0B PPA_R1_2 PPA_M1A_2 PPA_M1B PPA_R2_2 PPA_M2A_2 PPA_M2B PPA_M3A PPA_M3B
+      "s_branch .Lpp_end%=\n"
+      ".Lpp_l1%=:\n" PPA_R0_5 PPA_M0A_4 PPA_M0B PPA_R1_2 PPA_M1A_2 PPA_M1B PPA_R2_2 PPA_M2A_2 PPA_M2B PPA_M3A PPA_M3B
+      "s_branch .Lpp_end%=\n"
+      ".Lpp_l2%=:\n" PPA_R0_5 PPA_M0A_4 PPA_M0B PPA_R1_2 PPA_M1A_2 PPA_M1B PPA_R2_2 PPA_M2A_2 PPA_M2B PPA_M3A PPA_M3B
+      "s_branch .Lpp_end%=\n"
+      ".Lpp_l3%=:\n" PPA_R0_5 PPA_M0A_4 PPA_M0B PPA_R1_2 PPA_M1A_2 PPA_M1B PPA_R2_2 PPA_M2A_2 PPA_M2B PPA_M3A PPA_M3B
+      "s_branch .Lpp_end%=\n"
+      ".Lpp_l4%=:\n" PPA_R0_5 PPA_M0A_4 PPA_M0B PPA_R1_2 PPA_M1A_2 PPA_M1B PPA_R2_2 PPA_M2A_2 PPA_M2B PPA_M3A PPA_M3B
+      "s_branch .Lpp_end%=\n"
+      ".Lpp_end%=:\n" "s_cmp_eq_u32 s75, 0\n"
+      "s_cbranch_scc0 .Lpp_g1%=\n"
+      "s_barrier\n"
+      ".Lpp_g1%=:\n" "s_nop 7\n" "s_nop 7\n"
+      : "+{v[0:15]}"(c[0]), "+{v[16:31]}"(c[1]), "+{v[32:47]}"(c[2]), "+{v[48:63]}"(c[3]), "+{v[64:79]}"(c[4]), "+{v[80:95]}"(c[5]), "+{v[96:111]}"(c[6]), "+{v[112:127]}"(c[7]),
+        "+{v[200:207]}"(f.ra), "+{v[208:211]}"(f.rb), "+{s[64:65]}"(ab), "+{s[66:67]}"(bb), "+{s68}"(nk)
+      : "{v[192:199]}"(f.dma), "{s[72:75]}"(sc)
+      : "memory", "m0", "scc", "v128", "v129", "v130", "v131", "v132", "v133", "v134", "v135", "v136", "v137", "v138", "v139", "v140", "v141", "v142", "v143", "v144", "v145", "v146", "v147", "v148", "v149", "v150", "v151", "v152", "v153", "v154", "v155", "v156", "v157", "v158", "v159", "v160", "v161", "v162", "v163", "v164", "v165", "v166", "v167", "v168", "v169", "v170", "v171", "v172", "v173", "v174", "v175", "v176", "v177", "v178", "v179", "v180", "v181", "v182", "v183", "v184", "v185", "v186", "v187", "v188", "v189", "v190", "v191");
+}
diff --git a/owl-audio-exps_amd/owl_wms/_lib/__init__.py b/owl-audio-exps_amd/owl_wms/_lib/__init__.py
--- a/owl-audio-exps_amd/owl_wms/_lib/__init__.py
+++ b/owl-audio-exps_amd/owl_wms/_lib/__init__.py
@@ -51,6 +51,7 @@
     "owlk_attn_bwd_fused": [P, L, L, P, L, L, P, L, L, P, L, L, P, P, P, L, L, P, L, L, P, L, L, L, I, L, I, F, L, I, I,
                             P, P, P, P, L, P, L, I, P],
     "owlk_set_cu_reserve": [I],
+    "owlk_set_gemm_pp": [I, L],
     "owlk_gemm_attn_delta": [L, L, L, P, L, P, L, P, L, P, L, L, I, I, P, P],
     "owlk_gemm_qk_rope": [L, L, L, P, L, P, L, P, P, L, I, I, P, P, L, L, L, L, P, L, P, P],
     "owlk_flow_noise": [P, P, P, I, I, L, P, P, P, P],
```

After: 152,800 latent-tokens/s, median of 6. +3.4%, better.
